# index-tts/index-tts

Measured on AMD Instinct MI355X. Metric: audio-seconds/sec (RTF) IndexTTS-2.5, 64-utt batch @1/2/4/8 MI355X, higher is better.
Workload: dtype bf16 (GPT GEMM operands / KV cache; f32 accumulate, residual stream, norms: the reference's own GPU mode) + fp32x3 (flow matching: f32 activations / weights / accumulation, GEMM and attention products on the bf16 matrix pipe with every f32 operand carried exactly as three bf16 planes = 24 significan

## Files before the change

### include/indextts_hip.h

```cpp
#ifndef INDEXTTS_HIP_H
#define INDEXTTS_HIP_H

#include <stddef.h>
#include <stdint.h>

#ifdef __cplusplus
extern "C" {
#endif

#define ITTS_ABI_VERSION 13

int itts_abi_version(void);
const char* itts_last_error(void);
int itts_device_count(void);

int itts_set_option(const char* name, int value);
int itts_get_option(const char* name, int* value);
int itts_reset_options(void);
int itts_option_count(void);
const char* itts_option_name(int index);
const char* itts_option_doc(int index);
int itts_option_default(int index);


int itts_aa_act_forward(const float* x, float* y, const float* alpha, const float* beta, const float* up_filter,
                        const float* down_filter, int B, int C, int T, const int32_t* lens, int len_mult,
                        int logscale, void* stream);

size_t itts_packed_conv_floats(int Cout, int Cin, int k);
int itts_pack_conv1d_weight(const float* w, int Cout, int Cin, int k, float* out);
int itts_pack_convT_weight(const float* w, int Cin, int Cout, int k, int u, int phase, float* out);

int itts_conv1d_forward(const float* x, const float* wpk, const float* bias, const float* bias_b, const float* res,
                        float* y, int B, int Cin, int Cout, int T, int k, int dilation, const int32_t* lens,
                        int len_mult, int acc_mode, float div, void* stream);

size_t itts_conv1d_h3_packed_bytes(int Cout, int Cin, int k);
int itts_pack_conv1d_h3_weight(const float* w, int Cout, int Cin, int k, void* out);
size_t itts_conv1d_h3_scratch_bytes(int B, int Cin, int T);
int itts_conv1d_h3_forward(const float* x, const void* wp3, const float* bias, const float* res, float* y, int B, int Cin, int Cout,
                           int T, int k, int dilation, const int32_t* lens, int len_mult, int acc_mode, float div, void* scratch,
                           void* stream);

size_t itts_conv1d_x3_packed_bytes(int Cout, int Cin, int k);
int itts_pack_conv1d_x3_weight(const float* w, int Cout, int Cin, int k, void* out);
size_t itts_conv1d_x3_scratch_bytes(int B, int Cin, int T);
int itts_conv1d_x3_forward(const float* x, const void* wp3, const float* bias, const float* res, float* y, int B, int Cin, int Cout,
                           int T, int k, int dilation, const int32_t* lens, int len_mult, int acc_mode, float div, void* scratch,
                           void* stream);
int itts_conv_transpose1d_forward(const float* x, const float* wpk_phases, const float* bias, const float* bias_b,
                                  float* y, int B, int Cin, int Cout, int Tin, int k, int u, const int32_t* lens,
                                  int len_mult_in, void* stream);

const char* itts_voc_last_path(void);
int itts_voc_path_count(void);
const char* itts_voc_path_name(int index);
int itts_aa_act_planes_forward(const float* x, void* planes, const float* alpha, const float* beta, const float* up_filter,
                               const float* down_filter, int B, int C, int T, const int32_t* lens, int len_mult, int logscale,
                               void* stream);
int itts_sin_reduced_forward(const float* x, float* y, size_t n, void* stream);

typedef struct {
    int32_t in_channels;
    int32_t upsample_initial_channel;
    int32_t num_upsamples;
    int32_t upsample_rates[8];
    int32_t upsample_kernel_sizes[8];
    int32_t num_kernels;
    int32_t resblock_kernel_sizes[4];
    int32_t num_dilations;
    int32_t resblock_dilations[4][4];
    int32_t snake_logscale;
    int32_t activation;
    int32_t use_tanh_at_final;
    int32_t use_bias_at_final;
    int32_t cond_dim;
    int32_t cond_in_each_up_layer;
} itts_bigvgan_config;

typedef struct itts_bigvgan itts_bigvgan;

int itts_bigvgan_create(const itts_bigvgan_config* cfg, itts_bigvgan** out);
int itts_bigvgan_device(const itts_bigvgan* h);
int itts_bigvgan_set_conv_mode(itts_bigvgan* h, int mode, int min_channels);
int itts_bigvgan_range_check(itts_bigvgan* h);
int itts_bigvgan_load_tensor(itts_bigvgan* h, const char* name, const float* host_data, const int64_t* shape, int ndim);
int itts_bigvgan_finalize(itts_bigvgan* h);
void itts_bigvgan_destroy(itts_bigvgan* h);
size_t itts_bigvgan_workspace_bytes(const itts_bigvgan* h, int B, int T);

int itts_bigvgan_forward(itts_bigvgan* h, const float* x, const int32_t* lens, const float* spk, float* wav, int B,
                         int T, void* workspace, size_t workspace_bytes, void* stream);

typedef struct itts_bigvgan_stream itts_bigvgan_stream;
int itts_bigvgan_stream_open(itts_bigvgan* h, int chunk_frames, int halo_frames, itts_bigvgan_stream** out);
size_t itts_bigvgan_stream_workspace_bytes(const itts_bigvgan_stream* s);
int itts_bigvgan_stream_push(itts_bigvgan_stream* s, const float* mel, int ld_mel, int n_frames, int is_last,
                             const float* spk, float* wav_out, int32_t* n_samples_out, void* workspace,
                             size_t workspace_bytes, void* stream);
void itts_bigvgan_stream_close(itts_bigvgan_stream* s);

int itts_bigvgan_set_profiling(itts_bigvgan* h, int enable);
int itts_bigvgan_profile_read(itts_bigvgan* h, double* ms, double* launches, double* flops, double* bytes);
int itts_bigvgan_profile_records(itts_bigvgan* h, double* out, int max_records);

#define ITTS_PREC_F32 0
#define ITTS_PREC_BF16 1
#define ITTS_PREC_F32X3 2

typedef struct {
    int32_t layers, model_dim, heads;
    int32_t vocab;
    int32_t n_mel_pos;
    int32_t precision;
    int32_t start_mel_token, stop_mel_token;
    float ln_eps;
} itts_gpt_config;

typedef struct {
    int32_t do_sample;
    int32_t num_beams;
    int32_t top_k;
    int32_t min_tokens_to_keep;
    int32_t max_new_tokens;
    int32_t pos_offset;
    float top_p, temperature, repetition_penalty, length_penalty;
    float typical_mass;
    int32_t reserved;
    uint64_t seed;
} itts_gen_params;

typedef struct itts_gpt itts_gpt;

size_t itts_packed_gemm_bytes(int K, int N, int precision);
int itts_pack_gemm_weight(const float* w, int K, int N, int transposed, int precision, void* out);

int itts_gpt_create(const itts_gpt_config* cfg, itts_gpt** out);
int itts_gpt_device(const itts_gpt* h);
int itts_gpt_load_tensor(itts_gpt* h, const char* name, const float* host_data, const int64_t* shape, int ndim);
int itts_gpt_finalize(itts_gpt* h);
void itts_gpt_destroy(itts_gpt* h);
size_t itts_gpt_workspace_bytes(const itts_gpt* h, int nseq, int S, int Tmax);

int itts_gpt_generate(itts_gpt* h, const float* prefix_embeds, const int32_t* pad_lens, int nseq, int S,
                      const itts_gen_params* params, const int32_t* penalty_ids, int n_penalty_ids,
                      const double* uniforms, int64_t* codes_out, int32_t* n_steps_out, void* workspace,
                      size_t workspace_bytes, int use_graph, void* stream);
int itts_gpt_generate_chunk(itts_gpt* h, const float* prefix_embeds, const int32_t* pad_lens, int nseq, int S,
                            const itts_gen_params* params, const int32_t* penalty_ids, int n_penalty_ids,
                            const double* uniforms, int64_t* codes_out, int32_t step_limit, int32_t* n_steps_out,
                            void* workspace, size_t workspace_bytes, int use_graph, void* stream);
size_t itts_gpt_admit_workspace_bytes(const itts_gpt* h, int n_new, int S_new);
int itts_gpt_admit_rows(itts_gpt* h, const float* prefix_embeds, const int32_t* pad_lens, const int32_t* slots, int n_new, int S_new,
                        const int32_t* row_limits_new, const itts_gen_params* params, const int32_t* penalty_ids, int n_penalty_ids,
                        const double* uniforms, int64_t* codes_out, void* workspace, size_t workspace_bytes, void* admit_workspace,
                        size_t admit_bytes, void* stream);
size_t itts_gpt_beam_workspace_bytes(const itts_gpt* h, int n_utts, int num_beams, int S, int Tmax);
int itts_gpt_generate_beam(itts_gpt* h, const float* prefix_embeds, const int32_t* pad_lens, int n_utts, int num_beams,
                           int S, const itts_gen_params* params, const int32_t* penalty_ids, int n_penalty_ids,
                           const double* uniforms, int32_t* hist_tok_out, int32_t* hist_par_out, float* beam_scores_out,
                           float* hyps_out, int32_t* n_hyps_out, uint8_t* done_out, int32_t* n_steps_out,
                           void* workspace, size_t workspace_bytes, int use_graph, void* stream);
int itts_gpt_generate_beam_chunk(itts_gpt* h, const float* prefix_embeds, const int32_t* pad_lens, int n_utts, int num_beams, int S,
                                 const itts_gen_params* params, const int32_t* penalty_ids, int n_penalty_ids, const int32_t* group_caps,
                                 int32_t* hist_tok_out, int32_t* hist_par_out, float* beam_scores_out, float* hyps_out, int32_t* n_hyps_out,
                                 uint8_t* done_out, int32_t step_limit, int32_t* n_steps_out, void* workspace, size_t workspace_bytes,
                                 int use_graph, void* stream);
size_t itts_gpt_admit_beam_workspace_bytes(const itts_gpt* h, int n_new, int S_new);
int itts_gpt_admit_beam_groups(itts_gpt* h, const float* prefix_embeds, const int32_t* pad_lens, const int32_t* slots, int n_new, int S_new,
                               const int32_t* group_caps_new, const itts_gen_params* params, const int32_t* penalty_ids, int n_penalty_ids,
                               void* workspace, size_t workspace_bytes, void* admit_workspace, size_t admit_bytes, void* stream);
int itts_gpt_last_timing(const itts_gpt* h, float* prefill_ms, float* decode_ms, int32_t* steps);
int itts_gpt_graph_stats(const itts_gpt* h, int32_t* captures, int32_t* hits);
int itts_gpt_set_compaction(itts_gpt* h, int enable, int granularity);
int itts_gpt_set_chunk_return(itts_gpt* h, int finished_rows);
int itts_gpt_set_row_limits(itts_gpt* h, const int32_t* limits, int n);
int itts_gpt_set_code_prefix(itts_gpt* h, const int64_t* codes, const int32_t* lens, int n, int width, int prefix_pos_offset, int chunk);
size_t itts_gpt_admit_prefix_workspace_bytes(const itts_gpt* h, int n_new, int S_new, int max_prefix);
int itts_gpt_last_prefix(const itts_gpt* h, int32_t* max_len, int32_t* chunks);
int itts_gpt_set_token_scores(itts_gpt* h, float* logp_model, float* logp_sampled, int n, int max_new);
int itts_gpt_set_alignment(itts_gpt* h, const int32_t* pairs, int n_pairs, const int32_t* span, float* out, int n, int max_new, int text_cap);
typedef struct {
    int32_t  do_sample, top_k, min_tokens_to_keep;
    float    top_p, temperature, repetition_penalty, typical_mass;
    int32_t  stream;
    uint64_t seed;
} itts_row_sampling;
int itts_gpt_set_row_sampling(itts_gpt* h, const itts_row_sampling* table, int n);
typedef struct {
    int32_t  do_sample, top_k, min_tokens_to_keep;
    float    top_p, temperature, repetition_penalty, typical_mass, length_penalty;
    int32_t  stream;
    uint64_t seed;
} itts_group_sampling;
int itts_gpt_set_group_sampling(itts_gpt* h, const itts_group_sampling* table, int n_groups);
typedef struct {
    int32_t  min_new_tokens;
    int32_t  min_length;
    int32_t  no_repeat_ngram_size;
    int32_t  decay_start;
    float    min_p;
    float    epsilon_cutoff;
    float    eta_cutoff;
    int32_t  n_suppress, n_begin_suppress, n_decay;
    const int32_t* suppress_ids;
    const int32_t* begin_suppress_ids;
    const float*   decay_table;
} itts_logits_filters;
int itts_gpt_set_logits_filters(itts_gpt* h, const itts_logits_filters* f);
int itts_gpt_compaction_stats(const itts_gpt* h, int64_t* row_steps, int32_t* compactions);

int itts_gpt_forward_latent(itts_gpt* h, const float* x, int nseq, int S, float* out, void* workspace,
                            size_t workspace_bytes, void* stream);
// ... 155 lines not shown
```

### indextts_amd/_lib.py

```python
import ctypes as C
import os

HERE = os.path.dirname(os.path.abspath(__file__))
LIB_PATH = os.path.join(HERE, "csrc", "libindextts_hip.so")

c_f32p = C.POINTER(C.c_float)
c_i32p = C.POINTER(C.c_int32)
c_i64p = C.POINTER(C.c_int64)
vp = C.c_void_p


class BigVGANConfig(C.Structure):
    _fields_ = [
        ("in_channels", C.c_int32), ("upsample_initial_channel", C.c_int32), ("num_upsamples", C.c_int32),
        ("upsample_rates", C.c_int32 * 8), ("upsample_kernel_sizes", C.c_int32 * 8), ("num_kernels", C.c_int32),
        ("resblock_kernel_sizes", C.c_int32 * 4), ("num_dilations", C.c_int32),
        ("resblock_dilations", (C.c_int32 * 4) * 4), ("snake_logscale", C.c_int32), ("activation", C.c_int32),
        ("use_tanh_at_final", C.c_int32), ("use_bias_at_final", C.c_int32), ("cond_dim", C.c_int32),
        ("cond_in_each_up_layer", C.c_int32),
    ]


class S2MelConfig(C.Structure):
    _fields_ = [("hidden_dim", C.c_int32), ("num_heads", C.c_int32), ("depth", C.c_int32), ("in_channels", C.c_int32),
                ("wavenet_hidden", C.c_int32), ("wavenet_layers", C.c_int32), ("wavenet_kernel", C.c_int32),
                ("wavenet_dilation_rate", C.c_int32), ("precision", C.c_int32), ("norm_eps", C.c_float)]


class FbankConfig(C.Structure):
    _fields_ = [("frame_length", C.c_int32), ("hop", C.c_int32), ("n_fft", C.c_int32), ("n_mels", C.c_int32), ("pad", C.c_int32),
                ("remove_dc", C.c_int32), ("power", C.c_int32), ("take_log", C.c_int32), ("layout", C.c_int32),
                ("preemphasis", C.c_float), ("mag_eps", C.c_float), ("floor", C.c_float), ("scale", C.c_float)]


class GPTConfig(C.Structure):
    _fields_ = [("layers", C.c_int32), ("model_dim", C.c_int32), ("heads", C.c_int32), ("vocab", C.c_int32),
                ("n_mel_pos", C.c_int32), ("precision", C.c_int32), ("start_mel_token", C.c_int32),
                ("stop_mel_token", C.c_int32), ("ln_eps", C.c_float)]


ABI_VERSION = 13
ERR_ARG, ERR_HIP, ERR_STATE = 1, 2, 3


class GenParams(C.Structure):
    _fields_ = [("do_sample", C.c_int32), ("num_beams", C.c_int32), ("top_k", C.c_int32),
                ("min_tokens_to_keep", C.c_int32), ("max_new_tokens", C.c_int32), ("pos_offset", C.c_int32),
                ("top_p", C.c_float), ("temperature", C.c_float), ("repetition_penalty", C.c_float),
                ("length_penalty", C.c_float), ("typical_mass", C.c_float), ("reserved", C.c_int32),
                ("seed", C.c_uint64)]


class RowSampling(C.Structure):
    _fields_ = [("do_sample", C.c_int32), ("top_k", C.c_int32), ("min_tokens_to_keep", C.c_int32),
                ("top_p", C.c_float), ("temperature", C.c_float), ("repetition_penalty", C.c_float),
                ("typical_mass", C.c_float), ("stream", C.c_int32), ("seed", C.c_uint64)]


class GroupSampling(C.Structure):
    _fields_ = [("do_sample", C.c_int32), ("top_k", C.c_int32), ("min_tokens_to_keep", C.c_int32),
                ("top_p", C.c_float), ("temperature", C.c_float), ("repetition_penalty", C.c_float),
                ("typical_mass", C.c_float), ("length_penalty", C.c_float), ("stream", C.c_int32), ("seed", C.c_uint64)]


class LogitsFilters(C.Structure):
    _fields_ = [("min_new_tokens", C.c_int32), ("min_length", C.c_int32), ("no_repeat_ngram_size", C.c_int32), ("decay_start", C.c_int32),
                ("min_p", C.c_float), ("epsilon_cutoff", C.c_float), ("eta_cutoff", C.c_float),
                ("n_suppress", C.c_int32), ("n_begin_suppress", C.c_int32), ("n_decay", C.c_int32),
                ("suppress_ids", C.POINTER(C.c_int32)), ("begin_suppress_ids", C.POINTER(C.c_int32)), ("decay_table", C.POINTER(C.c_float))]


SIGNATURES = {
    "itts_abi_version": (C.c_int, []),
    "itts_last_error": (C.c_char_p, []),
    "itts_device_count": (C.c_int, []),
    "itts_set_option": (C.c_int, [C.c_char_p, C.c_int]),
    "itts_get_option": (C.c_int, [C.c_char_p, C.POINTER(C.c_int)]),
    "itts_reset_options": (C.c_int, []),
    "itts_option_count": (C.c_int, []),
    "itts_option_name": (C.c_char_p, [C.c_int]),
    "itts_option_doc": (C.c_char_p, [C.c_int]),
    "itts_option_default": (C.c_int, [C.c_int]),
    "itts_aa_act_forward": (C.c_int, [vp, vp, vp, vp, vp, vp, C.c_int, C.c_int, C.c_int, vp, C.c_int, C.c_int, vp]),
    "itts_packed_conv_floats": (C.c_size_t, [C.c_int, C.c_int, C.c_int]),
    "itts_pack_conv1d_weight": (C.c_int, [vp, C.c_int, C.c_int, C.c_int, vp]),
    "itts_pack_convT_weight": (C.c_int, [vp, C.c_int, C.c_int, C.c_int, C.c_int, C.c_int, vp]),
    "itts_conv1d_forward": (C.c_int, [vp, vp, vp, vp, vp, vp, C.c_int, C.c_int, C.c_int, C.c_int, C.c_int, C.c_int,
                                      vp, C.c_int, C.c_int, C.c_float, vp]),
    "itts_conv_transpose1d_forward": (C.c_int, [vp, vp, vp, vp, vp, C.c_int, C.c_int, C.c_int, C.c_int, C.c_int,
                                                C.c_int, vp, C.c_int, vp]),
    "itts_voc_last_path": (C.c_char_p, []),
    "itts_voc_path_count": (C.c_int, []),
    "itts_voc_path_name": (C.c_char_p, [C.c_int]),
    "itts_aa_act_planes_forward": (C.c_int, [vp, vp, vp, vp, vp, vp, C.c_int, C.c_int, C.c_int, vp, C.c_int, C.c_int, vp]),
    "itts_sin_reduced_forward": (C.c_int, [vp, vp, C.c_size_t, vp]),
    "itts_bigvgan_create": (C.c_int, [C.POINTER(BigVGANConfig), C.POINTER(vp)]),
    "itts_bigvgan_device": (C.c_int, [vp]),
    "itts_bigvgan_load_tensor": (C.c_int, [vp, C.c_char_p, vp, c_i64p, C.c_int]),
    "itts_bigvgan_set_conv_mode": (C.c_int, [vp, C.c_int, C.c_int]),
    "itts_bigvgan_range_check": (C.c_int, [vp]),
    "itts_conv1d_h3_packed_bytes": (C.c_size_t, [C.c_int, C.c_int, C.c_int]),
    "itts_pack_conv1d_h3_weight": (C.c_int, [vp, C.c_int, C.c_int, C.c_int, vp]),
    "itts_conv1d_h3_scratch_bytes": (C.c_size_t, [C.c_int, C.c_int, C.c_int]),
    "itts_conv1d_h3_forward": (C.c_int, [vp, vp, vp, vp, vp, C.c_int, C.c_int, C.c_int, C.c_int, C.c_int, C.c_int, vp, C.c_int, C.c_int,
                                         C.c_float, vp, vp]),
    "itts_conv1d_x3_packed_bytes": (C.c_size_t, [C.c_int, C.c_int, C.c_int]),
    "itts_pack_conv1d_x3_weight": (C.c_int, [vp, C.c_int, C.c_int, C.c_int, vp]),
    "itts_conv1d_x3_scratch_bytes": (C.c_size_t, [C.c_int, C.c_int, C.c_int]),
    "itts_conv1d_x3_forward": (C.c_int, [vp, vp, vp, vp, vp, C.c_int, C.c_int, C.c_int, C.c_int, C.c_int, C.c_int, vp, C.c_int, C.c_int,
                                         C.c_float, vp, vp]),
    "itts_bigvgan_finalize": (C.c_int, [vp]),
    "itts_bigvgan_destroy": (None, [vp]),
    "itts_bigvgan_workspace_bytes": (C.c_size_t, [vp, C.c_int, C.c_int]),
    "itts_bigvgan_forward": (C.c_int, [vp, vp, vp, vp, vp, C.c_int, C.c_int, vp, C.c_size_t, vp]),
    "itts_bigvgan_stream_open": (C.c_int, [vp, C.c_int, C.c_int, C.POINTER(vp)]),
    "itts_bigvgan_stream_workspace_bytes": (C.c_size_t, [vp]),
    "itts_bigvgan_stream_push": (C.c_int, [vp, vp, C.c_int, C.c_int, C.c_int, vp, vp, C.POINTER(C.c_int32), vp, C.c_size_t, vp]),
    "itts_bigvgan_stream_close": (None, [vp]),
    "itts_bigvgan_set_profiling": (C.c_int, [vp, C.c_int]),
    "itts_bigvgan_profile_read": (C.c_int, [vp, vp, vp, vp, vp]),
    "itts_bigvgan_profile_records": (C.c_int, [vp, vp, C.c_int]),
    "itts_packed_gemm_bytes": (C.c_size_t, [C.c_int, C.c_int, C.c_int]),
    "itts_pack_gemm_weight": (C.c_int, [vp, C.c_int, C.c_int, C.c_int, C.c_int, vp]),
    "itts_gpt_create": (C.c_int, [C.POINTER(GPTConfig), C.POINTER(vp)]),
    "itts_gpt_device": (C.c_int, [vp]),
    "itts_gpt_load_tensor": (C.c_int, [vp, C.c_char_p, vp, c_i64p, C.c_int]),
    "itts_gpt_finalize": (C.c_int, [vp]),
    "itts_gpt_destroy": (None, [vp]),
    "itts_gpt_workspace_bytes": (C.c_size_t, [vp, C.c_int, C.c_int, C.c_int]),
    "itts_gpt_generate": (C.c_int, [vp, vp, vp, C.c_int, C.c_int, C.POINTER(GenParams), c_i32p, C.c_int, vp, vp,
                                    C.POINTER(C.c_int32), vp, C.c_size_t, C.c_int, vp]),
    "itts_gpt_generate_chunk": (C.c_int, [vp, vp, vp, C.c_int, C.c_int, C.POINTER(GenParams), c_i32p, C.c_int, vp, vp, C.c_int32,
                                          C.POINTER(C.c_int32), vp, C.c_size_t, C.c_int, vp]),
    "itts_gpt_beam_workspace_bytes": (C.c_size_t, [vp, C.c_int, C.c_int, C.c_int, C.c_int]),
    "itts_gpt_generate_beam": (C.c_int, [vp, vp, vp, C.c_int, C.c_int, C.c_int, C.POINTER(GenParams), c_i32p, C.c_int, vp,
                                         vp, vp, vp, vp, vp, vp, C.POINTER(C.c_int32), vp, C.c_size_t, C.c_int, vp]),
    "itts_gpt_admit_workspace_bytes": (C.c_size_t, [vp, C.c_int, C.c_int]),
    "itts_gpt_admit_rows": (C.c_int, [vp, vp, vp, vp, C.c_int, C.c_int, vp, vp, vp, C.c_int, vp, vp, vp, C.c_size_t, vp, C.c_size_t, vp]),
    "itts_gpt_generate_beam_chunk": (C.c_int, [vp, vp, vp, C.c_int, C.c_int, C.c_int, C.POINTER(GenParams), c_i32p, C.c_int, c_i32p,
                                               vp, vp, vp, vp, vp, vp, C.c_int32, C.POINTER(C.c_int32), vp, C.c_size_t, C.c_int, vp]),
    "itts_gpt_admit_beam_workspace_bytes": (C.c_size_t, [vp, C.c_int, C.c_int]),
    "itts_gpt_admit_beam_groups": (C.c_int, [vp, vp, vp, c_i32p, C.c_int, C.c_int, c_i32p, C.POINTER(GenParams), c_i32p, C.c_int,
                                             vp, C.c_size_t, vp, C.c_size_t, vp]),
    "itts_gpt_last_timing": (C.c_int, [vp, C.POINTER(C.c_float), C.POINTER(C.c_float), C.POINTER(C.c_int32)]),
    "itts_gpt_graph_stats": (C.c_int, [vp, C.POINTER(C.c_int32), C.POINTER(C.c_int32)]),
    "itts_gpt_set_compaction": (C.c_int, [vp, C.c_int, C.c_int]),
    "itts_gpt_set_row_limits": (C.c_int, [vp, vp, C.c_int]),
    "itts_gpt_set_code_prefix": (C.c_int, [vp, vp, c_i32p, C.c_int, C.c_int, C.c_int, C.c_int]),
    "itts_gpt_admit_prefix_workspace_bytes": (C.c_size_t, [vp, C.c_int, C.c_int, C.c_int]),
    "itts_gpt_last_prefix": (C.c_int, [vp, C.POINTER(C.c_int32), C.POINTER(C.c_int32)]),
    "itts_gpt_set_token_scores": (C.c_int, [vp, vp, vp, C.c_int, C.c_int]),
    "itts_gpt_set_alignment": (C.c_int, [vp, C.POINTER(C.c_int32), C.c_int, vp, vp, C.c_int, C.c_int, C.c_int]),
    "itts_gpt_set_row_sampling": (C.c_int, [vp, vp, C.c_int]),
    "itts_gpt_set_group_sampling": (C.c_int, [vp, vp, C.c_int]),
    "itts_gpt_set_logits_filters": (C.c_int, [vp, C.POINTER(LogitsFilters)]),
    "itts_gpt_set_chunk_return": (C.c_int, [vp, C.c_int]),
    "itts_gpt_compaction_stats": (C.c_int, [vp, C.POINTER(C.c_int64), C.POINTER(C.c_int32)]),
    "itts_gpt_forward_latent": (C.c_int, [vp, vp, C.c_int, C.c_int, vp, vp, C.c_size_t, vp]),
    "itts_gpt_latent_workspace_bytes": (C.c_size_t, [vp, C.c_int, C.c_int, C.c_int, C.c_int]),
    "itts_gpt_latent_open": (C.c_int, [vp, vp, c_i32p, C.c_int, C.c_int, C.c_int, C.c_int, vp, C.c_size_t, vp, C.POINTER(vp)]),
    "itts_gpt_latent_append": (C.c_int, [vp, vp, C.c_int, vp, vp]),
    "itts_gpt_latent_appended": (C.c_int, [vp]),
    "itts_gpt_latent_close": (C.c_int, [vp]),
    "itts_gpt_rescore_workspace_bytes": (C.c_size_t, [vp, C.c_int, C.c_int, C.c_int, C.c_int]),
    "itts_gpt_rescore": (C.c_int, [vp, vp, vp, C.c_int, C.c_int, vp, c_i32p, C.c_int, C.c_int, vp, c_i32p, C.c_int, vp, vp, C.c_int, C.c_int,
                                   vp, C.c_size_t, vp]),
    "itts_gpt_logp_gather_forward": (C.c_int, [vp, vp, vp, C.c_int, C.c_int, C.c_int, vp]),
    "itts_gpt_attention_align_mq_forward": (C.c_int, [vp, vp, vp, vp, C.POINTER(C.c_int32), C.c_int, vp, vp, vp, vp, vp,
                                                      C.c_int, C.c_int, C.c_int, C.c_int, C.c_int, C.c_int, C.c_int, C.c_int, C.c_int, vp]),
    "itts_gemm_tile_occupancy": (C.c_int, [C.c_int, C.POINTER(C.c_int32)]),
    "itts_s2mel_create": (C.c_int, [C.POINTER(S2MelConfig), C.POINTER(vp)]),
    "itts_s2mel_device": (C.c_int, [vp]),
    "itts_s2mel_load_tensor": (C.c_int, [vp, C.c_char_p, vp, c_i64p, C.c_int]),
    "itts_s2mel_set_tail": (C.c_int, [vp, vp, vp, vp, vp, vp, vp, vp, C.c_int, C.c_int, C.c_int]),
    "itts_s2mel_finalize": (C.c_int, [vp]),
    "itts_s2mel_destroy": (None, [vp]),
    "itts_s2mel_workspace_bytes": (C.c_size_t, [vp, C.c_int, C.c_int, C.c_int]),
    "itts_s2mel_mods_per_step": (C.c_int, [vp]),
    "itts_s2mel_estimator": (C.c_int, [vp, vp, vp, vp, vp, vp, vp, vp, vp, vp, C.c_int, C.c_int, C.c_int, vp, vp, C.c_size_t, vp]),
    "itts_s2mel_solve": (C.c_int, [vp, vp, vp, vp, vp, vp, vp, vp, vp, vp, vp, C.c_int, C.c_int, C.c_int, C.c_int, C.c_int,
                                   C.POINTER(C.c_float), C.c_float, vp, C.c_size_t, vp]),
    "itts_s2mel_set_profiling": (C.c_int, [vp, C.c_int]),
    "itts_s2mel_profile_read": (C.c_int, [vp, vp, vp, vp]),
    "itts_s2mel_set_trace": (C.c_int, [vp, vp, C.c_int]),
    "itts_s2mel_trace_count": (C.c_int, [vp]),
    "itts_s2mel_trace_wanted": (C.c_int, [vp]),
    "itts_s2mel_trace_label": (C.c_char_p, [vp, C.c_int]),
    "itts_s2mel_set_capture": (C.c_int, [vp, vp, C.c_size_t, C.c_char_p]),
    "itts_s2mel_capture_offset": (C.c_longlong, [vp, C.c_int, C.POINTER(C.c_size_t)]),
    "itts_s2mel_noise_forward": (C.c_int, [vp, vp, vp, vp, vp, vp, vp, C.c_int, C.c_int, C.c_int, vp]),
    "itts_s2mel_attention_scratch_bytes": (C.c_size_t, [C.c_int, C.c_int, C.c_int, C.c_int, C.c_int]),
    "itts_s2mel_attention_forward": (C.c_int, [vp, vp, vp, vp, vp, vp, vp, C.c_int, C.c_int, C.c_int, C.c_int, C.c_int, vp, vp,
                                               C.c_size_t, vp]),
    "itts_vq_project_forward": (C.c_int, [vp, vp, vp, vp, vp, C.c_int, C.c_int, C.c_int, C.c_int, vp]),
    "itts_vq_search_forward": (C.c_int, [vp, vp, vp, vp, vp, vp, C.c_int, C.c_int, C.c_int, C.c_int, vp]),
    "itts_tok_gather_conv_forward": (C.c_int, [vp, vp, vp, vp, vp, vp, vp, C.c_int, C.c_int, C.c_int, vp]),
    "itts_tok_dwconv_forward": (C.c_int, [vp, vp, vp, vp, vp, vp, vp, C.c_int, C.c_int, C.c_int, vp]),
    "itts_tok_gelu_forward": (C.c_int, [vp, C.c_size_t, vp]),
    "itts_attention_forward": (C.c_int, [vp, vp, vp, vp, vp, vp, C.c_int, C.c_int, C.c_int, C.c_int, C.c_float, vp]),
    "itts_attention_relkey_forward": (C.c_int, [vp, vp, vp, vp, vp, vp, vp, vp, C.c_int, C.c_int, C.c_int, C.c_int, C.c_int, C.c_int, C.c_float, vp]),
    "itts_tok_dwconv_causal_forward": (C.c_int, [vp, vp, vp, vp, vp, vp, vp, C.c_int, C.c_int, C.c_int, vp]),
    "itts_tok_glu_forward": (C.c_int, [vp, vp, C.c_int, C.c_int, C.c_int, vp]),
    "itts_tok_act_forward": (C.c_int, [vp, C.c_size_t, C.c_int, vp]),
    "itts_tok_l2norm_forward": (C.c_int, [vp, vp, C.c_int, C.c_int, C.c_float, vp]),
    "itts_tok_affine_forward": (C.c_int, [vp, C.c_int, vp, vp, vp, C.c_int, C.c_int, C.c_int, vp]),
    "itts_tok_ctxpool_forward": (C.c_int, [vp, vp, C.c_int, C.c_int, C.c_int, vp]),
    "itts_tok_gate_forward": (C.c_int, [vp, vp, C.c_size_t, vp]),
    "itts_tok_attnstats_forward": (C.c_int, [vp, vp, vp, C.c_int, C.c_int, C.c_float, vp]),
    "itts_tok_statspool_forward": (C.c_int, [vp, vp, C.c_int, C.c_int, vp]),
    "itts_tok_ctxpool_seq_forward": (C.c_int, [vp, vp, vp, vp, C.c_int, C.c_int, C.c_int, vp]),
    "itts_tok_statspool_seq_forward": (C.c_int, [vp, vp, vp, vp, C.c_int, C.c_int, vp]),
    "itts_tok_gather_conv1d_seq_forward": (C.c_int, [vp, vp, vp, vp, vp, vp, C.c_int, C.c_int, C.c_int, C.c_int, C.c_int, C.c_int, vp]),
    "itts_tok_gather_conv2d_seq_forward": (C.c_int, [vp, vp, vp, vp, C.c_int, C.c_int, C.c_int, C.c_int, C.c_int, vp]),
    "itts_tok_scale_residual_forward": (C.c_int, [vp, vp, vp, C.c_int, C.c_int, vp]),
    "itts_tok_groupnorm_mish_forward": (C.c_int, [vp, vp, vp, vp, vp, C.c_int, C.c_int, C.c_float, vp]),
    "itts_gemm_last_path": (C.c_char_p, []),
    "itts_gemm_path_count": (C.c_int, []),
    "itts_gemm_path_name": (C.c_char_p, [C.c_int]),
    "itts_gemm_forward": (C.c_int, [vp, vp, vp, vp, C.c_int, C.c_int, C.c_int, C.c_int, C.c_int, C.c_int, vp]),
    "itts_attention_last_path": (C.c_char_p, []),
    "itts_attention_path_count": (C.c_int, []),
    "itts_attention_path_name": (C.c_char_p, [C.c_int]),
    "itts_gpt_attention_forward": (C.c_int, [vp, vp, vp, vp, vp, vp, vp, vp, vp, vp, vp, C.c_int, C.c_int, C.c_int, C.c_int, C.c_int, C.c_int, vp]),
    "itts_gpt_attention_align_forward": (C.c_int, [vp, vp, vp, vp, C.POINTER(C.c_int32), C.c_int, vp, vp, vp, vp, vp, vp, vp, vp, vp,
                                                   C.c_int, C.c_int, C.c_int, C.c_int, C.c_int, C.c_int, C.c_int, vp]),
    "itts_layernorm_forward": (C.c_int, [vp, vp, vp, vp, vp, vp, C.c_int, C.c_int, C.c_float, vp]),
    "itts_gemm_ln_forward": (C.c_int, [vp, vp, vp, vp, vp, C.c_float, vp, vp, vp, vp, C.c_int, C.c_int, C.c_int, vp]),
    "itts_fbank_frames": (C.c_int, [C.POINTER(FbankConfig), C.c_int]),
    "itts_fbank_forward": (C.c_int, [vp, C.c_int, C.c_int, C.c_int64, C.POINTER(FbankConfig), vp, vp, vp, vp, C.c_int, C.c_int64, vp]),
    "itts_resample_forward": (C.c_int, [vp, vp, vp, C.c_int, C.c_int, C.c_int64, C.c_int, C.c_int64, C.c_int, C.c_int, C.c_int, vp]),
    "itts_tok_colnorm_forward": (C.c_int, [vp, vp, C.c_int, C.c_int, C.c_int, C.c_int, C.c_int, C.c_float, vp]),
}

_lib = None


class HipEngineError(RuntimeError):
    pass


def lib():
    global _lib
    if _lib is None:
        if not os.path.exists(LIB_PATH):
            raise HipEngineError(
                f"{LIB_PATH} is missing: build it with `python indextts_amd/build.py` (hipcc, gfx950). "
                "The engine has no CPU fallback.")
        import torch
# ... 104 lines not shown
```

### indextts_amd/bigvgan.py

```python
import ctypes as C
import json
import os
from typing import Dict, Optional

import torch

from . import _lib

_V2_DEFAULTS = dict(
    num_mels=80, upsample_rates=[4, 4, 2, 2, 2, 2], upsample_kernel_sizes=[8, 8, 4, 4, 4, 4],
    upsample_initial_channel=1536, resblock_kernel_sizes=[3, 7, 11],
    resblock_dilation_sizes=[[1, 3, 5], [1, 3, 5], [1, 3, 5]], activation="snakebeta", snake_logscale=True,
    use_tanh_at_final=True, use_bias_at_final=True, resblock="1")


def fold_weight_norm(sd: Dict[str, torch.Tensor]) -> Dict[str, torch.Tensor]:
    out = dict(sd)
    for k in list(sd.keys()):
        if k.endswith(".weight_g"):
            base, g, v = k[:-9], sd[k], sd[k[:-9] + ".weight_v"]
        elif k.endswith(".parametrizations.weight.original0"):
            base = k[: -len(".parametrizations.weight.original0")]
            g, v = sd[k], sd[base + ".parametrizations.weight.original1"]
        else:
# ... 178 lines not shown
                spk = spk.expand(x.shape[0], -1).contiguous()
        else:
            spk = None
        x = x.float().contiguous()
        B, Cin, T = x.shape
        if Cin != self.in_channels:
            raise ValueError(f"expected {self.in_channels} input channels, got {Cin}")
        wav = torch.empty(B, 1, T * self.total_up, dtype=torch.float32, device=x.device)
        if B == 0 or T == 0:
            return (wav, None) if v1 else wav
        lens_t = None
        if lens is not None:
            lens_t = torch.as_tensor(lens, dtype=torch.int32, device=x.device).contiguous()
            if lens_t.numel() != B:
                raise ValueError("lens must have one entry per batch row")
        ws = self._workspace(B, T, x.device)
        rc = _lib.lib().itts_bigvgan_forward(self._h, _lib.ptr(x), _lib.ptr(lens_t), _lib.ptr(spk), _lib.ptr(wav), B, T,
                                             _lib.ptr(ws), ws.numel(), _lib.stream_ptr(x.device))
        _lib.check(rc, "itts_bigvgan_forward")
        if self.conv_mode == 1:
            bad = _lib.lib().itts_bigvgan_range_check(self._h)
            if bad:
                raise _lib.HipEngineError("BigVGAN(conv_mode='f16x3'): an activation was not finite or outside the f16 range "
                                          "(|x| >= 65504); use the exact f32 mode for this model / input")
        return (wav, None) if v1 else wav

    __call__ = forward

    def receptive_field_frames(self) -> int:
        h = self.h
        kmax = max(h["resblock_kernel_sizes"])
        reach = 0
        for d in max(h["resblock_dilation_sizes"], key=lambda ds: sum(ds)):
            reach += 6 + (kmax - 1) // 2 * d + 6 + (kmax - 1) // 2
        frames, rate = 3.0, 1
        for u, k in zip(h["upsample_rates"], h["upsample_kernel_sizes"]):
            frames += (k / u) / rate
            rate *= u
            frames += reach / rate
        frames += (6 + 3) / rate
        return int(frames) + 2

    def stream(self, mel: torch.Tensor, chunk_frames: int = 256, halo_frames: Optional[int] = None):
        halo = self.receptive_field_frames() if halo_frames is None else int(halo_frames)
        T = mel.shape[-1]
        up = self.total_up
        for t0 in range(0, T, chunk_frames):
            t1 = min(T, t0 + chunk_frames)
            a, b = max(0, t0 - halo), min(T, t1 + halo)
            w = self.forward(mel[..., a:b].contiguous())
            yield w[..., (t0 - a) * up: (t0 - a) * up + (t1 - t0) * up]

    def open_stream(self, chunk_frames: int = 256, halo_frames: Optional[int] = None) -> "BigVGANStream":
        return BigVGANStream(self, chunk_frames, self.receptive_field_frames() if halo_frames is None else int(halo_frames))

    def forward_chunked(self, mel: torch.Tensor, chunk_frames: int = 256, halo_frames: Optional[int] = None) -> torch.Tensor:
        return torch.cat(list(self.stream(mel, chunk_frames, halo_frames)), dim=-1)

    def set_profiling(self, enable: bool):
        _lib.check(_lib.lib().itts_bigvgan_set_profiling(self._h, int(enable)), "itts_bigvgan_set_profiling")

    def profile_records(self):
        buf = (C.c_double * (4 * 1024))()
        n = _lib.lib().itts_bigvgan_profile_records(self._h, buf, 1024)
        if n < 0:
            _lib.check(1, "itts_bigvgan_profile_records")
        return [(int(buf[4 * i]), buf[4 * i + 1], buf[4 * i + 2], buf[4 * i + 3]) for i in range(min(n, 1024))]

    def profile(self):
        arr = [(C.c_double * 4)() for _ in range(4)]
        _lib.check(_lib.lib().itts_bigvgan_profile_read(self._h, *arr), "itts_bigvgan_profile_read")
        names = ("conv1d_mfma", "conv_transpose1d_mfma", "aa_activation", "conv_post")
        return {n: dict(ms=arr[0][i], launches=int(arr[1][i]), flops=arr[2][i], bytes=arr[3][i]) for i, n in enumerate(names)}

    def __del__(self):
        try:
            if getattr(self, "_h", None) and self._h.value:
                _lib.lib().itts_bigvgan_destroy(self._h)
                self._h = C.c_void_p()
        except Exception:
            pass


class BigVGANStream:
    def __init__(self, model: BigVGAN, chunk_frames: int, halo_frames: int):
        if model.cond_dim > 0:
            raise NotImplementedError("streaming is wired for the v2 generator (no speaker conditioning)")
        self.model, self.chunk, self.halo = model, int(chunk_frames), int(halo_frames)
        self._s = C.c_void_p()
        _lib.check(_lib.lib().itts_bigvgan_stream_open(model._h, self.chunk, self.halo, C.byref(self._s)), "itts_bigvgan_stream_open")
        self._ws = None

    def push(self, mel_chunk: torch.Tensor, last: bool = False) -> torch.Tensor:
        n_new = int(mel_chunk.shape[-1])
        x = mel_chunk.reshape(self.model.in_channels, n_new).float().contiguous()
        if not x.is_cuda:
            raise _lib.HipEngineError("BigVGANStream needs a CUDA/HIP tensor")
        L = _lib.lib()
        if self._ws is None:
            self._ws = torch.empty(L.itts_bigvgan_stream_workspace_bytes(self._s), dtype=torch.uint8, device=x.device)
        out = torch.empty((self.chunk + self.halo) * self.model.total_up, dtype=torch.float32, device=x.device)
        n = C.c_int32(0)
        _lib.check(L.itts_bigvgan_stream_push(self._s, _lib.ptr(x) if n_new else None, max(1, n_new), n_new,
                                              int(last), None, _lib.ptr(out), C.byref(n), _lib.ptr(self._ws), self._ws.numel(),
                                              _lib.stream_ptr(x.device)), "itts_bigvgan_stream_push")
        return out[: n.value].reshape(1, 1, -1)

    def close(self):
        if self._s and self._s.value:
            _lib.lib().itts_bigvgan_stream_close(self._s)
            self._s = C.c_void_p()

    def __del__(self):
        try:
            self.close()
        except Exception:
            pass


def anti_alias_activation(x, up_filter, down_filter, alpha, beta, lens=None, logscale=True, *, len_mult=1, out=None):
    if not x.is_cuda:
        raise _lib.HipEngineError("anti_alias_activation needs a device tensor")
    x = x.float().contiguous()
    y = out if out is not None else torch.empty_like(x)
    B, Cc, T = x.shape
    dev = x.device
    f = lambda t: t.detach().reshape(-1).to(dev, torch.float32).contiguous()
    a, b, fu, fd = f(alpha), f(beta), f(up_filter), f(down_filter)
    lens_t = None if lens is None else torch.as_tensor(lens, dtype=torch.int32, device=dev).contiguous()
    with _lib.on_device(x.device):
        _lib.check(_lib.lib().itts_aa_act_forward(_lib.ptr(x), _lib.ptr(y), _lib.ptr(a), _lib.ptr(b), _lib.ptr(fu),
                                                  _lib.ptr(fd), B, Cc, T, _lib.ptr(lens_t), int(len_mult), int(logscale),
                                                  _lib.stream_ptr(x.device)), "itts_aa_act_forward")
        return y


def anti_alias_activation_planes(x, up_filter, down_filter, alpha, beta, lens=None, logscale=True, *, len_mult=1, out=None):
    if not x.is_cuda:
        raise _lib.HipEngineError("anti_alias_activation_planes needs a device tensor")
    x = x.float().contiguous()
    B, Cc, T = x.shape
    dev = x.device
    p = out if out is not None else torch.empty(3, B, T, Cc, dtype=torch.bfloat16, device=dev)
    f = lambda t: t.detach().reshape(-1).to(dev, torch.float32).contiguous()
    a, b, fu, fd = f(alpha), f(beta), f(up_filter), f(down_filter)
    lens_t = None if lens is None else torch.as_tensor(lens, dtype=torch.int32, device=dev).contiguous()
    with _lib.on_device(x.device):
        _lib.check(_lib.lib().itts_aa_act_planes_forward(_lib.ptr(x), _lib.ptr(p), _lib.ptr(a), _lib.ptr(b), _lib.ptr(fu), _lib.ptr(fd), B, Cc, T,
                                                         _lib.ptr(lens_t), int(len_mult), int(logscale), _lib.stream_ptr(x.device)),
                   "itts_aa_act_planes_forward")
        return p


def sin_reduced(x):
    if not x.is_cuda:
        raise _lib.HipEngineError("sin_reduced needs a device tensor")
    x = x.float().contiguous()
    y = torch.empty_like(x)
    with _lib.on_device(x.device):
        _lib.check(_lib.lib().itts_sin_reduced_forward(_lib.ptr(x), _lib.ptr(y), x.numel(), _lib.stream_ptr(x.device)), "itts_sin_reduced_forward")
        return y


def pack_conv1d_weight(w: torch.Tensor) -> torch.Tensor:
    w = w.detach().to("cpu", torch.float32).contiguous()
    Cout, Cin, k = w.shape
    L = _lib.lib()
    out = torch.empty(L.itts_packed_conv_floats(Cout, Cin, k), dtype=torch.float32)
    _lib.check(L.itts_pack_conv1d_weight(_lib.ptr(w), Cout, Cin, k, _lib.ptr(out)), "itts_pack_conv1d_weight")
    return out


def pack_conv1d_h3_weight(w: torch.Tensor) -> torch.Tensor:
    w = w.detach().to("cpu", torch.float32).contiguous()
    Cout, Cin, k = w.shape
    L = _lib.lib()
    n = L.itts_conv1d_h3_packed_bytes(Cout, Cin, k)
    if n == 0:
        raise ValueError("pack_conv1d_h3_weight: C_in must be a multiple of 32")
    out = torch.empty(n, dtype=torch.uint8)
    _lib.check(L.itts_pack_conv1d_h3_weight(_lib.ptr(w), Cout, Cin, k, _lib.ptr(out)), "itts_pack_conv1d_h3_weight")
    return out


def conv1d_h3(x, w3_packed, bias, Cout, k, dilation=1, res=None, lens=None, len_mult=1, out=None, acc_mode=0, div=1.0):
    x = x.float().contiguous()
    B, Cin, T = x.shape
    y = out if out is not None else torch.empty(B, Cout, T, dtype=torch.float32, device=x.device)
    lens_t = None if lens is None else torch.as_tensor(lens, dtype=torch.int32, device=x.device).contiguous()
    L = _lib.lib()
    scratch = torch.empty(L.itts_conv1d_h3_scratch_bytes(B, Cin, T), dtype=torch.uint8, device=x.device)
    with _lib.on_device(x.device):
        _lib.check(L.itts_conv1d_h3_forward(_lib.ptr(x), _lib.ptr(w3_packed), _lib.ptr(bias), _lib.ptr(res), _lib.ptr(y), B, Cin, Cout, T, k,
                                            dilation, _lib.ptr(lens_t), len_mult, acc_mode, float(div), _lib.ptr(scratch),
                                            _lib.stream_ptr(x.device)), "itts_conv1d_h3_forward")
        return y


def pack_conv1d_x3_weight(w: torch.Tensor) -> torch.Tensor:
    w = w.detach().to("cpu", torch.float32).contiguous()
    Cout, Cin, k = w.shape
    L = _lib.lib()
    n = L.itts_conv1d_x3_packed_bytes(Cout, Cin, k)
    if n == 0:
        raise ValueError("pack_conv1d_x3_weight: C_in must be a multiple of 32")
    out = torch.empty(n, dtype=torch.uint8)
    _lib.check(L.itts_pack_conv1d_x3_weight(_lib.ptr(w), Cout, Cin, k, _lib.ptr(out)), "itts_pack_conv1d_x3_weight")
    return out


def conv1d_x3(x, w3_packed, bias, Cout, k, dilation=1, res=None, lens=None, len_mult=1, out=None, acc_mode=0, div=1.0):
    x = x.float().contiguous()
    B, Cin, T = x.shape
    y = out if out is not None else torch.empty(B, Cout, T, dtype=torch.float32, device=x.device)
    lens_t = None if lens is None else torch.as_tensor(lens, dtype=torch.int32, device=x.device).contiguous()
    L = _lib.lib()
    scratch = torch.empty(L.itts_conv1d_x3_scratch_bytes(B, Cin, T), dtype=torch.uint8, device=x.device)
    with _lib.on_device(x.device):
        _lib.check(L.itts_conv1d_x3_forward(_lib.ptr(x), _lib.ptr(w3_packed), _lib.ptr(bias), _lib.ptr(res), _lib.ptr(y), B, Cin, Cout, T, k,
                                            dilation, _lib.ptr(lens_t), len_mult, acc_mode, float(div), _lib.ptr(scratch),
                                            _lib.stream_ptr(x.device)), "itts_conv1d_x3_forward")
        return y


def pack_convT_weight(w: torch.Tensor, u: int) -> torch.Tensor:
    w = w.detach().to("cpu", torch.float32).contiguous()
    Cin, Cout, k = w.shape
    L = _lib.lib()
    per = L.itts_packed_conv_floats(Cout, Cin, k // u)
    out = torch.empty(per * u, dtype=torch.float32)
    for r in range(u):
        _lib.check(L.itts_pack_convT_weight(_lib.ptr(w), Cin, Cout, k, u, r, C.c_void_p(out.data_ptr() + 4 * per * r)),
                   "itts_pack_convT_weight")
    return out


def conv1d(x, w_packed, bias, Cout, k, dilation=1, res=None, lens=None, len_mult=1, out=None, acc_mode=0, div=1.0, *, bias_b=None):
    x = x.float().contiguous()
    B, Cin, T = x.shape
    y = out if out is not None else torch.empty(B, Cout, T, dtype=torch.float32, device=x.device)
    lens_t = None if lens is None else torch.as_tensor(lens, dtype=torch.int32, device=x.device).contiguous()
    with _lib.on_device(x.device):
        _lib.check(_lib.lib().itts_conv1d_forward(_lib.ptr(x), _lib.ptr(w_packed), _lib.ptr(bias), _lib.ptr(bias_b), _lib.ptr(res),
                                                  _lib.ptr(y), B, Cin, Cout, T, k, dilation, _lib.ptr(lens_t), len_mult,
                                                  acc_mode, float(div), _lib.stream_ptr(x.device)), "itts_conv1d_forward")
        return y


def conv_transpose1d(x, w_packed, bias, Cout, k, u, lens=None, *, bias_b=None, len_mult=1, out=None):
    x = x.float().contiguous()
    B, Cin, T = x.shape
    y = out if out is not None else torch.zeros(B, Cout, T * u, dtype=torch.float32, device=x.device)
    lens_t = None if lens is None else torch.as_tensor(lens, dtype=torch.int32, device=x.device).contiguous()
    with _lib.on_device(x.device):
        _lib.check(_lib.lib().itts_conv_transpose1d_forward(_lib.ptr(x), _lib.ptr(w_packed), _lib.ptr(bias), _lib.ptr(bias_b),
                                                            _lib.ptr(y), B, Cin, Cout, T, k, u, _lib.ptr(lens_t), int(len_mult),
                                                            _lib.stream_ptr(x.device)), "itts_conv_transpose1d_forward")
        return y
```

### indextts_amd/csrc/bigvgan_kernels.h

```cpp
#pragma once
#include "common.h"

struct ConvArgs {
    const float* x;
    float* y;
    const float* wpk;
    const float* bias;
    const float* bias_b;
    const float* res;
    const int* lens;
    int len_mult_in, len_mult_out;
    int Cin, Cout, Tin, Tout;
    int k, tap_base, tap_step, ostride, ooff, m_extra;
    int acc_mode;
    float div;
    int B, n_mt, n_co;
};

enum VocPath {
    VP_NONE = -1,
    VP_CONV_F32_BM32, VP_CONV_F32_BM64, VP_CONV_F32_BM96, VP_CONV_F32_BM128,
    VP_CONV_X3_NH1, VP_CONV_X3_NH2,
    VP_CONV_H3_TWO_STAGE, VP_CONV_H3_WIN256X128, VP_CONV_H3_WIN192X192, VP_CONV_H3_WIN256X96,
    VP_AA_V1_SINF, VP_AA_V2_SINF, VP_AA_V2_VSIN, VP_AA_PLANES_VSIN,
    VP_COUNT
};
void voc_note_path(int path);
int voc_last_path();
const char* voc_path_name(int path);

int launch_aa_act(const float* x, float* y, const float* alpha, const float* beta, const float* fu, const float* fd,
                  int B, int C, int T, const int* lens, int len_mult, int logscale, hipStream_t st);
int launch_sin_reduced(const float* x, float* y, size_t n, hipStream_t st);
int launch_conv(const ConvArgs& a, int B, hipStream_t st);
int launch_conv_post(const float* x, float* y, const float* w, const float* bias, int B, int Cin, int T, int k,
                     const int* lens, int len_mult, int use_tanh, hipStream_t st);
int launch_cond_bias(const float* spk, const float* w, const float* bias, float* out, int B, int Cout, int cond_dim,
                     hipStream_t st);

struct ConvH3Args {
    const void* xh; const void* xl;
    const void* wp;
    const float* bias;
    const float* res;
    float* y;
    const void* zero_row;
    const int* lens; int len_mult;
    int B, Cin, Cout, T, k, dil;
    int acc_mode; float div;
    int n_mt, n_co;
};
struct ConvX3Args {
    const void* xp;
    const void* wp;
    const float* bias;
    const float* res;
    float* y;
    const void* zero_row;
    const int* lens; int len_mult;
    int B, Cin, Cout, T, k, dil;
    int acc_mode; float div;
    int n_mt, n_co;
};
bool conv_x3_supported(int Cin, int Cout, int k, int dil);
size_t conv_x3_packed_bytes(int Cout, int Cin, int k);
int conv_x3_pack(const float* w, int Cout, int Cin, int k, void* out);
int launch_split_tm3(const float* x, void* xp, int B, int C, int T, const int* lens, int len_mult, hipStream_t st);
int launch_aa_act_planes(const float* x, void* xp, const float* alpha, const float* beta, const float* fu, const float* fd,
                         int B, int C, int T, const int* lens, int len_mult, int logscale, hipStream_t st);
int launch_conv_x3(const ConvX3Args& a, hipStream_t st);
size_t conv_h3_packed_bytes(int Cout, int Cin, int k);
int conv_h3_pack(const float* w, int Cout, int Cin, int k, void* out);
int launch_split_tm(const float* x, void* xh, void* xl, int B, int C, int T, const int* lens, int len_mult, int* range_flag, hipStream_t st);
int launch_conv_h3(const ConvH3Args& a, hipStream_t st);
```

### indextts_amd/csrc/bigvgan_kernels.hip

```cpp
#include "bigvgan_kernels.h"
#include <stdlib.h>

#define AA_TILE 1024

__global__ __launch_bounds__(256) void aa_act_kernel(const float* __restrict__ x, float* __restrict__ y,
                                                     const float* __restrict__ alpha, const float* __restrict__ beta,
                                                     const float* __restrict__ fu, const float* __restrict__ fd,
                                                     int C, int T, const int* __restrict__ lens, int len_mult,
                                                     int logscale) {
    __shared__ float xs[AA_TILE + 16];
    __shared__ float vs[2 * AA_TILE + 16];
    __shared__ float fus[12], fds[12];
    const int b = blockIdx.z, c = blockIdx.y;
    const int t0 = blockIdx.x * AA_TILE;
    const int len = lens ? min(lens[b] * len_mult, T) : T;
    if (t0 >= len) return;
    const int tid = threadIdx.x;
    if (tid < 12) { fus[tid] = fu[tid]; fds[tid] = fd[tid]; }
    const float* xr = x + ((size_t)b * C + c) * T;
    float* yr = y + ((size_t)b * C + c) * T;
    float a_e = alpha[c], b_e = beta[c];
    if (logscale) { a_e = expf(a_e); b_e = expf(b_e); }
    const float inv_b = 1.0f / (b_e + 1e-9f);
    const int n_out = min(AA_TILE, len - t0);
// ... 142 lines not shown
            for (int p = 0; p < 4; ++p)
                if (i0 + p < n_out) yr[t0 + i0 + p] = o[p];
        }
    }
}

#define AAP_TT 128
#define AAP_CB 32
#define AAP_RS 36
__device__ __forceinline__ uint32_t aap_cvt2(float a, float b) {
    typedef __bf16 bf2 __attribute__((ext_vector_type(2)));
    typedef float f2 __attribute__((ext_vector_type(2)));
    return __builtin_bit_cast(uint32_t, __builtin_convertvector(f2{a, b}, bf2));
}
__device__ __forceinline__ void aap_wave_sync() {
    __builtin_amdgcn_fence(__ATOMIC_RELEASE, "wavefront");
    __builtin_amdgcn_wave_barrier();
    __builtin_amdgcn_fence(__ATOMIC_ACQUIRE, "wavefront");
}
__device__ __forceinline__ int aap_slot(int tt) { return (tt & 3) * 32 + (tt >> 2); }

__global__ __launch_bounds__(256) void aa_act_planes_kernel(const float* __restrict__ x, u16* __restrict__ xh, u16* __restrict__ xm, u16* __restrict__ xl,
                                                            const float* __restrict__ alpha, const float* __restrict__ beta,
                                                            const float* __restrict__ fu, const float* __restrict__ fd,
                                                            int C, int T, const int* __restrict__ lens, int len_mult, int logscale) {
    __shared__ __attribute__((aligned(256))) float xs[4][2][192];
    __shared__ __attribute__((aligned(256))) float vs[4][2][320];
    __shared__ __attribute__((aligned(16))) u16 ot[3][AAP_TT][AAP_RS];
    const int b = blockIdx.z, c0 = blockIdx.y * AAP_CB, t0 = blockIdx.x * AAP_TT;
    const int tid = threadIdx.x, lane = tid & 63, w = tid >> 6, sub = lane >> 5, pos = lane & 31;
    const int len = lens ? min(lens[b] * len_mult, T) : T;
    const int n_out = len - t0 < AAP_TT ? (len - t0 < 0 ? 0 : len - t0) : AAP_TT;
    if (n_out > 0) {
        float fus[12], fds[12];
#pragma unroll
        for (int j = 0; j < 12; ++j) { fus[j] = 2.0f * fu[j]; fds[j] = fd[j]; }
        float* xw_ = xs[w][sub];
        float* vw_ = vs[w][sub];
        int toff[5];
#pragma unroll
        for (int k = 0; k < 5; ++k) {
            int t = t0 - 6 + pos + 32 * k;
            toff[k] = t < 0 ? 0 : (t > len - 1 ? len - 1 : t);
        }
        auto chan = [&](int it) { const int c = c0 + w * 8 + it * 2 + sub; return c < C ? c : C - 1; };
        float xn[5];
        {
            const float* xr = x + ((size_t)b * C + chan(0)) * T;
#pragma unroll
            for (int k = 0; k < 5; ++k) xn[k] = xr[toff[k]];
        }
#pragma unroll 1
        for (int it = 0; it < 4; ++it) {
            const int cl = w * 8 + it * 2 + sub;
            const bool c_ok = c0 + cl < C;
            float a_e = alpha[chan(it)], b_e = beta[chan(it)];
            if (logscale) { a_e = expf(a_e); b_e = expf(b_e); }
            const float inv_b = 1.0f / (b_e + 1e-9f);
            aap_wave_sync();
#pragma unroll
            for (int k = 0; k < 5; ++k) xw_[pos + 32 * k] = xn[k];
            if (it < 3) {
                const float* xr = x + ((size_t)b * C + chan(it + 1)) * T;
#pragma unroll
                for (int k = 0; k < 5; ++k) xn[k] = xr[toff[k]];
            }
            aap_wave_sync();
            auto snake8 = [&](int vb, float* v) {
                float xw[12];
                *(f32x4*)&xw[0] = *(const f32x4*)&xw_[(vb >> 1)];
                *(f32x4*)&xw[4] = *(const f32x4*)&xw_[(vb >> 1) + 4];
                *(f32x4*)&xw[8] = *(const f32x4*)&xw_[(vb >> 1) + 8];
#pragma unroll
                for (int p = 0; p < 4; ++p) {
                    float ue = 0.f, uo = 0.f;
#pragma unroll
                    for (int j = 0; j < 6; ++j) {
                        ue = fmaf(fus[1 + 2 * j], xw[p + 5 - j], ue);
                        uo = fmaf(fus[2 * j], xw[p + 6 - j], uo);
                    }
                    const float se = sin_reduced(ue * a_e);
                    const float so = sin_reduced(uo * a_e);
                    v[2 * p] = fmaf(inv_b * se, se, ue);
                    v[2 * p + 1] = fmaf(inv_b * so, so, uo);
                }
            };
            {
                float v[8];
                const int vb = 8 * pos;
                snake8(vb, v);
                *(f32x4*)&vw_[aa_sw(vb)] = *(const f32x4*)&v[0];
                *(f32x4*)&vw_[aa_sw(vb + 4)] = *(const f32x4*)&v[4];
            }
            if (pos < 2) {
                float vt[8];
                snake8(2 * AAP_TT + 8 * pos, vt);
                *(f32x4*)&vw_[aa_sw(2 * AAP_TT + 8 * pos)] = *(const f32x4*)&vt[0];
                *(f32x4*)&vw_[aa_sw(2 * AAP_TT + 8 * pos + 4)] = *(const f32x4*)&vt[4];
            }
            aap_wave_sync();
            if (t0 == 0 && pos < 6) vw_[aa_sw(pos)] = vw_[aa_sw(6)];
            const int vi_end = (2 * len - 1) - (2 * t0 - 6);
            if (vi_end < 2 * AAP_TT + 12 - 1) {
                const int vi = vi_end + 1 + pos;
                if (pos < 8 && vi < 2 * AAP_TT + 16) vw_[aa_sw(vi)] = vw_[aa_sw(vi_end)];
            }
            aap_wave_sync();
            float vw[20];
            const int base = 8 * pos;
#pragma unroll
            for (int k = 0; k < 5; ++k) *(f32x4*)&vw[4 * k] = *(const f32x4*)&vw_[aa_sw(base + 4 * k)];
            float o[4];
#pragma unroll
            for (int p = 0; p < 4; ++p) {
                float acc = 0.f;
#pragma unroll
                for (int j = 0; j < 12; ++j) acc = fmaf(fds[j], vw[2 * p + j + 1], acc);
                o[p] = (4 * pos + p < n_out && c_ok) ? acc : 0.f;
            }
#pragma unroll
            for (int e = 0; e < 2; ++e) {
                const float f0 = o[2 * e], f1 = o[2 * e + 1];
                const uint32_t h = aap_cvt2(f0, f1);
                const float r0 = f0 - __uint_as_float(h << 16), r1 = f1 - __uint_as_float(h & 0xffff0000u);
                const uint32_t m = aap_cvt2(r0, r1);
                const float s0 = r0 - __uint_as_float(m << 16), s1 = r1 - __uint_as_float(m & 0xffff0000u);
                const uint32_t l = aap_cvt2(s0, s1);
                const int sa = aap_slot(4 * pos + 2 * e), sb = aap_slot(4 * pos + 2 * e + 1);
                ot[0][sa][cl] = (u16)h; ot[0][sb][cl] = (u16)(h >> 16);
                ot[1][sa][cl] = (u16)m; ot[1][sb][cl] = (u16)(m >> 16);
                ot[2][sa][cl] = (u16)l; ot[2][sb][cl] = (u16)(l >> 16);
            }
        }
    }
    __syncthreads();
    const size_t plane_row = (size_t)b * T;
    const int q = tid & 3;
#pragma unroll 1
    for (int r = tid >> 2; r < 3 * AAP_TT; r += 64) {
        const int p = r / AAP_TT, tt = r - p * AAP_TT;
        const int t = t0 + tt;
        if (t >= T || c0 + 8 * q >= C) continue;
        uint2 lo = {0u, 0u}, hi = {0u, 0u};
        if (n_out > 0) {
            const u16* src = &ot[p][aap_slot(tt)][8 * q];
            lo = *(const uint2*)src;
            hi = *(const uint2*)(src + 4);
        }
        u16* dst = (p == 0 ? xh : (p == 1 ? xm : xl)) + (plane_row + t) * C + c0 + 8 * q;
        *(uint4*)dst = uint4{lo.x, lo.y, hi.x, hi.y};
    }
}

#define CI_CHUNK 32
#define CONV_HALO 64


template <int WM, int WN, int MT, int NT>
__global__ __launch_bounds__(256) __attribute__((amdgpu_waves_per_eu((WM == 1 && MT == 1) ? 4 : 1, (WM == 1 && MT == 1) ? 4 : 8)))
void conv_mfma_kernel(ConvArgs a) {
    constexpr int BM = WM * MT * 32;
    constexpr int BN = WN * NT * 32;
    constexpr int LDW = BN + CONV_HALO;
    extern __shared__ __attribute__((aligned(16))) float xs[];

    const int tid = threadIdx.x, lane = tid & 63, w = tid >> 6;
    const int wm = w / WN, wn = w % WN;
    const int L = blockIdx.x;
    const int xcd = L & 7, slot = L >> 3;
    const int tile = (slot / a.n_co) * 8 + xcd;
    if (tile >= a.n_mt * a.B) return;
    const int b = tile / a.n_mt;
    const int m0 = (tile - b * a.n_mt) * BN;
    const int co0 = (slot % a.n_co) * BM;
    const int len_in = a.lens ? min(a.lens[b] * a.len_mult_in, a.Tin) : a.Tin;
    const int len_out = a.lens ? min(a.lens[b] * a.len_mult_out, a.Tout) : a.Tout;
    const int m_count = len_in + a.m_extra;
    if (m0 >= m_count) return;

    const int span = (a.k - 1) * (a.tap_step < 0 ? -a.tap_step : a.tap_step);
    const int last_off = a.tap_base + (a.k - 1) * a.tap_step;
    const int min_off = a.tap_base < last_off ? a.tap_base : last_off;
    const int W = BN + span;
    const int n_cosub = (a.Cout + 31) >> 5;
    const int cin8 = a.Cin >> 3;

    f32x16 acc[MT][NT];
#pragma unroll
    for (int i = 0; i < MT; ++i)
#pragma unroll
        for (int j = 0; j < NT; ++j)
#pragma unroll
            for (int r = 0; r < 16; ++r) acc[i][j][r] = 0.f;

    const float* xb = a.x + (size_t)b * a.Cin * a.Tin;
    const int lane_row = lane >> 5;
    const int lane_col = lane & 31;

    constexpr int NCOL = LDW / 64;
    float stage[CI_CHUNK / 4][NCOL];
    const int w_u = __builtin_amdgcn_readfirstlane(w);
    auto stage_load = [&](int ci0s) {
        const int cnt = min(CI_CHUNK, a.Cin - ci0s);
#pragma unroll
        for (int rr = 0; rr < CI_CHUNK / 4; ++rr) {
            const int r = w_u + 4 * rr;
            const bool row_ok = r < cnt;
            const float* xr = xb + (size_t)(ci0s + (row_ok ? r : 0)) * a.Tin;
            const __amdgpu_buffer_rsrc_t rsrc =
                __builtin_amdgcn_make_buffer_rsrc(const_cast<float*>(xr), 0, row_ok ? len_in * 4 : 0, 0x00020000);
#pragma unroll
            for (int i = 0; i < NCOL; ++i) {
                const int t = m0 + min_off + lane + 64 * i;
                stage[rr][i] = __builtin_bit_cast(float, __builtin_amdgcn_raw_buffer_load_b32(rsrc, t * 4, 0, 0));
            }
        }
    };
    auto stage_write = [&]() {
#pragma unroll
        for (int rr = 0; rr < CI_CHUNK / 4; ++rr)
#pragma unroll
            for (int i = 0; i < NCOL; ++i) xs[(w + 4 * rr) * LDW + lane + 64 * i] = stage[rr][i];
    };
    stage_load(0);

    constexpr int CP4 = CI_CHUNK / 8;
    f32x4 a_cur[CP4][MT], a_nxt[CP4][MT];
    const int nchunks = (a.Cin + CI_CHUNK - 1) / CI_CHUNK;
    const int G = nchunks * a.k;
    const unsigned wpk_bytes = (unsigned)n_cosub * a.k * cin8 * 64u * 16u;
    const __amdgpu_buffer_rsrc_t wrs = __builtin_amdgcn_make_buffer_rsrc(const_cast<float*>(a.wpk), 0, (int)wpk_bytes, 0x00020000);
    auto load_tap = [&](int g, f32x4 (&dst)[CP4][MT]) {
        const int c = g / a.k, j = g - c * a.k;
        const int cbase = c * CI_CHUNK;
        const int cp4n = min(CI_CHUNK, a.Cin - cbase) >> 3;
#pragma unroll
        for (int cp4 = 0; cp4 < CP4; ++cp4) {
#pragma unroll
            for (int mt = 0; mt < MT; ++mt) {
                const int co_sub = (co0 >> 5) + wm * MT + mt;
                const bool ok = (cp4 < cp4n) && (co_sub < n_cosub);
                const unsigned off = ok ? ((unsigned)((co_sub * a.k + j) * cin8 + ((cbase >> 3) + cp4)) * 64u + lane) * 16u
                                        : 0xFFFFFFF0u;
                dst[cp4][mt] = __builtin_bit_cast(f32x4, __builtin_amdgcn_raw_buffer_load_b128(wrs, off, 0, 0));
            }
        }
    };
    auto compute_tap = [&](int j) {
        const int colb = wn * NT * 32 + lane_col + (a.tap_base + j * a.tap_step - min_off);
        const float* xcol = xs + lane_row * LDW + colb;
        float bcur[4][NT], bnxt[4][NT];
#pragma unroll
        for (int sidx = 0; sidx < 4; ++sidx)
#pragma unroll
            for (int nt = 0; nt < NT; ++nt) bcur[sidx][nt] = xcol[(2 * sidx) * LDW + nt * 32];
#pragma unroll
        for (int cp4 = 0; cp4 < CP4; ++cp4) {
            if (cp4 + 1 < CP4) {
#pragma unroll
                for (int sidx = 0; sidx < 4; ++sidx)
#pragma unroll
                    for (int nt = 0; nt < NT; ++nt) bnxt[sidx][nt] = xcol[((cp4 + 1) * 8 + 2 * sidx) * LDW + nt * 32];
            }
#pragma unroll
            for (int sidx = 0; sidx < 4; ++sidx)
#pragma unroll
                for (int mt = 0; mt < MT; ++mt)
#pragma unroll
                    for (int nt = 0; nt < NT; ++nt)
                        acc[mt][nt] = __builtin_amdgcn_mfma_f32_32x32x2f32(a_cur[cp4][mt][sidx], bcur[sidx][nt], acc[mt][nt], 0, 0, 0);
            if (cp4 + 1 < CP4) {
#pragma unroll
                for (int sidx = 0; sidx < 4; ++sidx)
#pragma unroll
                    for (int nt = 0; nt < NT; ++nt) bcur[sidx][nt] = bnxt[sidx][nt];
            }
        }
#pragma unroll
        for (int cp4 = 0; cp4 < CP4; ++cp4)
#pragma unroll
            for (int mt = 0; mt < MT; ++mt) a_cur[cp4][mt] = a_nxt[cp4][mt];
    };
    load_tap(0, a_cur);
    int g = 0;
    for (int ci0 = 0; ci0 < a.Cin; ci0 += CI_CHUNK) {
        __syncthreads();
        stage_write();
        __syncthreads();
        load_tap(g + 1 < G ? g + 1 : G - 1, a_nxt);
        stage_load(ci0 + CI_CHUNK);
        compute_tap(0);
        ++g;
        for (int j = 1; j < a.k; ++j, ++g) {
            load_tap(g + 1 < G ? g + 1 : G - 1, a_nxt);
            compute_tap(j);
        }
    }

    const int plane_bytes = a.Cout * a.Tout * 4;
    const __amdgpu_buffer_rsrc_t yrs =
        __builtin_amdgcn_make_buffer_rsrc(a.y + (size_t)b * a.Cout * a.Tout, 0, plane_bytes, 0x00020000);
    const float* resb = a.res ? a.res + (size_t)b * a.Cout * a.Tout : a.y;
    const __amdgpu_buffer_rsrc_t rrs = __builtin_amdgcn_make_buffer_rsrc(const_cast<float*>(resb), 0, plane_bytes, 0x00020000);
#pragma unroll
    for (int mt = 0; mt < MT; ++mt) {
#pragma unroll
        for (int hf = 0; hf < 2; ++hf) {
            int corow[8];
            float badd[8];
#pragma unroll
            for (int q = 0; q < 8; ++q) {
                const int r = hf * 8 + q;
                corow[q] = co0 + (wm * MT + mt) * 32 + (r & 3) + 8 * (r >> 2) + 4 * lane_row;
                badd[q] = 0.f;
            }
            if (a.bias) {
#pragma unroll
                for (int q = 0; q < 8; ++q) badd[q] = a.bias[corow[q] < a.Cout ? corow[q] : a.Cout - 1];
            }
            if (a.bias_b) {
                const float* bb = a.bias_b + (size_t)b * a.Cout;
#pragma unroll
                for (int q = 0; q < 8; ++q) badd[q] += bb[corow[q] < a.Cout ? corow[q] : a.Cout - 1];
            }
#pragma unroll
            for (int nt = 0; nt < NT; ++nt) {
                const int m = m0 + (wn * NT + nt) * 32 + lane_col;
                const int n = m * a.ostride + a.ooff;
                const bool n_ok = (m < m_count) && (n >= 0) && (n < len_out);
                unsigned voff[8];
                float v[8];
#pragma unroll
                for (int q = 0; q < 8; ++q) {
                    const bool ok = n_ok && corow[q] < a.Cout;
                    voff[q] = ok ? (unsigned)(corow[q] * a.Tout + n) * 4u : 0xFFFFFFF0u;
                    v[q] = acc[mt][nt][hf * 8 + q] + badd[q];
                }
                if (a.res) {
                    float rv[8];
#pragma unroll
                    for (int q = 0; q < 8; ++q) rv[q] = __builtin_bit_cast(float, __builtin_amdgcn_raw_buffer_load_b32(rrs, voff[q], 0, 0));
#pragma unroll
                    for (int q = 0; q < 8; ++q) v[q] += rv[q];
                }
                if (a.acc_mode != 0) {
                    float yo[8];
#pragma unroll
                    for (int q = 0; q < 8; ++q) yo[q] = __builtin_bit_cast(float, __builtin_amdgcn_raw_buffer_load_b32(yrs, voff[q], 0, 0));
#pragma unroll
                    for (int q = 0; q < 8; ++q) v[q] = a.acc_mode == 1 ? yo[q] + v[q] : (yo[q] + v[q]) / a.div;
                }
#pragma unroll
                for (int q = 0; q < 8; ++q) __builtin_amdgcn_raw_buffer_store_b32(__builtin_bit_cast(unsigned, v[q]), yrs, voff[q], 0, 0);
            }
        }
    }
}

__global__ __launch_bounds__(256) void conv_post_kernel(const float* __restrict__ x, float* __restrict__ y,
                                                        const float* __restrict__ w, const float* __restrict__ bias,
                                                        int Cin, int T, int k, const int* __restrict__ lens,
                                                        int len_mult, int use_tanh) {
    extern __shared__ float ws[];
    const int b = blockIdx.y;
    for (int i = threadIdx.x; i < Cin * k; i += 256) ws[i] = w[i];
    __syncthreads();
    const int t = blockIdx.x * 256 + threadIdx.x;
    if (t >= T) return;
    const int len = lens ? min(lens[b] * len_mult, T) : T;
    float acc = 0.f;
    if (t < len) {
        const int pad = (k - 1) / 2;
        acc = bias ? bias[0] : 0.f;
        const float* xb = x + (size_t)b * Cin * T;
        for (int ci = 0; ci < Cin; ++ci) {
            const float* xr = xb + (size_t)ci * T;
            for (int j = 0; j < k; ++j) {
                const int tt = t + j - pad;
                if (tt >= 0 && tt < len) acc = fmaf(ws[ci * k + j], xr[tt], acc);
            }
        }
        acc = use_tanh ? tanhf(acc) : fminf(1.0f, fmaxf(-1.0f, acc));
    }
    y[(size_t)b * T + t] = acc;
}

__global__ __launch_bounds__(256) void cond_bias_kernel(const float* __restrict__ spk, const float* __restrict__ w,
                                                        const float* __restrict__ bias, float* __restrict__ out,
                                                        int Cout, int cond_dim) {
    const int b = blockIdx.y;
    const int co = blockIdx.x * 256 + threadIdx.x;
    if (co >= Cout) return;
    float acc = bias ? bias[co] : 0.f;
    const float* wr = w + (size_t)co * cond_dim;
    const float* sr = spk + (size_t)b * cond_dim;
    for (int d = 0; d < cond_dim; ++d) acc = fmaf(wr[d], sr[d], acc);
    out[(size_t)b * Cout + co] = acc;
}

static const char* const kVocPathNames[VP_COUNT] = {
    "conv_f32_bm32", "conv_f32_bm64", "conv_f32_bm96", "conv_f32_bm128",
    "conv_x3_nh1", "conv_x3_nh2",
    "conv_h3_two_stage", "conv_h3_win256x128", "conv_h3_win192x192", "conv_h3_win256x96",
    "aa_v1_sinf", "aa_v2_sinf", "aa_v2_vsin", "aa_planes_vsin",
};
static thread_local int t_voc_last_path = VP_NONE;
void voc_note_path(int path) { t_voc_last_path = path; }
int voc_last_path() { return t_voc_last_path; }
const char* voc_path_name(int path) { return (path >= 0 && path < VP_COUNT) ? kVocPathNames[path] : nullptr; }

int launch_aa_act(const float* x, float* y, const float* alpha, const float* beta, const float* fu, const float* fd,
                  int B, int C, int T, const int* lens, int len_mult, int logscale, hipStream_t st) {
    if (B <= 0 || C <= 0 || T <= 0) return ITTS_OK;
    const int mode = itts_opt(OPT_AA_ACT);
    voc_note_path(mode == 0 ? VP_AA_V1_SINF : mode == 1 ? VP_AA_V2_SINF : VP_AA_V2_VSIN);
    if (mode == 0) hipLaunchKernelGGL(aa_act_kernel, dim3(ceil_div(T, AA_TILE), C, B), dim3(256), 0, st, x, y, alpha, beta, fu, fd, C, T, lens, len_mult, logscale);
    else if (mode == 1) hipLaunchKernelGGL((aa_act_kernel_v2<4, false>), dim3(ceil_div(T, 1024), C, B), dim3(256), 0, st, x, y, alpha, beta, fu, fd, C, T, lens, len_mult, logscale);
    else hipLaunchKernelGGL((aa_act_kernel_v2<4, true>), dim3(ceil_div(T, 1024), C, B), dim3(256), 0, st, x, y, alpha, beta, fu, fd, C, T, lens, len_mult, logscale);
    HIP_TRY(hipGetLastError());
    return ITTS_OK;
}

int launch_sin_reduced(const float* x, float* y, size_t n, hipStream_t st) {
    if (n == 0) return ITTS_OK;
    if (n > ((size_t)1 << 31)) { itts_set_error("sin_reduced: n too large"); return ITTS_ERR_ARG; }
    hipLaunchKernelGGL(sin_reduced_kernel, dim3((unsigned)((n + 255) / 256)), dim3(256), 0, st, x, y, n);
    HIP_TRY(hipGetLastError());
    return ITTS_OK;
}

int launch_aa_act_planes(const float* x, void* xp, const float* alpha, const float* beta, const float* fu, const float* fd,
                         int B, int C, int T, const int* lens, int len_mult, int logscale, hipStream_t st) {
    if (B <= 0 || C <= 0 || T <= 0) return ITTS_OK;
    if (C % 8) { itts_set_error("aa_act_planes: C %% 8 != 0"); return ITTS_ERR_ARG; }
    u16* p = (u16*)xp;
    const size_t plane = (size_t)B * T * C;
    voc_note_path(VP_AA_PLANES_VSIN);
    hipLaunchKernelGGL(aa_act_planes_kernel, dim3(ceil_div(T, AAP_TT), ceil_div(C, AAP_CB), B), dim3(256), 0, st, x, p, p + plane, p + 2 * plane,
                       alpha, beta, fu, fd, C, T, lens, len_mult, logscale);
    HIP_TRY(hipGetLastError());
    return ITTS_OK;
}

template <int WM, int WN, int MT, int NT>
static int launch_conv_cfg(const ConvArgs& a, int B, int m_total, hipStream_t st) {
    constexpr int BM = WM * MT * 32, BN = WN * NT * 32;
    const size_t lds = (size_t)CI_CHUNK * (BN + CONV_HALO) * sizeof(float);
    ConvArgs a2 = a;
    a2.B = B;
    a2.n_mt = ceil_div(m_total, BN);
    a2.n_co = ceil_div(a.Cout, BM);
    const long long tiles8 = ((long long)a2.n_mt * B + 7) / 8 * 8;
    const long long nblocks = tiles8 * a2.n_co;
    if (nblocks > 2147483647ll) { itts_set_error("conv: grid too large"); return ITTS_ERR_ARG; }
    voc_note_path(VP_CONV_F32_BM32 + BM / 32 - 1);
    hipLaunchKernelGGL((conv_mfma_kernel<WM, WN, MT, NT>), dim3((unsigned)nblocks), dim3(256), lds, st, a2);
    HIP_TRY(hipGetLastError());
    return ITTS_OK;
}

int launch_conv(const ConvArgs& a, int B, hipStream_t st) {
    if (B <= 0) return ITTS_OK;
    if (a.Cin % 8 != 0) { itts_set_error("conv: C_in=%d must be a multiple of 8", a.Cin); return ITTS_ERR_ARG; }
    if ((long long)a.Cout * a.Tout >= (1ll << 29)) { itts_set_error("conv: C_out*T_out = %lld exceeds the 2 GiB per-row plane limit", (long long)a.Cout * a.Tout); return ITTS_ERR_ARG; }
    if ((long long)a.Tin >= (1ll << 29)) { itts_set_error("conv: T too large"); return ITTS_ERR_ARG; }
    const int span = (a.k - 1) * (a.tap_step < 0 ? -a.tap_step : a.tap_step);
    if (span > CONV_HALO) { itts_set_error("conv: tap span %d exceeds halo %d", span, CONV_HALO); return ITTS_ERR_ARG; }
    const int m_total = a.Tin + a.m_extra;
    const int n_cosub = (a.Cout + 31) / 32;
    const int force_bm = itts_opt(OPT_CONV_BM);
    const int bm_sub = force_bm ? force_bm / 32 : 1;
    (void)n_cosub;
    switch (bm_sub) {
        case 1: return launch_conv_cfg<1, 4, 1, 2>(a, B, m_total, st);
        case 2: return launch_conv_cfg<1, 4, 2, 2>(a, B, m_total, st);
        case 3: return launch_conv_cfg<1, 4, 3, 2>(a, B, m_total, st);
        default: return launch_conv_cfg<2, 2, 2, 2>(a, B, m_total, st);
    }
}

int launch_conv_post(const float* x, float* y, const float* w, const float* bias, int B, int Cin, int T, int k,
                     const int* lens, int len_mult, int use_tanh, hipStream_t st) {
    if (B <= 0 || T <= 0) return ITTS_OK;
    dim3 grid(ceil_div(T, 256), B);
    hipLaunchKernelGGL(conv_post_kernel, grid, dim3(256), (size_t)Cin * k * sizeof(float), st, x, y, w, bias, Cin, T, k,
                       lens, len_mult, use_tanh);
    HIP_TRY(hipGetLastError());
    return ITTS_OK;
}

int launch_cond_bias(const float* spk, const float* w, const float* bias, float* out, int B, int Cout, int cond_dim,
                     hipStream_t st) {
    if (B <= 0 || Cout <= 0) return ITTS_OK;
    dim3 grid(ceil_div(Cout, 256), B);
    hipLaunchKernelGGL(cond_bias_kernel, grid, dim3(256), 0, st, spk, w, bias, out, Cout, cond_dim);
    HIP_TRY(hipGetLastError());
    return ITTS_OK;
}
```

### indextts_amd/csrc/bigvgan_x3.hip

```cpp
#include <string.h>

#include "bigvgan_kernels.h"
#include "common.h"

typedef __bf16 x3_bf16x8 __attribute__((ext_vector_type(8)));
typedef uint32_t x3_v4u __attribute__((ext_vector_type(4)));

#define CX3_BK 32
#define CX3_MT 4
#define CX3_NT 3
#define CX3_BM 256
#define CX3_BN 96
#define CX3_SLACK 64
#define CX3_ACH ((CX3_BM + CX3_SLACK) / 16)
#define CX3_ABUF (3 * CX3_ACH * 1024)
#define CX3_NWT 6
#define CX3_WST (3 * CX3_NWT * 1024)
#define CX3_LDS (2 * CX3_ABUF + 2 * CX3_WST)

__device__ __forceinline__ uint32_t cx3_cvt2(float a, float b) {
    typedef __bf16 bf2 __attribute__((ext_vector_type(2)));
    typedef float f2 __attribute__((ext_vector_type(2)));
    return __builtin_bit_cast(uint32_t, __builtin_convertvector(f2{a, b}, bf2));
}

__global__ __launch_bounds__(256) void split_tm3_kernel(const float* __restrict__ x, u16* __restrict__ xh, u16* __restrict__ xm, u16* __restrict__ xl,
                                                        int C, int T, const int* __restrict__ lens, int len_mult) {
    __shared__ float tile[64][65];
    const int b = blockIdx.z, c0 = blockIdx.y * 64, t0 = blockIdx.x * 64;
    const int tid = threadIdx.x, lane = tid & 63, w = tid >> 6;
    const int len = lens ? min(lens[b] * len_mult, T) : T;
    const float* xb = x + (size_t)b * C * T;
#pragma unroll
    for (int i = 0; i < 16; ++i) {
        const int c = c0 + w * 16 + i, t = t0 + lane;
        tile[w * 16 + i][lane] = (c < C && t < len) ? xb[(size_t)c * T + t] : 0.f;
    }
    __syncthreads();
    const int cb = (tid & 7) * 8;
    if (c0 + cb >= C) return;
#pragma unroll
    for (int hf = 0; hf < 2; ++hf) {
        const int tl = (tid >> 3) + 32 * hf, t = t0 + tl;
        if (t >= T) break;
        x3_v4u ph, pm, pl;
#pragma unroll
        for (int e = 0; e < 4; ++e) {
            const float f0 = tile[cb + 2 * e][tl], f1 = tile[cb + 2 * e + 1][tl];
            const uint32_t h = cx3_cvt2(f0, f1);
            const float r0 = f0 - __uint_as_float(h << 16), r1 = f1 - __uint_as_float(h & 0xffff0000u);
            const uint32_t m = cx3_cvt2(r0, r1);
            const float s0 = r0 - __uint_as_float(m << 16), s1 = r1 - __uint_as_float(m & 0xffff0000u);
            ph[e] = h; pm[e] = m; pl[e] = cx3_cvt2(s0, s1);
        }
        const size_t o = ((size_t)b * T + t) * C + c0 + cb;
        *(x3_v4u*)(xh + o) = ph;
        *(x3_v4u*)(xm + o) = pm;
        *(x3_v4u*)(xl + o) = pl;
    }
}

template <int N>
__device__ __forceinline__ void cx3_wait_vm() { asm volatile("s_waitcnt vmcnt(%0)" ::"n"(N) : "memory"); }

template <int NH>
__global__ __launch_bounds__(512) __attribute__((amdgpu_waves_per_eu(2, 2))) void conv_x3w_kernel(ConvX3Args a) {
    extern __shared__ __attribute__((aligned(16))) char sm[];
    const int lane = threadIdx.x & 63, w = __builtin_amdgcn_readfirstlane(threadIdx.x >> 6);
    const int wr = w >> 1, wc = w & 1;
    const int L = blockIdx.x;
    const int xcd = L & 7, slot = L >> 3;
    const int tile = (slot / a.n_co) * 8 + xcd;
    if (tile >= a.n_mt * a.B) return;
    const int b = tile / a.n_mt;
    const int m0 = (tile - b * a.n_mt) * CX3_BM;
    const int co0 = (slot % a.n_co) * (CX3_BN * NH);
    const int len = a.lens ? min(a.lens[b] * a.len_mult, a.T) : a.T;
    if (m0 >= len) return;
    const int nkc = a.Cin / CX3_BK, G = a.k * nkc * NH;
    const int ntiles = (a.Cout + 15) >> 4;
    const int pad = (a.k - 1) / 2 * a.dil;
    const int nach = (CX3_BM + 2 * pad + 15) >> 4;

    const int srow = lane & 15, skp = lane >> 4;
    const size_t plane = (size_t)a.B * a.T * a.Cin * 2;
    const char* x_b = (const char*)a.xp + ((size_t)b * a.T * a.Cin + skp * 8) * 2;
    const char* zr = (const char*)a.zero_row;
    const int my_ach = (nach - w + 7) >> 3;
    auto issue_a = [&](int kc_, int buf) {
        char* base = sm + buf * CX3_ABUF;
#pragma unroll
        for (int i = 0; i < 3; ++i) {
            const int c = w + 8 * i;
            if (c < nach) {
                const int t = m0 - pad + c * 16 + srow;
                const bool ok = (unsigned)t < (unsigned)a.T;
                const size_t o = ((size_t)(ok ? t : 0) * a.Cin + kc_ * CX3_BK) * 2;
#pragma unroll
                for (int pl = 0; pl < 3; ++pl)
                    __builtin_amdgcn_global_load_lds((const __attribute__((address_space(1))) void*)(ok ? x_b + pl * plane + o : zr),
                                                     (__attribute__((address_space(3))) void*)(base + (pl * CX3_ACH + c) * 1024), 16, 0, 0);
            }
        }
    };
    const bool w_on = w < CX3_NWT;
    auto issue_w = [&](int g) {
        if (!w_on) return;
        const int kc_ = g / (a.k * NH), r_ = g - kc_ * a.k * NH;
        const int h_ = r_ / a.k, j_ = r_ - h_ * a.k;
        int ntg = (co0 >> 4) + h_ * CX3_NWT + w;
        ntg = ntg < ntiles ? ntg : ntiles - 1;
        const char* wsrc = (const char*)a.wp + ((size_t)ntg * a.k * nkc + (size_t)j_ * nkc + kc_) * 1024 + lane * 16;
        const size_t wstream = (size_t)ntiles * a.k * nkc * 1024;
        char* base = sm + 2 * CX3_ABUF + (g & 1) * CX3_WST;
#pragma unroll
        for (int pl = 0; pl < 3; ++pl)
            __builtin_amdgcn_global_load_lds((const __attribute__((address_space(1))) void*)(wsrc + pl * wstream),
                                             (__attribute__((address_space(3))) void*)(base + (pl * CX3_NWT + w) * 1024), 16, 0, 0);
    };

    f32x4 acc[NH][CX3_MT][CX3_NT];
#pragma unroll
    for (int h = 0; h < NH; ++h)
#pragma unroll
        for (int i = 0; i < CX3_MT; ++i)
#pragma unroll
            for (int jn = 0; jn < CX3_NT; ++jn) acc[h][i][jn] = f32x4{0.f, 0.f, 0.f, 0.f};

    const int row16 = lane & 15, kg = lane >> 4;
    const int b_off = wc * CX3_NT * 1024 + lane * 16;

    issue_a(0, 0);
    issue_w(0);
    auto read_a = [&](int kc, int j, x3_v4u (&af)[CX3_MT][3]) {
        const char* abase = sm + (kc & 1) * CX3_ABUF;
        const int rbase = wr * CX3_MT * 16 + row16 + j * a.dil;
#pragma unroll
        for (int mt = 0; mt < CX3_MT; ++mt) {
            const int rr = rbase + mt * 16;
            const char* ap = abase + (rr >> 4) * 1024 + kg * 256 + (rr & 15) * 16;
#pragma unroll
            for (int pl = 0; pl < 3; ++pl) af[mt][pl] = *(const x3_v4u*)(ap + pl * CX3_ACH * 1024);
        }
    };
    bool a_recent = false;
    x3_v4u afc[CX3_MT][3];
    auto ktile = [&](int g, int kc, int kc_n, int j_n, f32x4 (&ac)[CX3_MT][CX3_NT], bool first_of_chunk) {
        if (a_recent) { if (my_ach == 3) cx3_wait_vm<9>(); else cx3_wait_vm<6>(); } else cx3_wait_vm<0>();
        __builtin_amdgcn_s_barrier();
        asm volatile("" ::: "memory");
        if (g + 1 < G) issue_w(g + 1);
        a_recent = false;
        if (first_of_chunk && kc + 1 < nkc) { issue_a(kc + 1, (kc + 1) & 1); a_recent = true; }
        const char* wbase = sm + 2 * CX3_ABUF + (g & 1) * CX3_WST;
        x3_v4u bf[CX3_NT][3];
#pragma unroll
        for (int nt = 0; nt < CX3_NT; ++nt)
#pragma unroll
            for (int pl = 0; pl < 3; ++pl) bf[nt][pl] = *(const x3_v4u*)(wbase + pl * CX3_NWT * 1024 + b_off + nt * 1024);
        if (g == 0) read_a(0, 0, afc);
        const char* abase_n = sm + (kc_n & 1) * CX3_ABUF;
        const int rbase_n = wr * CX3_MT * 16 + row16 + j_n * a.dil;
        const bool more = g + 1 < G;
#pragma unroll
        for (int mt = 0; mt < CX3_MT; ++mt) {
            constexpr int PA[6] = {2, 0, 1, 1, 0, 0};
            constexpr int PB[6] = {0, 2, 1, 0, 1, 0};
#pragma unroll
            for (int q = 0; q < 6; ++q)
#pragma unroll
                for (int nt = 0; nt < CX3_NT; ++nt)
                    ac[mt][nt] = __builtin_amdgcn_mfma_f32_16x16x32_bf16(__builtin_bit_cast(x3_bf16x8, afc[mt][PA[q]]),
                                                                         __builtin_bit_cast(x3_bf16x8, bf[nt][PB[q]]), ac[mt][nt], 0, 0, 0);
            if (more) {
                const int rr = rbase_n + mt * 16;
                const char* ap = abase_n + (rr >> 4) * 1024 + kg * 256 + (rr & 15) * 16;
#pragma unroll
                for (int pl = 0; pl < 3; ++pl) afc[mt][pl] = *(const x3_v4u*)(ap + pl * CX3_ACH * 1024);
            }
        }
    };
    {
        int g = 0;
        for (int kc = 0; kc < nkc; ++kc) {
#pragma unroll
            for (int h = 0; h < NH; ++h)
                for (int j = 0; j < a.k; ++j, ++g) {
                    int j_n = j + 1, kc_n = kc;
                    if (j_n == a.k) { j_n = 0; if (h == NH - 1) kc_n = kc + 1; }
                    ktile(g, kc, kc_n, j_n, acc[h], h == 0 && j == 0);
                }
        }
    }

    const bool vec = (a.T & 3) == 0;
    float* yb = a.y + (size_t)b * a.Cout * a.T;
    const float* rb = a.res ? a.res + (size_t)b * a.Cout * a.T : nullptr;
#pragma unroll
    for (int h = 0; h < NH; ++h)
#pragma unroll
    for (int nt = 0; nt < CX3_NT; ++nt) {
        const int co = co0 + h * CX3_BN + (wc * CX3_NT + nt) * 16 + (lane & 15);
        if (co >= a.Cout) continue;
        const float bias = a.bias ? a.bias[co] : 0.f;
#pragma unroll
        for (int mt = 0; mt < CX3_MT; ++mt) {
            const int t = m0 + (wr * CX3_MT + mt) * 16 + (lane >> 4) * 4;
            if (t >= len) continue;
            f32x4 v;
#pragma unroll
            for (int r = 0; r < 4; ++r) v[r] = acc[h][mt][nt][r] + bias;
            const size_t o = (size_t)co * a.T + t;
            if (vec && t + 3 < len) {
                if (rb) { const f32x4 rv = *(const f32x4*)(rb + o); v += rv; }
                if (a.acc_mode != 0) {
                    const f32x4 yo = *(const f32x4*)(yb + o);
                    v = yo + v;
                    if (a.acc_mode == 2) v = v / a.div;
                }
                *(f32x4*)(yb + o) = v;
            } else {
#pragma unroll
                for (int r = 0; r < 4; ++r) {
                    if (t + r >= len) break;
                    float s = v[r];
                    if (rb) s += rb[o + r];
                    if (a.acc_mode != 0) { s = yb[o + r] + s; if (a.acc_mode == 2) s = s / a.div; }
                    yb[o + r] = s;
                }
            }
        }
    }
}

bool conv_x3_supported(int Cin, int Cout, int k, int dil) {
    return Cin >= CX3_BK && Cin % CX3_BK == 0 && Cout >= 1 && (k & 1) && k >= 3 && (k - 1) * dil <= CX3_SLACK;
}

size_t conv_x3_packed_bytes(int Cout, int Cin, int k) {
    return (size_t)3 * ((Cout + 15) / 16) * ((size_t)k * (Cin / CX3_BK)) * 1024;
}

static uint16_t cx3_bf16_rne(float f) {
    uint32_t u;
    memcpy(&u, &f, 4);
    if ((u & 0x7f800000u) == 0x7f800000u) return (uint16_t)(u >> 16);
    u += 0x7fffu + ((u >> 16) & 1u);
    return (uint16_t)(u >> 16);
}
static float cx3_bf16_f(uint16_t h) { const uint32_t u = (uint32_t)h << 16; float f; memcpy(&f, &u, 4); return f; }

int conv_x3_pack(const float* w, int Cout, int Cin, int k, void* out) {
    if (!w || !out || Cout < 1 || Cin < CX3_BK || Cin % CX3_BK || k < 1 || !(k & 1)) {
        itts_set_error("conv_x3_pack: need C_in %% 32 == 0 and an odd kernel size (Cout=%d Cin=%d k=%d)", Cout, Cin, k);
        return ITTS_ERR_ARG;
    }
    const int ntiles = (Cout + 15) / 16, nkc = Cin / CX3_BK;
    const size_t nk = (size_t)k * nkc, stream = (size_t)ntiles * nk * 512;
    u16* o0 = (u16*)out;
    for (int nt = 0; nt < ntiles; ++nt)
        for (int j = 0; j < k; ++j)
            for (int kc = 0; kc < nkc; ++kc)
                for (int lane = 0; lane < 64; ++lane)
                    for (int e = 0; e < 8; ++e) {
                        const int co = nt * 16 + (lane & 15), ci = kc * CX3_BK + (lane >> 4) * 8 + e;
                        const float f = co < Cout ? w[((size_t)co * Cin + ci) * k + j] : 0.f;
                        if (!(f - f == 0.f)) { itts_set_error("conv_x3_pack: weight %g is not finite", (double)f); return ITTS_ERR_ARG; }
                        const uint16_t h = cx3_bf16_rne(f);
                        const float r = f - cx3_bf16_f(h);
                        const uint16_t m = cx3_bf16_rne(r);
                        const uint16_t l = cx3_bf16_rne(r - cx3_bf16_f(m));
                        const size_t o = (((size_t)nt * nk + (size_t)j * nkc + kc) * 64 + lane) * 8 + e;
                        o0[o] = h; o0[stream + o] = m; o0[2 * stream + o] = l;
                    }
    return ITTS_OK;
}

int launch_split_tm3(const float* x, void* xp, int B, int C, int T, const int* lens, int len_mult, hipStream_t st) {
    if (B <= 0 || C <= 0 || T <= 0) return ITTS_OK;
    if (C % 8) { itts_set_error("split_tm3: C %% 8 != 0"); return ITTS_ERR_ARG; }
    u16* p = (u16*)xp;
    const size_t plane = (size_t)B * T * C;
    hipLaunchKernelGGL(split_tm3_kernel, dim3(ceil_div(T, 64), ceil_div(C, 64), B), dim3(256), 0, st, x, p, p + plane, p + 2 * plane, C, T, lens, len_mult);
    HIP_TRY(hipGetLastError());
    return ITTS_OK;
}

int launch_conv_x3(const ConvX3Args& a0, hipStream_t st) {
    if (a0.B <= 0 || a0.T <= 0) return ITTS_OK;
    if (!conv_x3_supported(a0.Cin, a0.Cout, a0.k, a0.dil)) {
        itts_set_error("conv_x3: need C_in %% 32 == 0, odd k >= 3 and (k - 1) * dilation <= %d (Cin=%d k=%d dil=%d)", CX3_SLACK, a0.Cin, a0.k, a0.dil);
        return ITTS_ERR_ARG;
    }
    if ((long long)a0.Cout * a0.T >= (1ll << 31) || (long long)a0.Cin * a0.T >= (1ll << 31)) { itts_set_error("conv_x3: row plane too large"); return ITTS_ERR_ARG; }
    ConvX3Args a = a0;
    const int nh = a.Cout > CX3_BN ? 2 : 1;
    a.n_mt = ceil_div(a.T, CX3_BM);
    a.n_co = ceil_div(a.Cout, CX3_BN * nh);
    const long long tiles8 = ((long long)a.n_mt * a.B + 7) / 8 * 8;
    const long long nblocks = tiles8 * a.n_co;
    if (nblocks > 2147483647ll) { itts_set_error("conv_x3: grid too large"); return ITTS_ERR_ARG; }
    static ItPerDevice<bool> attr_set_pd;
    bool& attr_set = attr_set_pd.cur();
    if (!attr_set) {
        HIP_TRY(hipFuncSetAttribute((const void*)conv_x3w_kernel<1>, hipFuncAttributeMaxDynamicSharedMemorySize, CX3_LDS));
        HIP_TRY(hipFuncSetAttribute((const void*)conv_x3w_kernel<2>, hipFuncAttributeMaxDynamicSharedMemorySize, CX3_LDS));
        attr_set = true;
    }
    voc_note_path(nh == 2 ? VP_CONV_X3_NH2 : VP_CONV_X3_NH1);
    if (nh == 2) hipLaunchKernelGGL(conv_x3w_kernel<2>, dim3((unsigned)nblocks), dim3(512), CX3_LDS, st, a);
    else hipLaunchKernelGGL(conv_x3w_kernel<1>, dim3((unsigned)nblocks), dim3(512), CX3_LDS, st, a);
    HIP_TRY(hipGetLastError());
    return ITTS_OK;
}
```

### indextts_amd/csrc/capi_bigvgan.hip

```cpp
#include <math.h>
#include <stdarg.h>
#include <string.h>
#include <map>
#include <string>
#include <vector>

#include "../../include/indextts_hip.h"
#include "bigvgan_kernels.h"

static thread_local char g_err[1024] = "";
void itts_set_error(const char* fmt, ...) {
    va_list ap;
    va_start(ap, fmt);
    vsnprintf(g_err, sizeof(g_err), fmt, ap);
    va_end(ap);
}
extern "C" const char* itts_last_error(void) { return g_err; }
extern "C" int itts_abi_version(void) { return ITTS_ABI_VERSION; }
extern "C" int itts_device_count(void) {
    int n = 0;
    hipError_t e = hipGetDeviceCount(&n);
    if (e != hipSuccess) {
        itts_set_error("hipGetDeviceCount: %s", hipGetErrorString(e));
        return -1;
    }
    return n;
}

extern "C" size_t itts_packed_conv_floats(int Cout, int Cin, int k) {
    return (size_t)((Cout + 31) / 32) * k * (Cin / 8) * 64 * 4;
}

template <class F>
static void pack_generic(F w, int Cout, int Cin, int k, float* out) {
    const int n_cosub = (Cout + 31) / 32, cin8 = Cin / 8;
    for (int cs = 0; cs < n_cosub; ++cs)
        for (int j = 0; j < k; ++j)
            for (int c8 = 0; c8 < cin8; ++c8)
                for (int lane = 0; lane < 64; ++lane)
                    for (int s = 0; s < 4; ++s) {
                        const int co = cs * 32 + (lane & 31);
                        const int ci = c8 * 8 + 2 * s + (lane >> 5);
                        const size_t o = ((((size_t)cs * k + j) * cin8 + c8) * 64 + lane) * 4 + s;
                        out[o] = co < Cout ? w(co, ci, j) : 0.f;
                    }
}

extern "C" int itts_pack_conv1d_weight(const float* w, int Cout, int Cin, int k, float* out) {
    if (!w || !out || Cout <= 0 || Cin <= 0 || Cin % 8 || k <= 0) {
        itts_set_error("pack_conv1d: bad args Cout=%d Cin=%d k=%d (C_in must be a multiple of 8)", Cout, Cin, k);
        return ITTS_ERR_ARG;
    }
    pack_generic([&](int co, int ci, int j) { return w[((size_t)co * Cin + ci) * k + j]; }, Cout, Cin, k, out);
    return ITTS_OK;
}

extern "C" int itts_pack_convT_weight(const float* w, int Cin, int Cout, int k, int u, int phase, float* out) {
    if (!w || !out || Cin % 8 || u < 1 || k < u || k % u || ((k - u) & 1) || phase < 0 || phase >= u) {
        itts_set_error("pack_convT: bad args Cin=%d Cout=%d k=%d u=%d phase=%d (need k a multiple of u with k-u even)", Cin, Cout, k, u, phase);
        return ITTS_ERR_ARG;
    }
    pack_generic([&](int co, int ci, int jj) { return w[((size_t)ci * Cout + co) * k + phase + jj * u]; }, Cout, Cin, k / u,
                 out);
    return ITTS_OK;
}

extern "C" int itts_aa_act_forward(const float* x, float* y, const float* alpha, const float* beta,
                                   const float* up_filter, const float* down_filter, int B, int C, int T,
                                   const int32_t* lens, int len_mult, int logscale, void* stream) {
    if (!x || !y || !alpha || !beta || !up_filter || !down_filter || B < 0 || C < 0 || T < 0) {
        itts_set_error("aa_act: null pointer or negative dim");
        return ITTS_ERR_ARG;
    }
    if (B > 65535 || C > 65535) { itts_set_error("aa_act: B, C must be <= 65535"); return ITTS_ERR_ARG; }
    return launch_aa_act(x, y, alpha, beta, up_filter, down_filter, B, C, T, lens, len_mult < 1 ? 1 : len_mult,
                         logscale, (hipStream_t)stream);
}

extern "C" const char* itts_voc_last_path(void) {
    const char* n = voc_path_name(voc_last_path());
    return n ? n : "none";
}
extern "C" int itts_voc_path_count(void) { return VP_COUNT; }
extern "C" const char* itts_voc_path_name(int index) { return voc_path_name(index); }

extern "C" int itts_aa_act_planes_forward(const float* x, void* planes, const float* alpha, const float* beta, const float* up_filter,
                                          const float* down_filter, int B, int C, int T, const int32_t* lens, int len_mult, int logscale,
                                          void* stream) {
    if (!x || !planes || !alpha || !beta || !up_filter || !down_filter || B < 0 || C < 0 || T < 0) {
        itts_set_error("aa_act_planes: null pointer or negative dim");
        return ITTS_ERR_ARG;
    }
    if (B > 65535 || C > 65535 * 32) { itts_set_error("aa_act_planes: B must be <= 65535, C <= 32 * 65535"); return ITTS_ERR_ARG; }
    return launch_aa_act_planes(x, planes, alpha, beta, up_filter, down_filter, B, C, T, lens, len_mult < 1 ? 1 : len_mult, logscale,
                                (hipStream_t)stream);
}

extern "C" int itts_sin_reduced_forward(const float* x, float* y, size_t n, void* stream) {
    if (!x || !y) { itts_set_error("sin_reduced: null pointer"); return ITTS_ERR_ARG; }
    return launch_sin_reduced(x, y, n, (hipStream_t)stream);
}

static int conv1d_impl(const float* x, const float* wpk, const float* bias, const float* bias_b, const float* res,
                       float* y, int B, int Cin, int Cout, int T, int k, int dil, const int* lens, int len_mult,
                       int acc_mode, float div, hipStream_t st) {
    ConvArgs a;
    a.x = x; a.y = y; a.wpk = wpk; a.bias = bias; a.bias_b = bias_b; a.res = res; a.lens = lens;
    a.len_mult_in = a.len_mult_out = len_mult;
    a.Cin = Cin; a.Cout = Cout; a.Tin = T; a.Tout = T;
    a.k = k; a.tap_base = -((k - 1) / 2) * dil; a.tap_step = dil; a.ostride = 1; a.ooff = 0; a.m_extra = 0;
    a.acc_mode = acc_mode; a.div = div;
    return launch_conv(a, B, st);
}

extern "C" int itts_conv1d_forward(const float* x, const float* wpk, const float* bias, const float* bias_b,
                                   const float* res, float* y, int B, int Cin, int Cout, int T, int k, int dilation,
                                   const int32_t* lens, int len_mult, int acc_mode, float div, void* stream) {
    if (!x || !wpk || !y || B < 0 || T < 0 || k < 1 || (k & 1) == 0 || dilation < 1) {
        itts_set_error("conv1d: bad args (odd k, dilation >= 1 required)");
        return ITTS_ERR_ARG;
    }
    if (B > 65535) { itts_set_error("conv1d: B must be <= 65535"); return ITTS_ERR_ARG; }
    if (T == 0 || B == 0) return ITTS_OK;
    return conv1d_impl(x, wpk, bias, bias_b, res, y, B, Cin, Cout, T, k, dilation, lens, len_mult < 1 ? 1 : len_mult,
                       acc_mode, div, (hipStream_t)stream);
}

extern "C" size_t itts_conv1d_h3_packed_bytes(int Cout, int Cin, int k) { return (Cin > 0 && Cin % 32 == 0 && Cout > 0 && k > 0) ? conv_h3_packed_bytes(Cout, Cin, k) : 0; }
extern "C" int itts_pack_conv1d_h3_weight(const float* w, int Cout, int Cin, int k, void* out) { return conv_h3_pack(w, Cout, Cin, k, out); }
extern "C" size_t itts_conv1d_h3_scratch_bytes(int B, int Cin, int T) { return (size_t)B * T * Cin * 4 + 512; }
extern "C" int itts_conv1d_h3_forward(const float* x, const void* wp3, const float* bias, const float* res, float* y, int B, int Cin, int Cout,
                                      int T, int k, int dilation, const int32_t* lens, int len_mult, int acc_mode, float div, void* scratch,
                                      void* stream) {
    if (!x || !wp3 || !y || !scratch || B < 0 || T < 0 || acc_mode < 0 || acc_mode > 2) { itts_set_error("conv1d_h3_forward: bad args"); return ITTS_ERR_ARG; }
    if (B == 0 || T == 0) return ITTS_OK;
    hipStream_t st = (hipStream_t)stream;
    char* base = (char*)(((uintptr_t)scratch + 255) & ~(uintptr_t)255);
    const size_t half = (size_t)B * T * Cin * 2;
    void* zr = base + half * 2;
    HIP_TRY(hipMemsetAsync(zr, 0, 64, st));
    int rc = launch_split_tm(x, base, base + half, B, Cin, T, lens, len_mult < 1 ? 1 : len_mult, nullptr, st);
    if (rc) return rc;
    ConvH3Args g{};
    g.xh = base; g.xl = base + half; g.wp = wp3; g.bias = bias; g.res = res; g.y = y; g.zero_row = zr; g.lens = lens; g.len_mult = len_mult < 1 ? 1 : len_mult;
    g.B = B; g.Cin = Cin; g.Cout = Cout; g.T = T; g.k = k; g.dil = dilation; g.acc_mode = acc_mode; g.div = div;
    return launch_conv_h3(g, st);
}

extern "C" size_t itts_conv1d_x3_packed_bytes(int Cout, int Cin, int k) { return (Cin > 0 && Cin % 32 == 0 && Cout > 0 && k > 0) ? conv_x3_packed_bytes(Cout, Cin, k) : 0; }
extern "C" int itts_pack_conv1d_x3_weight(const float* w, int Cout, int Cin, int k, void* out) { return conv_x3_pack(w, Cout, Cin, k, out); }
extern "C" size_t itts_conv1d_x3_scratch_bytes(int B, int Cin, int T) { return (size_t)B * T * Cin * 6 + 512; }
extern "C" int itts_conv1d_x3_forward(const float* x, const void* wp3, const float* bias, const float* res, float* y, int B, int Cin, int Cout,
                                      int T, int k, int dilation, const int32_t* lens, int len_mult, int acc_mode, float div, void* scratch,
                                      void* stream) {
    if (!x || !wp3 || !y || !scratch || B < 0 || T < 0 || acc_mode < 0 || acc_mode > 2) { itts_set_error("conv1d_x3_forward: bad args"); return ITTS_ERR_ARG; }
    if (B == 0 || T == 0) return ITTS_OK;
    hipStream_t st = (hipStream_t)stream;
    char* base = (char*)(((uintptr_t)scratch + 255) & ~(uintptr_t)255);
    const size_t planes = (size_t)B * T * Cin * 6;
    void* zr = base + planes;
    HIP_TRY(hipMemsetAsync(zr, 0, 64, st));
    int rc = launch_split_tm3(x, base, B, Cin, T, lens, len_mult < 1 ? 1 : len_mult, st);
    if (rc) return rc;
    ConvX3Args g{};
    g.xp = base; g.wp = wp3; g.bias = bias; g.res = res; g.y = y; g.zero_row = zr; g.lens = lens; g.len_mult = len_mult < 1 ? 1 : len_mult;
    g.B = B; g.Cin = Cin; g.Cout = Cout; g.T = T; g.k = k; g.dil = dilation; g.acc_mode = acc_mode; g.div = div;
    return launch_conv_x3(g, st);
}

static int convT_impl(const float* x, const float* wpk_phases, const float* bias, const float* bias_b, float* y, int B,
                      int Cin, int Cout, int Tin, int k, int u, const int* lens, int len_mult_in, hipStream_t st) {
    const int p = (k - u) / 2, ntaps = k / u;
    const size_t per_phase = itts_packed_conv_floats(Cout, Cin, ntaps);
    for (int r = 0; r < u; ++r) {
        ConvArgs a;
        a.x = x; a.y = y; a.wpk = wpk_phases + per_phase * r; a.bias = bias; a.bias_b = bias_b; a.res = nullptr;
        a.lens = lens; a.len_mult_in = len_mult_in; a.len_mult_out = len_mult_in * u;
        a.Cin = Cin; a.Cout = Cout; a.Tin = Tin; a.Tout = Tin * u;
        a.k = ntaps; a.tap_base = 0; a.tap_step = -1; a.ostride = u; a.ooff = r - p; a.m_extra = ntaps - 1;
        a.acc_mode = 0; a.div = 1.f;
        int rc = launch_conv(a, B, st);
        if (rc) return rc;
    }
    return ITTS_OK;
}

extern "C" int itts_conv_transpose1d_forward(const float* x, const float* wpk_phases, const float* bias,
                                             const float* bias_b, float* y, int B, int Cin, int Cout, int Tin, int k,
                                             int u, const int32_t* lens, int len_mult_in, void* stream) {
    if (!x || !wpk_phases || !y || u < 1 || k < u || k % u || ((k - u) & 1)) {
        itts_set_error("conv_transpose1d: need k a multiple of u with k-u even (k=%d u=%d)", k, u);
        return ITTS_ERR_ARG;
    }
    if (B <= 0 || Tin <= 0) return ITTS_OK;
    return convT_impl(x, wpk_phases, bias, bias_b, y, B, Cin, Cout, Tin, k, u, lens, len_mult_in < 1 ? 1 : len_mult_in,
                      (hipStream_t)stream);
}

struct DevBuf {
    float* p = nullptr;
    size_t n = 0;
};
struct ConvL {
    int Cin = 0, Cout = 0, k = 0;
    DevBuf w, b;
    bool has_w = false, has_b = false;
    void* w3 = nullptr;
};
struct ActL {
    int C = 0;
    DevBuf alpha, beta, fu, fd;
    bool has_a = false, has_b = false, has_fu = false, has_fd = false;
};

struct itts_bigvgan {
    itts_bigvgan_config cfg;
    ConvL conv_pre;
    std::vector<ConvL> ups;
    std::vector<ConvL> convs1, convs2;
    std::vector<ActL> acts;
    ActL act_post;
    DevBuf post_w, post_b;
    bool has_post_w = false, has_post_b = false;
    ConvL cond_layer;
    std::vector<ConvL> conds;
    DevBuf default_filter;
    bool finalized = false;
    std::vector<float*> owned;
    int total_up = 1;
    bool profiling = false;
    std::vector<hipEvent_t> ev_pool;
    struct Rec { int cls; double flops; double bytes; };
    std::vector<Rec> recs;
    hipStream_t prof_stream = nullptr;
    int device = -1;
    int conv_mode = 0, h3_min_c = 96;
    void* zero_row = nullptr;
};

enum { PC_CONV = 0, PC_CONVT = 1, PC_ACT = 2, PC_POST = 3, PC_COUNT = 4 };

struct ProfScope {
    itts_bigvgan* h;
    hipStream_t st;
    bool on;
    size_t idx;
    ProfScope(itts_bigvgan* h_, hipStream_t st_, int cls, double flops, double bytes) : h(h_), st(st_), on(h_->profiling), idx(0) {
        if (!on) return;
        idx = h->recs.size();
        h->recs.push_back({cls, flops, bytes});
        while (h->ev_pool.size() < 2 * (idx + 1)) {
            hipEvent_t e;
            if (hipEventCreate(&e) != hipSuccess) { on = false; return; }
            h->ev_pool.push_back(e);
        }
        (void)hipEventRecord(h->ev_pool[2 * idx], st);
    }
    ~ProfScope() {
        if (on) (void)hipEventRecord(h->ev_pool[2 * idx + 1], st);
    }
};

static int upload(itts_bigvgan* h, const float* host, size_t n, DevBuf* dst) {
    if (dst->p) {
        dst->p = nullptr;
    }
    float* d = nullptr;
    HIP_TRY(hipMalloc((void**)&d, n * sizeof(float)));
    h->owned.push_back(d);
    HIP_TRY(hipMemcpy(d, host, n * sizeof(float), hipMemcpyHostToDevice));
    dst->p = d;
    dst->n = n;
    return ITTS_OK;
}

static int stage_channels(const itts_bigvgan_config& c, int i) { return c.upsample_initial_channel >> (i + 1); }

extern "C" int itts_bigvgan_create(const itts_bigvgan_config* cfg, itts_bigvgan** out) {
    if (!cfg || !out) { itts_set_error("bigvgan_create: null"); return ITTS_ERR_ARG; }
    const itts_bigvgan_config& c = *cfg;
    if (c.num_upsamples < 1 || c.num_upsamples > 8 || c.num_kernels < 1 || c.num_kernels > 4 || c.num_dilations < 1 ||
        c.num_dilations > 4 || c.in_channels % 8 || c.in_channels <= 0) {
        itts_set_error("bigvgan_create: unsupported config (ups=%d kernels=%d dil=%d in=%d)", c.num_upsamples,
                       c.num_kernels, c.num_dilations, c.in_channels);
        return ITTS_ERR_ARG;
    }
    for (int i = 0; i < c.num_upsamples; ++i) {
        const int uk = c.upsample_kernel_sizes[i], uu = c.upsample_rates[i];
        if (uu < 1 || uk < uu || uk % uu || ((uk - uu) & 1)) {
            itts_set_error("bigvgan_create: upsampler %d needs k a multiple of the stride with k-stride even (k=%d u=%d)", i, uk, uu);
            return ITTS_ERR_ARG;
        }
        if (stage_channels(c, i) < 1 || (c.upsample_initial_channel >> i) % 8) {
            itts_set_error("bigvgan_create: channel count at stage %d not a multiple of 8", i);
            return ITTS_ERR_ARG;
        }
    }
    if (stage_channels(c, c.num_upsamples - 1) % 8) {
        itts_set_error("bigvgan_create: final channel count %d not a multiple of 8", stage_channels(c, c.num_upsamples - 1));
        return ITTS_ERR_ARG;
    }
    for (int j = 0; j < c.num_kernels; ++j) {
        if ((c.resblock_kernel_sizes[j] & 1) == 0) { itts_set_error("even resblock kernel"); return ITTS_ERR_ARG; }
        for (int d = 0; d < c.num_dilations; ++d)
            if ((c.resblock_kernel_sizes[j] - 1) * c.resblock_dilations[j][d] > 64) {
                itts_set_error("bigvgan_create: receptive span of k=%d d=%d exceeds the 64-sample LDS halo",
                               c.resblock_kernel_sizes[j], c.resblock_dilations[j][d]);
                return ITTS_ERR_ARG;
            }
    }
    itts_bigvgan* h = new itts_bigvgan();
    h->cfg = c;
    h->device = itts_current_device();
    const int nres = c.num_upsamples * c.num_kernels;
    h->ups.resize(c.num_upsamples);
    h->conds.resize(c.num_upsamples);
    h->convs1.resize((size_t)nres * c.num_dilations);
    h->convs2.resize((size_t)nres * c.num_dilations);
    h->acts.resize((size_t)nres * 2 * c.num_dilations);
    h->total_up = 1;
    for (int i = 0; i < c.num_upsamples; ++i) h->total_up *= c.upsample_rates[i];
    *out = h;
    return ITTS_OK;
}

extern "C" int itts_bigvgan_device(const itts_bigvgan* h) { return h ? h->device : -1; }

extern "C" int itts_bigvgan_set_conv_mode(itts_bigvgan* h, int mode, int min_channels) {
    if (!h || mode < 0 || mode > 2) { itts_set_error("bigvgan_set_conv_mode: mode 0 (f32 MFMA), 1 (f16 x 3 split operands) or 2 (bf16 x 3 plane operands)"); return ITTS_ERR_ARG; }
    for (const ConvL& L : h->convs1)
        if (L.has_w) { itts_set_error("bigvgan_set_conv_mode: call before loading the weights"); return ITTS_ERR_STATE; }
    ItDevGuard dg(h->device);
    h->conv_mode = mode;
// ... 192 lines not shown
    const double cutoff = 0.25, half_width = 0.3, pi = 3.14159265358979323846;
    const double delta_f = 4 * half_width;
    const double A = 2.285 * (half - 1) * pi * delta_f + 7.95;
    double beta = 0.0;
    if (A > 50.0) beta = 0.1102 * (A - 8.7);
    else if (A >= 21.0) beta = 0.5842 * pow(A - 21.0, 0.4) + 0.07886 * (A - 21.0);
    double v[12], sum = 0;
    for (int n = 0; n < K; ++n) {
        const double r = 2.0 * n / (K - 1) - 1.0;
        const double win = bessel_i0(beta * sqrt(1.0 - r * r)) / bessel_i0(beta);
        const double t = (n - half) + 0.5;
        const double xx = 2 * cutoff * t;
        const double sinc = xx == 0 ? 1.0 : sin(pi * xx) / (pi * xx);
        v[n] = 2 * cutoff * win * sinc;
        sum += v[n];
    }
    for (int n = 0; n < K; ++n) f[n] = (float)(v[n] / sum);
}

extern "C" int itts_bigvgan_finalize(itts_bigvgan* h) {
    if (!h) { itts_set_error("finalize: null"); return ITTS_ERR_ARG; }
    ItDevGuard dg(h->device);
    const itts_bigvgan_config& c = h->cfg;
    std::string missing;
    auto need = [&](bool ok, const std::string& n) { if (!ok) missing += n + " "; };
    need(h->conv_pre.has_w, "conv_pre.weight");
    need(h->conv_pre.has_b, "conv_pre.bias");
    need(h->has_post_w, "conv_post.weight");
    if (c.use_bias_at_final) need(h->has_post_b, "conv_post.bias");
    for (int i = 0; i < c.num_upsamples; ++i) {
        need(h->ups[i].has_w, "ups." + std::to_string(i) + ".0.weight");
        need(h->ups[i].has_b, "ups." + std::to_string(i) + ".0.bias");
        if (c.cond_dim > 0 && c.cond_in_each_up_layer) need(h->conds[i].has_w && h->conds[i].has_b, "conds." + std::to_string(i));
    }
    if (c.cond_dim > 0) need(h->cond_layer.has_w && h->cond_layer.has_b, "cond_layer");
    for (size_t n = 0; n < h->convs1.size(); ++n) {
        need(h->convs1[n].has_w && h->convs1[n].has_b, "resblocks.convs1#" + std::to_string(n));
        need(h->convs2[n].has_w && h->convs2[n].has_b, "resblocks.convs2#" + std::to_string(n));
    }
    bool need_default = false;
    for (size_t n = 0; n < h->acts.size(); ++n) {
        need(h->acts[n].has_a && (c.activation == 1 || h->acts[n].has_b), "resblocks.activations#" + std::to_string(n));
        if (!h->acts[n].has_fu || !h->acts[n].has_fd) need_default = true;
    }
    need(h->act_post.has_a && (c.activation == 1 || h->act_post.has_b), "activation_post");
    if (!h->act_post.has_fu || !h->act_post.has_fd) need_default = true;
    if (!missing.empty()) {
        itts_set_error("bigvgan_finalize: missing tensors: %s", missing.c_str());
        return ITTS_ERR_STATE;
    }
    if (need_default && !h->default_filter.p) {
        float f[12];
        default_filter12(f);
        int rc = upload(h, f, 12, &h->default_filter);
        if (rc) return rc;
    }
    auto fix = [&](ActL& a) {
        if (!a.has_fu) a.fu = h->default_filter;
        if (!a.has_fd) a.fd = h->default_filter;
        if (c.activation == 1) a.beta = a.alpha;
    };
    for (auto& a : h->acts) fix(a);
    fix(h->act_post);
    h->finalized = true;
    return ITTS_OK;
}

static size_t max_stage_floats(const itts_bigvgan* h, int B, int T) {
    const itts_bigvgan_config& c = h->cfg;
    size_t mx = (size_t)c.upsample_initial_channel * T;
    size_t t = T;
    for (int i = 0; i < c.num_upsamples; ++i) {
        t *= c.upsample_rates[i];
        size_t v = (size_t)stage_channels(c, i) * t;
        if (v > mx) mx = v;
    }
    return mx * (size_t)B;
}

static size_t align256(size_t x) { return (x + 255) & ~(size_t)255; }

extern "C" size_t itts_bigvgan_workspace_bytes(const itts_bigvgan* h, int B, int T) {
    if (!h || B <= 0 || T <= 0) return 0;
    const itts_bigvgan_config& c = h->cfg;
    size_t cond = 0;
    if (c.cond_dim > 0) {
        cond = align256((size_t)B * c.upsample_initial_channel * 4);
        for (int i = 0; i < c.num_upsamples; ++i) cond += align256((size_t)B * stage_channels(c, i) * 4);
    }
    return (size_t)(h->conv_mode == 2 ? 9 : h->conv_mode == 1 ? 8 : 7) * align256(max_stage_floats(h, B, T) * sizeof(float)) + cond + 256;
}

extern "C" int itts_bigvgan_forward(itts_bigvgan* h, const float* x, const int32_t* lens, const float* spk, float* wav,
                                    int B, int T, void* workspace, size_t workspace_bytes, void* stream) {
    if (!h || !x || !wav || !workspace) { itts_set_error("bigvgan_forward: null pointer"); return ITTS_ERR_ARG; }
    if (!h->finalized) { itts_set_error("bigvgan_forward: call itts_bigvgan_finalize first"); return ITTS_ERR_STATE; }
    ItDevGuard dg(h->device);
    {
        const int dx = itts_ptr_device(x), dw = itts_ptr_device(workspace);
        if ((dx >= 0 && dx != h->device) || (dw >= 0 && dw != h->device)) {
            itts_set_error("bigvgan_forward: tensors are on device %d/%d but the model was created on device %d", dx, dw, h->device);
            return ITTS_ERR_ARG;
        }
    }
    if (B <= 0 || T <= 0) return ITTS_OK;
    if (B > 65535) { itts_set_error("bigvgan_forward: B must be <= 65535"); return ITTS_ERR_ARG; }
    const itts_bigvgan_config& c = h->cfg;
    if (c.cond_dim > 0 && !spk) { itts_set_error("bigvgan_forward: this model needs a speaker embedding"); return ITTS_ERR_ARG; }
    if (workspace_bytes < itts_bigvgan_workspace_bytes(h, B, T)) {
        itts_set_error("bigvgan_forward: workspace too small (%zu < %zu)", workspace_bytes, itts_bigvgan_workspace_bytes(h, B, T));
        return ITTS_ERR_ARG;
    }
    hipStream_t st = (hipStream_t)stream;
    const size_t bufsz = align256(max_stage_floats(h, B, T) * sizeof(float));
    char* base = (char*)(((uintptr_t)workspace + 255) & ~(uintptr_t)255);
    const int nbuf = h->conv_mode == 2 ? 9 : h->conv_mode == 1 ? 8 : 7;
    float* buf[8];
    for (int i = 0; i < 8; ++i) buf[i] = (float*)(base + bufsz * (i < nbuf ? i : 0));
    char* condp = base + bufsz * nbuf;
    float* SP = buf[7];
    float *P = buf[0], *X = buf[1], *XS = buf[2], *T1 = buf[3], *T2 = buf[4], *RA = buf[5], *RB = buf[6];
    const int ND = c.num_dilations;
    int rc;

    const float* cond0 = nullptr;
    std::vector<const float*> cond_up(c.num_upsamples, nullptr);
    if (c.cond_dim > 0) {
        float* p = (float*)condp;
        rc = launch_cond_bias(spk, h->cond_layer.w.p, h->cond_layer.b.p, p, B, c.upsample_initial_channel, c.cond_dim, st);
        if (rc) return rc;
        cond0 = p;
        condp += align256((size_t)B * c.upsample_initial_channel * 4);
        if (c.cond_in_each_up_layer)
            for (int i = 0; i < c.num_upsamples; ++i) {
                float* q = (float*)condp;
                rc = launch_cond_bias(spk, h->conds[i].w.p, h->conds[i].b.p, q, B, stage_channels(c, i), c.cond_dim, st);
                if (rc) return rc;
                cond_up[i] = q;
                condp += align256((size_t)B * stage_channels(c, i) * 4);
            }
    }

    h->recs.clear();
    h->prof_stream = st;
    auto conv_flops = [&](int Cin, int Cout, int k, int t) { return 2.0 * Cin * Cout * k * (double)t * B; };
    auto tensor_bytes = [&](int C, int t) { return 4.0 * C * (double)t * B; };
    { ProfScope ps(h, st, PC_CONV, conv_flops(c.in_channels, c.upsample_initial_channel, 7, T), tensor_bytes(c.in_channels + c.upsample_initial_channel, T));
    rc = conv1d_impl(x, h->conv_pre.w.p, h->conv_pre.b.p, cond0, nullptr, P, B, c.in_channels, c.upsample_initial_channel, T,
                     7, 1, lens, 1, 0, 1.f, st); }
    if (rc) return rc;

    const bool act_planes = h->conv_mode == 2 && itts_opt(OPT_VOC_ACT_PLANES) != 0 && itts_opt(OPT_AA_ACT) == 2;
    auto x3_conv = [&](const ConvL& L, int ch_, int kk_, int dil_) { return L.w3 && h->conv_mode == 2 && conv_x3_supported(ch_, ch_, kk_, dil_); };
    auto res_conv = [&](const ConvL& L, const float* xin, const float* res, float* yout, int ch_, int t_, int kk_, int dil_, int mult_, int mode_,
                        float div_, bool planes_ready) -> int {
        if (!L.w3 || (h->conv_mode == 2 && !conv_x3_supported(ch_, ch_, kk_, dil_)))
            return conv1d_impl(xin, L.w.p, L.b.p, nullptr, res, yout, B, ch_, ch_, t_, kk_, dil_, lens, mult_, mode_, div_, st);
        if (h->conv_mode == 2) {
            int rc3 = planes_ready ? ITTS_OK : launch_split_tm3(xin, SP, B, ch_, t_, lens, mult_, st);
            if (rc3) return rc3;
            ConvX3Args g{};
            g.xp = SP; g.wp = L.w3; g.bias = L.b.p; g.res = res; g.y = yout; g.zero_row = h->zero_row; g.lens = lens; g.len_mult = mult_;
            g.B = B; g.Cin = ch_; g.Cout = ch_; g.T = t_; g.k = kk_; g.dil = dil_; g.acc_mode = mode_; g.div = div_;
            return launch_conv_x3(g, st);
        }
        void* sh = SP;
        void* sl = (char*)SP + (size_t)B * t_ * ch_ * 2;
        int rc2 = launch_split_tm(xin, sh, sl, B, ch_, t_, lens, mult_, (int*)((char*)h->zero_row + 128), st);
        if (rc2) return rc2;
        ConvH3Args g{};
        g.xh = sh; g.xl = sl; g.wp = L.w3; g.bias = L.b.p; g.res = res; g.y = yout; g.zero_row = h->zero_row; g.lens = lens; g.len_mult = mult_;
        g.B = B; g.Cin = ch_; g.Cout = ch_; g.T = t_; g.k = kk_; g.dil = dil_; g.acc_mode = mode_; g.div = div_;
        return launch_conv_h3(g, st);
    };

    int t_cur = T, mult = 1;
    for (int i = 0; i < c.num_upsamples; ++i) {
        const int Cin = c.upsample_initial_channel >> i, ch = stage_channels(c, i);
        const int u = c.upsample_rates[i], k = c.upsample_kernel_sizes[i];
        { ProfScope ps(h, st, PC_CONVT, conv_flops(Cin, ch, k / u, t_cur * u), tensor_bytes(Cin, t_cur) + tensor_bytes(ch, t_cur * u));
          rc = convT_impl(P, h->ups[i].w.p, h->ups[i].b.p, cond_up[i], X, B, Cin, ch, t_cur, k, u, lens, mult, st); }
        if (rc) return rc;
        t_cur *= u;
        mult *= u;
        for (int j = 0; j < c.num_kernels; ++j) {
            const int n = i * c.num_kernels + j;
            const int kk = c.resblock_kernel_sizes[j];
            const float* cur = X;
            for (int d = 0; d < ND; ++d) {
                const ActL& a1 = h->acts[(size_t)n * 2 * ND + 2 * d];
                const ActL& a2 = h->acts[(size_t)n * 2 * ND + 2 * d + 1];
                const ConvL& c1 = h->convs1[(size_t)n * ND + d];
                const ConvL& c2 = h->convs2[(size_t)n * ND + d];
                const bool p1 = act_planes && x3_conv(c1, ch, kk, c.resblock_dilations[j][d]), p2 = act_planes && x3_conv(c2, ch, kk, 1);
                { ProfScope ps(h, st, PC_ACT, 0, tensor_bytes(2 * ch, t_cur));
                  rc = p1 ? launch_aa_act_planes(cur, SP, a1.alpha.p, a1.beta.p, a1.fu.p, a1.fd.p, B, ch, t_cur, lens, mult, c.snake_logscale, st)
                          : launch_aa_act(cur, T1, a1.alpha.p, a1.beta.p, a1.fu.p, a1.fd.p, B, ch, t_cur, lens, mult, c.snake_logscale, st); }
                if (rc) return rc;
                { ProfScope ps(h, st, PC_CONV, conv_flops(ch, ch, kk, t_cur), tensor_bytes(2 * ch, t_cur));
                  rc = res_conv(c1, T1, nullptr, T2, ch, t_cur, kk, c.resblock_dilations[j][d], mult, 0, 1.f, p1); }
                if (rc) return rc;
                { ProfScope ps(h, st, PC_ACT, 0, tensor_bytes(2 * ch, t_cur));
                  rc = p2 ? launch_aa_act_planes(T2, SP, a2.alpha.p, a2.beta.p, a2.fu.p, a2.fd.p, B, ch, t_cur, lens, mult, c.snake_logscale, st)
                          : launch_aa_act(T2, T1, a2.alpha.p, a2.beta.p, a2.fu.p, a2.fd.p, B, ch, t_cur, lens, mult, c.snake_logscale, st); }
                if (rc) return rc;
                if (d < ND - 1) {
                    float* nxt = (cur == RA) ? RB : RA;
                    { ProfScope ps(h, st, PC_CONV, conv_flops(ch, ch, kk, t_cur), tensor_bytes(3 * ch, t_cur));
                      rc = res_conv(c2, T1, cur, nxt, ch, t_cur, kk, 1, mult, 0, 1.f, p2); }
                    if (rc) return rc;
                    cur = nxt;
                } else {
                    int mode = (j == 0) ? 0 : 1;
                    if (j == c.num_kernels - 1) mode = (c.num_kernels == 1) ? 0 : 2;
                    { ProfScope ps(h, st, PC_CONV, conv_flops(ch, ch, kk, t_cur), tensor_bytes((mode ? 4 : 3) * ch, t_cur));
                      rc = res_conv(c2, T1, cur, XS, ch, t_cur, kk, 1, mult, mode, (float)c.num_kernels, p2); }
                    if (rc) return rc;
                }
            }
        }
        float* tmp = P; P = XS; XS = tmp;
    }
    const int ch = stage_channels(c, c.num_upsamples - 1);
    { ProfScope ps(h, st, PC_ACT, 0, tensor_bytes(2 * ch, t_cur));
      rc = launch_aa_act(P, T1, h->act_post.alpha.p, h->act_post.beta.p, h->act_post.fu.p, h->act_post.fd.p, B, ch, t_cur, lens, mult,
                         c.snake_logscale, st); }
    if (rc) return rc;
    ProfScope ps(h, st, PC_POST, 2.0 * ch * 7 * (double)t_cur * B, tensor_bytes(ch + 1, t_cur));
    return launch_conv_post(T1, wav, h->post_w.p, c.use_bias_at_final ? h->post_b.p : nullptr, B, ch, t_cur, 7, lens, mult,
                            c.use_tanh_at_final, st);
}

extern "C" int itts_bigvgan_set_profiling(itts_bigvgan* h, int enable) {
    if (!h) { itts_set_error("set_profiling: null"); return ITTS_ERR_ARG; }
    h->profiling = enable != 0;
    h->recs.clear();
    return ITTS_OK;
}

extern "C" int itts_bigvgan_profile_records(itts_bigvgan* h, double* out, int max_records) {
    if (!h || !out) { itts_set_error("profile_records: null"); return -1; }
    ItDevGuard dg(h->device);
    if (h->recs.empty()) return 0;
    if (hipStreamSynchronize(h->prof_stream) != hipSuccess) return -1;
    int n = 0;
    for (size_t i = 0; i < h->recs.size() && n < max_records; ++i, ++n) {
        float t = 0.f;
        (void)hipEventElapsedTime(&t, h->ev_pool[2 * i], h->ev_pool[2 * i + 1]);
        out[4 * n + 0] = h->recs[i].cls; out[4 * n + 1] = t; out[4 * n + 2] = h->recs[i].flops; out[4 * n + 3] = h->recs[i].bytes;
    }
    return (int)h->recs.size();
}

extern "C" int itts_bigvgan_profile_read(itts_bigvgan* h, double* ms, double* launches, double* flops, double* bytes) {
    if (!h || !ms || !launches || !flops || !bytes) { itts_set_error("profile_read: null"); return ITTS_ERR_ARG; }
    ItDevGuard dg(h->device);
    for (int i = 0; i < PC_COUNT; ++i) ms[i] = launches[i] = flops[i] = bytes[i] = 0;
    if (h->recs.empty()) return ITTS_OK;
    HIP_TRY(hipStreamSynchronize(h->prof_stream));
    for (size_t i = 0; i < h->recs.size(); ++i) {
        float t = 0.f;
        HIP_TRY(hipEventElapsedTime(&t, h->ev_pool[2 * i], h->ev_pool[2 * i + 1]));
        const auto& r = h->recs[i];
        ms[r.cls] += t; launches[r.cls] += 1; flops[r.cls] += r.flops; bytes[r.cls] += r.bytes;
    }
    return ITTS_OK;
}


struct itts_bigvgan_stream {
    itts_bigvgan* h;
    int chunk, halo, cap;
    int received, emitted;
    int base;
    float* ctx;
    float* xwin;
    float* wwin;
};

extern "C" int itts_bigvgan_stream_open(itts_bigvgan* h, int chunk_frames, int halo_frames, itts_bigvgan_stream** out) {
    if (!h || !out) { itts_set_error("bigvgan_stream_open: null pointer"); return ITTS_ERR_ARG; }
    if (!h->finalized) { itts_set_error("bigvgan_stream_open: call itts_bigvgan_finalize first"); return ITTS_ERR_STATE; }
    if (chunk_frames <= 0 || halo_frames < 0) { itts_set_error("bigvgan_stream_open: bad chunk/halo"); return ITTS_ERR_ARG; }
    ItDevGuard dg(h->device);
    auto* s = new itts_bigvgan_stream();
    s->h = h; s->chunk = chunk_frames; s->halo = halo_frames; s->cap = 2 * chunk_frames + 2 * halo_frames;
    s->received = s->emitted = s->base = 0;
    s->ctx = s->xwin = s->wwin = nullptr;
    const size_t C = (size_t)h->cfg.in_channels;
    hipError_t e = hipMalloc((void**)&s->ctx, C * s->cap * sizeof(float));
    if (e == hipSuccess) e = hipMalloc((void**)&s->xwin, C * s->cap * sizeof(float));
    if (e == hipSuccess) e = hipMalloc((void**)&s->wwin, (size_t)s->cap * h->total_up * sizeof(float));
    if (e != hipSuccess) {
        itts_set_error("bigvgan_stream_open: hipMalloc -> %s", hipGetErrorString(e));
        if (s->ctx) (void)hipFree(s->ctx);
        if (s->xwin) (void)hipFree(s->xwin);
        delete s;
        return ITTS_ERR_HIP;
    }
    *out = s;
    return ITTS_OK;
}

extern "C" void itts_bigvgan_stream_close(itts_bigvgan_stream* s) {
    if (!s) return;
    ItDevGuard dg(s->h->device);
    (void)hipFree(s->ctx); (void)hipFree(s->xwin); (void)hipFree(s->wwin);
    delete s;
}

extern "C" size_t itts_bigvgan_stream_workspace_bytes(const itts_bigvgan_stream* s) {
    return s ? itts_bigvgan_workspace_bytes(s->h, 1, s->cap) : 0;
}

extern "C" int itts_bigvgan_stream_push(itts_bigvgan_stream* s, const float* mel, int ld_mel, int n_frames, int is_last,
                                        const float* spk, float* wav_out, int32_t* n_samples_out, void* workspace,
                                        size_t workspace_bytes, void* stream) {
    if (!s || !wav_out || !n_samples_out || !workspace || (n_frames > 0 && !mel)) { itts_set_error("bigvgan_stream_push: null pointer"); return ITTS_ERR_ARG; }
    if (n_frames < 0 || n_frames > s->chunk || (n_frames > 0 && ld_mel < n_frames)) { itts_set_error("bigvgan_stream_push: n_frames %d outside 0..%d", n_frames, s->chunk); return ITTS_ERR_ARG; }
    ItDevGuard dg(s->h->device);
    hipStream_t st = (hipStream_t)stream;
    const int C = s->h->cfg.in_channels, up = s->h->total_up;
    *n_samples_out = 0;
    if (n_frames > 0) {
        const int col = s->received - s->base;
        HIP_TRY(hipMemcpy2DAsync(s->ctx + col, (size_t)s->cap * 4, mel, (size_t)ld_mel * 4, (size_t)n_frames * 4, C,
                                 hipMemcpyDeviceToDevice, st));
        s->received += n_frames;
    }
    const int emit_to = is_last ? s->received : s->received - s->halo;
    if (emit_to <= s->emitted) return ITTS_OK;
    const int w0 = (s->emitted - s->halo) > s->base ? (s->emitted - s->halo) : s->base;
    const int w1 = (emit_to + s->halo) < s->received ? (emit_to + s->halo) : s->received;
    const int Tw = w1 - w0;
    HIP_TRY(hipMemcpy2DAsync(s->xwin, (size_t)Tw * 4, s->ctx + (w0 - s->base), (size_t)s->cap * 4, (size_t)Tw * 4, C,
                             hipMemcpyDeviceToDevice, st));
    int rc = itts_bigvgan_forward(s->h, s->xwin, nullptr, spk, s->wwin, 1, Tw, workspace, workspace_bytes, stream);
    if (rc) return rc;
    const int n_out = (emit_to - s->emitted) * up;
    HIP_TRY(hipMemcpyAsync(wav_out, s->wwin + (size_t)(s->emitted - w0) * up, (size_t)n_out * 4, hipMemcpyDeviceToDevice, st));
    *n_samples_out = n_out;
    s->emitted = emit_to;
    const int nb = (s->emitted - s->halo) > s->base ? (s->emitted - s->halo) : s->base;
    if (nb > s->base) {
        const int keep = s->received - nb;
        if (keep > 0) {
            HIP_TRY(hipMemcpy2DAsync(s->xwin, (size_t)keep * 4, s->ctx + (nb - s->base), (size_t)s->cap * 4, (size_t)keep * 4, C,
                                     hipMemcpyDeviceToDevice, st));
            HIP_TRY(hipMemcpy2DAsync(s->ctx, (size_t)s->cap * 4, s->xwin, (size_t)keep * 4, (size_t)keep * 4, C,
                                     hipMemcpyDeviceToDevice, st));
        }
        s->base = nb;
    }
    return ITTS_OK;
}
```

### indextts_amd/csrc/common.h

```cpp
#pragma once
#include <hip/hip_runtime.h>
#include <stdint.h>
#include <stdio.h>
#include <string.h>

#define ITTS_OK 0
#define ITTS_ERR_ARG 1
#define ITTS_ERR_HIP 2
#define ITTS_ERR_STATE 3
#define ITTS_ERR_NOMEM 4

#define HIP_TRY(expr)                                                                         \
    do {                                                                                      \
        hipError_t _e = (expr);                                                               \
        if (_e != hipSuccess) {                                                               \
            itts_set_error("%s:%d %s -> %s", __FILE__, __LINE__, #expr, hipGetErrorString(_e)); \
            return ITTS_ERR_HIP;                                                              \
        }                                                                                     \
    } while (0)

void itts_set_error(const char* fmt, ...);

enum { OPT_DECODE_FUSE_LN, OPT_DECODE_GEMM, OPT_DECODE_ROT, OPT_DECODE_WNT, OPT_DECODE_NT, OPT_PREFILL_GEMM, OPT_TILE256, OPT_F32_TILE,
       OPT_X3_PRODUCTS, OPT_X3_SCHED, OPT_X3_ATTN, OPT_SAMPLE_RADIX, OPT_GPT_COMPACT, OPT_ATTN_WAVES, OPT_S2MEL_FUSED, OPT_FA_QS,
       OPT_F32_ATTN_SCALAR, OPT_FA32_QS, OPT_AA_ACT, OPT_CONV_BM, OPT_H3_KERNEL, OPT_DECODE_LN_NT, OPT_X3_APLANES, OPT_X3_PIN, OPT_PREFILL_ATTN, OPT_VOC_ACT_PLANES, OPT_X3_WAVES, OPT_S2MEL_PRUNE_LAST, OPT_X3_ATTN_SKIP, OPT_COUNT };
int itts_opt(int id);
unsigned itts_opt_epoch();

typedef float f32x4 __attribute__((ext_vector_type(4)));
typedef float f32x16 __attribute__((ext_vector_type(16)));
typedef short bf16x8 __attribute__((ext_vector_type(8)));
typedef unsigned short u16;

static inline int ceil_div(int a, int b) { return (a + b - 1) / b; }

struct ItDevGuard {
    int prev = -1;
    bool switched = false;
    explicit ItDevGuard(int dev) {
        if (dev < 0) return;
        if (hipGetDevice(&prev) != hipSuccess) { prev = -1; (void)hipGetLastError(); }
        if (prev != dev && hipSetDevice(dev) == hipSuccess) switched = true;
    }
    ~ItDevGuard() { if (switched && prev >= 0) (void)hipSetDevice(prev); }
    ItDevGuard(const ItDevGuard&) = delete;
    ItDevGuard& operator=(const ItDevGuard&) = delete;
};
static inline int itts_current_device() {
    int d = -1;
    if (hipGetDevice(&d) != hipSuccess) { d = -1; (void)hipGetLastError(); }
    return d;
}
static inline int itts_ptr_device(const void* p) {
    hipPointerAttribute_t at;
    if (!p || hipPointerGetAttributes(&at, p) != hipSuccess) { (void)hipGetLastError(); return -1; }
    return at.type == hipMemoryTypeDevice ? at.device : -1;
}

template <class T>
struct ItPerDevice {
    T v[32] = {};
    T& cur() {
        const int d = itts_current_device();
        return v[(d >= 0 && d < 32) ? d : 0];
    }
};

#ifdef __HIPCC__
__device__ __forceinline__ float wave_sum(float v) {
#pragma unroll
    for (int o = 32; o > 0; o >>= 1) v += __shfl_xor(v, o, 64);
    return v;
}
__device__ __forceinline__ float wave_max(float v) {
#pragma unroll
    for (int o = 32; o > 0; o >>= 1) v = fmaxf(v, __shfl_xor(v, o, 64));
    return v;
}
__device__ __forceinline__ float bf16_to_f32(u16 h) { return __uint_as_float(((uint32_t)h) << 16); }
__device__ __forceinline__ u16 f32_to_bf16(float f) {
    uint32_t u = __float_as_uint(f);
    if ((u & 0x7fffffffu) > 0x7f800000u) return (u16)((u >> 16) | 0x40);
    u += 0x7fffu + ((u >> 16) & 1u);
    return (u16)(u >> 16);
}
#endif

static inline u16 host_f32_to_bf16(float f) {
    uint32_t u;
    memcpy(&u, &f, 4);
    if ((u & 0x7fffffffu) > 0x7f800000u) return (u16)((u >> 16) | 0x40);
    u += 0x7fffu + ((u >> 16) & 1u);
    return (u16)(u >> 16);
}
```

### indextts_amd/csrc/options.hip

```cpp
#include <atomic>
#include <stdlib.h>
#include <string.h>

#include "../../include/indextts_hip.h"
#include "common.h"

namespace {
struct OptDef {
    const char* name;
    int def, lo, hi;
    const char* doc;
    const char* allowed = nullptr;
};
const OptDef kDefs[OPT_COUNT] = {
    {"decode_fuse_ln", 1, 0, 2, "GPT decode: LayerNorm (+ split-K reduce, bias, residual) inside the consuming GEMM -- 1: steps of 1-8 rows (measured faster), 2: up to 16 rows (measured slower above 8, kept for the A/B record), 0: separate ln_kernel launches; bitwise equal"},
    {"decode_gemm", 1, 0, 1, "bf16 decode GEMMs on the LDS-DMA slab kernel (0: register-path gemm_kernel; bitwise equal)"},
    {"decode_rot", 1, 0, 1, "per-block rotation of the slab DMA issue order in the decode GEMM (same bytes, same LDS image)"},
    {"decode_wnt", 0, 0, 1, "non-temporal policy on the decode GEMM's weight stream"},
    {"decode_nt", 0, 0, 4, "force the n-tiles per block of the 64-row decode GEMM (0: smallest that fits one round of blocks)", "0,1,2,4"},
    {"prefill_gemm", 1, 0, 1, "bf16 prefill GEMMs on the LDS-DMA tile kernels (0: register-path gemm_kernel; bitwise equal)"},
    {"tile256", -1, -1, 2, "bf16 tile GEMM: -1 pick by shape, 0 always 128x128, 1 always 256x256, 2 always 256x128 (bitwise equal)"},
    {"f32_tile", 1, 0, 1, "f32 GEMMs with plain epilogues on the f32-MFMA tile kernel (0: register-path kernel; bitwise equal)"},
    {"x3_products", 6, 6, 8, "plane products per f32 product of the fp32x3 GEMMs and attention: 6 (hh, hm, mh, hl, lh, mm; drops m*l and l*m, 2^-24 |ab| each: measured error vs f64 <= the native f32-MFMA kernels' on every benchmarked shape) or 8 (every term down to 2^-24 |ab|; two blocks per CU like the default since the packed-RoPE fix -- option x3_pin = 1 restores round 4's one-block pin as a diagnostic)", "6,8"},
    {"x3_sched", 1, 0, 1, "fp32x3 GEMM: interleave the operand split with the MFMAs (0: split as a burst; bitwise equal)"},
    {"x3_attn", 1, 0, 1, "fp32x3 s2mel: attention products on bf16 planes too (K / V^T written as three planes by the wqkv epilogue, flash_attn_x3_kernel); 0: the f32-MFMA flash kernel"},
    {"sample_radix", -1, -1, 1, "top-k threshold: -1 per-kernel default (radix select in sample_kernel, ballot bisection in the beam kernels), 0 bisection, 1 radix select (identical ids)"},
    {"gpt_compact", 1, 0, 1, "row compaction of ragged decode batches (0 disables it for every handle; identical ids)"},
    {"attn_waves", 0, 0, 16, "waves per block of the KV-cache attention kernel: 0 pick by shape, else 4 / 8 / 16 (the 16 canonical key streams are mapped onto them; bitwise equal)", "0,4,8,16"},
    {"s2mel_fused", 1, 0, 2, "s2mel: fused GEMM epilogues, sampled when a handle is created -- 1: fused, 0: separate element-wise kernels (2: round 4's spelling of 'the bf16 wqkv epilogue fused too'; the same as 1 since the RoPE fix of round 5)"},
    {"fa_qs", 0, 0, 4, "bf16 flash attention: query sub-tiles per wave (0: pick by shape)", "0,1,2,4"},
    {"f32_attn_scalar", 0, 0, 1, "f32 s2mel attention on the one-wave-per-query reference kernel (the A/B path of the f32 flash kernel)"},
    {"fa32_qs", 2, 1, 2, "f32 flash attention: query sub-tiles per wave"},
    {"aa_act", 2, 0, 2, "anti-aliased activation kernel variant (2: swizzled LDS tiles)"},
    {"conv_bm", 0, 0, 128, "force the co-tile height of conv_mfma_kernel (0: pick by channel count)", "0,32,64,96,128"},
    {"h3_kernel", 1, 0, 1, "f16x3 vocoder conv: 1 window kernel, 0 two-stage kernel"},
    {"decode_ln_nt", 2, 2, 4, "LayerNorm-fused decode GEMM at 5-16 rows (weights on waves 0-3, LayerNorm on waves 4-7): n-tiles per block, 2 or 4 (bitwise equal)", "2,4"},
    {"x3_aplanes", 0, 0, 1, "fp32x3 s2mel: the adaptive-RMSNorm outputs as three bf16 planes in fragment order, wqkv / w1|w3 GEMMs without an operand split (bitwise equal)"},
    {"x3_pin", 0, 0, 1, "fp32x3 GEMM: 1 pins the variants that are not the default one (8 products, burst split) to one block per CU -- round 4's workaround for their run-to-run differences, kept as a diagnostic; not needed since the RoPE fix of round 5 (DESIGN.md section 9)"},
    {"prefill_attn", -1, -1, 1, "attention of S > 1 passes (prefill, latent pass): -1 causal MFMA kernel in the bf16 mode, canonical-stream kernel in the f32 parity mode; 0 canonical-stream kernel (one block per query) always; 1 MFMA kernel in both precisions"},
    {"voc_act_planes", 1, 0, 1, "vocoder, bf16x3 conv mode: the anti-aliased activation in front of an x3 conv writes the conv's three operand planes itself (aa_act_planes_kernel); 0: f32 activation + split pass (bit-identical planes)"},
    {"x3_waves", 8, 4, 8, "fp32x3 GEMM: waves per 128 x 128 block -- 8 (4 x 2, wave tile 32 x 64, weights through LDS: four waves per SIMD at two blocks per CU; 64-utterance solve 314.7 vs 323.0 ms per Euler step, profiles/r06k) or 4 (2 x 2, wave tile 64 x 64, weights in registers: round 5's kernel); bitwise equal", "4,8"},
    {"s2mel_prune_last", 1, 0, 1, "fp32x3 s2mel solve with a tail layout: the LAST DiT layer's attention runs the queries of the tail rows only (keys / values: every frame) and writes the tail layout, its wo / FFN norm / w1|w3 / w2 stages run on the tail rows (residual gathered by a row map in the wo epilogue); the x_in GEMM reads its residual from const_in instead of a copy of it; 0: every row, copy first (bitwise equal)"},
    {"x3_attn_skip", 1, 0, 1, "fp32x3 flash attention: a last key tile with <= 32 valid keys skips the MFMAs of its fully masked half, and a wave whose 32 queries are all out of range only stages its share of K / V^T (0: full tiles, every wave computes; bitwise equal)"},
};
std::atomic<int> g_val[OPT_COUNT];
std::atomic<unsigned> g_epoch{1};
std::atomic<bool> g_init{false};

void ensure_init() {
    if (g_init.load(std::memory_order_acquire)) return;
    static std::atomic_flag once = ATOMIC_FLAG_INIT;
    if (!once.test_and_set()) {
        for (int i = 0; i < OPT_COUNT; ++i) g_val[i].store(kDefs[i].def, std::memory_order_relaxed);
        g_init.store(true, std::memory_order_release);
    } else {
        while (!g_init.load(std::memory_order_acquire)) {}
    }
}
int find(const char* name) {
    if (!name) return -1;
    for (int i = 0; i < OPT_COUNT; ++i)
        if (strcmp(kDefs[i].name, name) == 0) return i;
    return -1;
}
}

int itts_opt(int id) {
    ensure_init();
    return g_val[id].load(std::memory_order_relaxed);
}
unsigned itts_opt_epoch() { return g_epoch.load(std::memory_order_relaxed); }

extern "C" int itts_set_option(const char* name, int value) {
    ensure_init();
    const int i = find(name);
    if (i < 0) { itts_set_error("set_option: unknown option '%s'", name ? name : "(null)"); return ITTS_ERR_ARG; }
    if (value < kDefs[i].lo || value > kDefs[i].hi) {
        itts_set_error("set_option: %s = %d outside [%d, %d]", name, value, kDefs[i].lo, kDefs[i].hi);
        return ITTS_ERR_ARG;
    }
    if (kDefs[i].allowed) {
        bool ok = false;
        for (const char* p = kDefs[i].allowed; *p;) {
            char* end;
            const long v = strtol(p, &end, 10);
            ok |= v == value;
            p = *end == ',' ? end + 1 : end;
        }
        if (!ok) { itts_set_error("set_option: %s = %d is not one of {%s}", name, value, kDefs[i].allowed); return ITTS_ERR_ARG; }
    }
    if (g_val[i].exchange(value) != value) g_epoch.fetch_add(1);
    return ITTS_OK;
}
extern "C" int itts_get_option(const char* name, int* value) {
    ensure_init();
    const int i = find(name);
    if (i < 0 || !value) { itts_set_error("get_option: unknown option '%s'", name ? name : "(null)"); return ITTS_ERR_ARG; }
    *value = g_val[i].load();
    return ITTS_OK;
}
extern "C" int itts_reset_options(void) {
    ensure_init();
    bool changed = false;
    for (int i = 0; i < OPT_COUNT; ++i) changed |= g_val[i].exchange(kDefs[i].def) != kDefs[i].def;
    if (changed) g_epoch.fetch_add(1);
    return ITTS_OK;
}
extern "C" int itts_option_count(void) { return OPT_COUNT; }
extern "C" const char* itts_option_name(int index) { return (index >= 0 && index < OPT_COUNT) ? kDefs[index].name : nullptr; }
extern "C" const char* itts_option_doc(int index) { return (index >= 0 && index < OPT_COUNT) ? kDefs[index].doc : nullptr; }
extern "C" int itts_option_default(int index) { return (index >= 0 && index < OPT_COUNT) ? kDefs[index].def : 0; }
```

Baseline: 143.2.

## Keep vocoder resblock residual stream token-major across x3 conv stages

Adds a token-major [B][T][C] layout for the BigVGAN residual stream in stages whose resblock convs all run on the bf16x3 kernel. The upsampler and x3 convs write through token-major epilogues, a new activation kernel reads token-major input directly into planes, and one transpose per stage hands the output back to channel-major for the next upsampler. The aim is to remove per-activation transpose or split work and improve coalescing, at the cost of an extra transpose pass and new code paths. It is enabled by default through the voc_tm option.

```diff
diff --git a/include/indextts_hip.h b/include/indextts_hip.h
--- a/include/indextts_hip.h
+++ b/include/indextts_hip.h
@@ -59,6 +59,13 @@
                                const float* down_filter, int B, int C, int T, const int32_t* lens, int len_mult, int logscale,
                                void* stream);
 int itts_sin_reduced_forward(const float* x, float* y, size_t n, void* stream);
+
+int itts_aa_act_planes_tm_forward(const float* x, void* planes, const float* alpha, const float* beta, const float* up_filter,
+                                  const float* down_filter, int B, int C, int T, const int32_t* lens, int len_mult, int logscale,
+                                  void* stream);
+int itts_conv1d_x3_tm_forward(const float* x, const void* wp3, const float* bias, const float* res, float* y, int B, int Cin, int Cout,
+                              int T, int k, int dilation, const int32_t* lens, int len_mult, int acc_mode, float div, void* scratch,
+                              void* stream);
 
 typedef struct {
     int32_t in_channels;
diff --git a/indextts_amd/_lib.py b/indextts_amd/_lib.py
--- a/indextts_amd/_lib.py
+++ b/indextts_amd/_lib.py
@@ -94,6 +94,9 @@
     "itts_voc_path_name": (C.c_char_p, [C.c_int]),
     "itts_aa_act_planes_forward": (C.c_int, [vp, vp, vp, vp, vp, vp, C.c_int, C.c_int, C.c_int, vp, C.c_int, C.c_int, vp]),
     "itts_sin_reduced_forward": (C.c_int, [vp, vp, C.c_size_t, vp]),
+    "itts_aa_act_planes_tm_forward": (C.c_int, [vp, vp, vp, vp, vp, vp, C.c_int, C.c_int, C.c_int, vp, C.c_int, C.c_int, vp]),
+    "itts_conv1d_x3_tm_forward": (C.c_int, [vp, vp, vp, vp, vp, C.c_int, C.c_int, C.c_int, C.c_int, C.c_int, C.c_int, vp, C.c_int, C.c_int,
+                                            C.c_float, vp, vp]),
     "itts_bigvgan_create": (C.c_int, [C.POINTER(BigVGANConfig), C.POINTER(vp)]),
     "itts_bigvgan_device": (C.c_int, [vp]),
     "itts_bigvgan_load_tensor": (C.c_int, [vp, C.c_char_p, vp, c_i64p, C.c_int]),
diff --git a/indextts_amd/bigvgan.py b/indextts_amd/bigvgan.py
--- a/indextts_amd/bigvgan.py
+++ b/indextts_amd/bigvgan.py
@@ -354,6 +354,23 @@
         return p
 
 
+def anti_alias_activation_planes_tm(x, up_filter, down_filter, alpha, beta, lens=None, logscale=True, *, len_mult=1, out=None):
+    if not x.is_cuda:
+        raise _lib.HipEngineError("anti_alias_activation_planes_tm needs a device tensor")
+    x = x.float().contiguous()
+    B, T, Cc = x.shape
+    dev = x.device
+    p = out if out is not None else torch.empty(3, B, T, Cc, dtype=torch.bfloat16, device=dev)
+    f = lambda t: t.detach().reshape(-1).to(dev, torch.float32).contiguous()
+    a, b, fu, fd = f(alpha), f(beta), f(up_filter), f(down_filter)
+    lens_t = None if lens is None else torch.as_tensor(lens, dtype=torch.int32, device=dev).contiguous()
+    with _lib.on_device(x.device):
+        _lib.check(_lib.lib().itts_aa_act_planes_tm_forward(_lib.ptr(x), _lib.ptr(p), _lib.ptr(a), _lib.ptr(b), _lib.ptr(fu), _lib.ptr(fd), B, Cc, T,
+                                                            _lib.ptr(lens_t), int(len_mult), int(logscale), _lib.stream_ptr(x.device)),
+                   "itts_aa_act_planes_tm_forward")
+        return p
+
+
 def sin_reduced(x):
     if not x.is_cuda:
         raise _lib.HipEngineError("sin_reduced needs a device tensor")
@@ -425,6 +442,20 @@
         return y
 
 
+def conv1d_x3_tm(x, w3_packed, bias, Cout, k, dilation=1, res=None, lens=None, len_mult=1, out=None, acc_mode=0, div=1.0):
+    x = x.float().contiguous()
+    B, Cin, T = x.shape
+    y = out if out is not None else torch.empty(B, T, Cout, dtype=torch.float32, device=x.device)
+    lens_t = None if lens is None else torch.as_tensor(lens, dtype=torch.int32, device=x.device).contiguous()
+    L = _lib.lib()
+    scratch = torch.empty(L.itts_conv1d_x3_scratch_bytes(B, Cin, T), dtype=torch.uint8, device=x.device)
+    with _lib.on_device(x.device):
+        _lib.check(L.itts_conv1d_x3_tm_forward(_lib.ptr(x), _lib.ptr(w3_packed), _lib.ptr(bias), _lib.ptr(res), _lib.ptr(y), B, Cin, Cout, T, k,
+                                               dilation, _lib.ptr(lens_t), len_mult, acc_mode, float(div), _lib.ptr(scratch),
+                                               _lib.stream_ptr(x.device)), "itts_conv1d_x3_tm_forward")
+        return y
+
+
 def pack_convT_weight(w: torch.Tensor, u: int) -> torch.Tensor:
     w = w.detach().to("cpu", torch.float32).contiguous()
     Cin, Cout, k = w.shape
diff --git a/indextts_amd/csrc/bigvgan_kernels.h b/indextts_amd/csrc/bigvgan_kernels.h
--- a/indextts_amd/csrc/bigvgan_kernels.h
+++ b/indextts_amd/csrc/bigvgan_kernels.h
@@ -15,6 +15,7 @@
     int acc_mode;
     float div;
     int B, n_mt, n_co;
+    int y_tm = 0;
 };
 
 enum VocPath {
@@ -61,6 +62,7 @@
     int B, Cin, Cout, T, k, dil;
     int acc_mode; float div;
     int n_mt, n_co;
+    int tm;
 };
 bool conv_x3_supported(int Cin, int Cout, int k, int dil);
 size_t conv_x3_packed_bytes(int Cout, int Cin, int k);
@@ -69,6 +71,9 @@
 int launch_aa_act_planes(const float* x, void* xp, const float* alpha, const float* beta, const float* fu, const float* fd,
                          int B, int C, int T, const int* lens, int len_mult, int logscale, hipStream_t st);
 int launch_conv_x3(const ConvX3Args& a, hipStream_t st);
+int launch_aa_act_planes_tm(const float* x, void* xp, const float* alpha, const float* beta, const float* fu, const float* fd,
+                            int B, int C, int T, const int* lens, int len_mult, int logscale, hipStream_t st);
+int launch_tm_to_cm(const float* x, float* y, int B, int C, int T, const int* lens, int len_mult, hipStream_t st);
 size_t conv_h3_packed_bytes(int Cout, int Cin, int k);
 int conv_h3_pack(const float* w, int Cout, int Cin, int k, void* out);
 int launch_split_tm(const float* x, void* xh, void* xl, int B, int C, int T, const int* lens, int len_mult, int* range_flag, hipStream_t st);
diff --git a/indextts_amd/csrc/bigvgan_kernels.hip b/indextts_amd/csrc/bigvgan_kernels.hip
--- a/indextts_amd/csrc/bigvgan_kernels.hip
+++ b/indextts_amd/csrc/bigvgan_kernels.hip
@@ -318,11 +318,131 @@
     }
 }
 
+#ifndef AAT_CHUNK
+#define AAT_CHUNK 128
+#endif
+#define AAT_U 4
+__global__ __launch_bounds__(256) void aa_act_planes_tm_kernel(const float* __restrict__ x, u16* __restrict__ xh, u16* __restrict__ xm, u16* __restrict__ xl,
+                                                               const float* __restrict__ alpha, const float* __restrict__ beta,
+                                                               const float* __restrict__ fu, const float* __restrict__ fd,
+                                                               int C, int T, int n_chunk, int n_cg, long long n_task,
+                                                               const int* __restrict__ lens, int len_mult, int logscale) {
+    const int lane = threadIdx.x & 63;
+    const long long task = (long long)blockIdx.x * 4 + __builtin_amdgcn_readfirstlane(threadIdx.x >> 6);
+    if (task >= n_task) return;
+    const int cg = (int)(task % n_cg);
+    const long long bc = task / n_cg;
+    const int b = (int)(bc / n_chunk), t0 = (int)(bc - (long long)b * n_chunk) * AAT_CHUNK;
+    const int c = cg * 64 + lane;
+    if (c >= C) return;
+    const int len = lens ? min(lens[b] * len_mult, T) : T;
+    const size_t row0 = (size_t)b * T;
+    u16* ph = xh + row0 * C + c;
+    u16* pm = xm + row0 * C + c;
+    u16* pl = xl + row0 * C + c;
+    const int t_end = min(t0 + AAT_CHUNK, T);
+    if (t0 >= len) {
+        for (int t = t0; t < t_end; ++t) { ph[(size_t)t * C] = 0; pm[(size_t)t * C] = 0; pl[(size_t)t * C] = 0; }
+        return;
+    }
+    float fus[12], fds[12];
+#pragma unroll
+    for (int j = 0; j < 12; ++j) { fus[j] = 2.0f * fu[j]; fds[j] = fd[j]; }
+    float a_e = alpha[c], b_e = beta[c];
+    if (logscale) { a_e = expf(a_e); b_e = expf(b_e); }
+    const float inv_b = 1.0f / (b_e + 1e-9f);
+    const float* xc = x + row0 * C + c;
+    auto ld = [&](int t) { t = t < 0 ? 0 : (t > len - 1 ? len - 1 : t); return xc[(size_t)t * C]; };
+    float vlast = 0.f;
+    auto pair = [&](const float* X, int tp, float& vo, float& ve) {
+        float uo = 0.f, ue = 0.f;
+#pragma unroll
+        for (int j = 0; j < 6; ++j) {
+            ue = fmaf(fus[1 + 2 * j], X[5 - j], ue);
+            uo = fmaf(fus[2 * j], X[5 - j], uo);
+        }
+        const float so = sin_reduced(uo * a_e);
+        const float se = sin_reduced(ue * a_e);
+        vo = fmaf(inv_b * so, so, uo);
+        ve = fmaf(inv_b * se, se, ue);
+        if (tp + 3 <= len) vlast = vo; else vo = vlast;
+        if (tp + 3 > len - 1) ve = vlast;
+    };
+    float X[5 + AAT_U], V[10 + 2 * AAT_U], xn[AAT_U];
+    {
+        float W[10];
+#pragma unroll
+        for (int i = 0; i < 10; ++i) W[i] = ld(t0 - 5 + i);
+#pragma unroll
+        for (int i = 0; i < AAT_U; ++i) xn[i] = ld(t0 + 5 + i);
+#pragma unroll
+        for (int p = 0; p < 5; ++p) pair(&W[p], t0 - 5 + p, V[2 * p], V[2 * p + 1]);
+#pragma unroll
+        for (int i = 0; i < 5; ++i) X[i] = W[5 + i];
+        if (t0 == 0) {
+#pragma unroll
+            for (int i = 0; i < 5; ++i) V[i] = V[5];
+        }
+    }
+#pragma unroll 1
+    for (int t = t0; t < t_end; t += AAT_U) {
+#pragma unroll
+        for (int i = 0; i < AAT_U; ++i) X[5 + i] = xn[i];
+        if (t + AAT_U < t_end && t + AAT_U < len) {
+#pragma unroll
+            for (int i = 0; i < AAT_U; ++i) xn[i] = ld(t + AAT_U + 5 + i);
+        }
+#pragma unroll
+        for (int p = 0; p < AAT_U; ++p) {
+            if (t + p >= t_end) break;
+            float o = 0.f;
+            if (t + p < len) {
+                pair(&X[p], t + p, V[10 + 2 * p], V[11 + 2 * p]);
+#pragma unroll
+                for (int j = 0; j < 12; ++j) o = fmaf(fds[j], V[2 * p + j], o);
+            }
+            const uint32_t h = aap_cvt2(o, 0.f) & 0xffffu;
+            const float r = o - __uint_as_float(h << 16);
+            const uint32_t m = aap_cvt2(r, 0.f) & 0xffffu;
+            const float s = r - __uint_as_float(m << 16);
+            const uint32_t l = aap_cvt2(s, 0.f) & 0xffffu;
+            const size_t off = (size_t)(t + p) * C;
+            ph[off] = (u16)h; pm[off] = (u16)m; pl[off] = (u16)l;
+        }
+#pragma unroll
+        for (int i = 0; i < 5; ++i) X[i] = X[AAT_U + i];
+#pragma unroll
+        for (int i = 0; i < 10; ++i) V[i] = V[2 * AAT_U + i];
+    }
+}
+
+__global__ __launch_bounds__(256) void tm_to_cm_kernel(const float* __restrict__ x, float* __restrict__ y, int C, int T,
+                                                       const int* __restrict__ lens, int len_mult) {
+    __shared__ float tile[64][65];
+    const int b = blockIdx.z, c0 = blockIdx.y * 64, t0 = blockIdx.x * 64;
+    const int len = lens ? min(lens[b] * len_mult, T) : T;
+    if (t0 >= len) return;
+    const int lane = threadIdx.x & 63, w = threadIdx.x >> 6;
+    const float* xb = x + (size_t)b * T * C;
+    float* yb = y + (size_t)b * C * T;
+#pragma unroll
+    for (int i = 0; i < 16; ++i) {
+        const int t = t0 + w * 16 + i, c = c0 + lane;
+        tile[w * 16 + i][lane] = (t < T && c < C) ? xb[(size_t)t * C + c] : 0.f;
+    }
+    __syncthreads();
+#pragma unroll
+    for (int i = 0; i < 16; ++i) {
+        const int c = c0 + w * 16 + i, t = t0 + lane;
+        if (c < C && t < T) yb[(size_t)c * T + t] = tile[lane][w * 16 + i];
+    }
+}
+
 #define CI_CHUNK 32
 #define CONV_HALO 64
 
 
-template <int WM, int WN, int MT, int NT>
+template <int WM, int WN, int MT, int NT, bool YTM = false>
 __global__ __launch_bounds__(256) __attribute__((amdgpu_waves_per_eu((WM == 1 && MT == 1) ? 4 : 1, (WM == 1 && MT == 1) ? 4 : 8)))
 void conv_mfma_kernel(ConvArgs a) {
     constexpr int BM = WM * MT * 32;
@@ -494,6 +614,19 @@
                 const int m = m0 + (wn * NT + nt) * 32 + lane_col;
                 const int n = m * a.ostride + a.ooff;
                 const bool n_ok = (m < m_count) && (n >= 0) && (n < len_out);
+                if (YTM) {
+#pragma unroll
+                    for (int g4 = 0; g4 < 2; ++g4) {
+                        const bool ok = n_ok && corow[4 * g4] < a.Cout;
+                        const unsigned off = ok ? (unsigned)(n * a.Cout + corow[4 * g4]) * 4u : 0xFFFFFFF0u;
+                        typedef unsigned u32x4 __attribute__((ext_vector_type(4)));
+                        u32x4 pv;
+#pragma unroll
+                        for (int q = 0; q < 4; ++q) pv[q] = __builtin_bit_cast(unsigned, acc[mt][nt][hf * 8 + 4 * g4 + q] + badd[4 * g4 + q]);
+                        __builtin_amdgcn_raw_buffer_store_b128(pv, yrs, off, 0, 0);
+                    }
+                    continue;
+                }
                 unsigned voff[8];
                 float v[8];
 #pragma unroll
@@ -608,8 +741,32 @@
     return ITTS_OK;
 }
 
+int launch_aa_act_planes_tm(const float* x, void* xp, const float* alpha, const float* beta, const float* fu, const float* fd,
+                            int B, int C, int T, const int* lens, int len_mult, int logscale, hipStream_t st) {
+    if (B <= 0 || C <= 0 || T <= 0) return ITTS_OK;
+    u16* p = (u16*)xp;
+    const size_t plane = (size_t)B * T * C;
+    const int n_chunk = ceil_div(T, AAT_CHUNK), n_cg = ceil_div(C, 64);
+    const long long n_task = (long long)B * n_chunk * n_cg;
+    const long long nblocks = (n_task + 3) / 4;
+    if (nblocks > 2147483647ll) { itts_set_error("aa_act_planes_tm: grid too large"); return ITTS_ERR_ARG; }
+    hipLaunchKernelGGL(aa_act_planes_tm_kernel, dim3((unsigned)nblocks), dim3(256), 0, st, x, p, p + plane, p + 2 * plane, alpha, beta, fu, fd,
+                       C, T, n_chunk, n_cg, n_task, lens, len_mult, logscale);
+    HIP_TRY(hipGetLastError());
+    return ITTS_OK;
+}
+
+int launch_tm_to_cm(const float* x, float* y, int B, int C, int T, const int* lens, int len_mult, hipStream_t st) {
+    if (B <= 0 || C <= 0 || T <= 0) return ITTS_OK;
+    if (B > 65535 || ceil_div(C, 64) > 65535) { itts_set_error("tm_to_cm: B and C / 64 must be <= 65535"); return ITTS_ERR_ARG; }
+    hipLaunchKernelGGL(tm_to_cm_kernel, dim3(ceil_div(T, 64), ceil_div(C, 64), B), dim3(256), 0, st, x, y, C, T, lens, len_mult);
+    HIP_TRY(hipGetLastError());
+    return ITTS_OK;
+}
+
 template <int WM, int WN, int MT, int NT>
 static int launch_conv_cfg(const ConvArgs& a, int B, int m_total, hipStream_t st) {
+    if (a.y_tm && ((a.Cout & 3) || a.res || a.acc_mode != 0)) { itts_set_error("conv: a token-major output needs C_out %% 4 == 0 and a plain store"); return ITTS_ERR_ARG; }
     constexpr int BM = WM * MT * 32, BN = WN * NT * 32;
     const size_t lds = (size_t)CI_CHUNK * (BN + CONV_HALO) * sizeof(float);
     ConvArgs a2 = a;
@@ -620,7 +777,8 @@
     const long long nblocks = tiles8 * a2.n_co;
     if (nblocks > 2147483647ll) { itts_set_error("conv: grid too large"); return ITTS_ERR_ARG; }
     voc_note_path(VP_CONV_F32_BM32 + BM / 32 - 1);
-    hipLaunchKernelGGL((conv_mfma_kernel<WM, WN, MT, NT>), dim3((unsigned)nblocks), dim3(256), lds, st, a2);
+    if (a.y_tm) hipLaunchKernelGGL((conv_mfma_kernel<WM, WN, MT, NT, true>), dim3((unsigned)nblocks), dim3(256), lds, st, a2);
+    else hipLaunchKernelGGL((conv_mfma_kernel<WM, WN, MT, NT, false>), dim3((unsigned)nblocks), dim3(256), lds, st, a2);
     HIP_TRY(hipGetLastError());
     return ITTS_OK;
 }
diff --git a/indextts_amd/csrc/bigvgan_x3.hip b/indextts_amd/csrc/bigvgan_x3.hip
--- a/indextts_amd/csrc/bigvgan_x3.hip
+++ b/indextts_amd/csrc/bigvgan_x3.hip
@@ -63,7 +63,7 @@
 template <int N>
 __device__ __forceinline__ void cx3_wait_vm() { asm volatile("s_waitcnt vmcnt(%0)" ::"n"(N) : "memory"); }
 
-template <int NH>
+template <int NH, bool TM>
 __global__ __launch_bounds__(512) __attribute__((amdgpu_waves_per_eu(2, 2))) void conv_x3w_kernel(ConvX3Args a) {
     extern __shared__ __attribute__((aligned(16))) char sm[];
     const int lane = threadIdx.x & 63, w = __builtin_amdgcn_readfirstlane(threadIdx.x >> 6);
@@ -170,8 +170,10 @@
             for (int q = 0; q < 6; ++q)
 #pragma unroll
                 for (int nt = 0; nt < CX3_NT; ++nt)
-                    ac[mt][nt] = __builtin_amdgcn_mfma_f32_16x16x32_bf16(__builtin_bit_cast(x3_bf16x8, afc[mt][PA[q]]),
-                                                                         __builtin_bit_cast(x3_bf16x8, bf[nt][PB[q]]), ac[mt][nt], 0, 0, 0);
+                    ac[mt][nt] = TM ? __builtin_amdgcn_mfma_f32_16x16x32_bf16(__builtin_bit_cast(x3_bf16x8, bf[nt][PB[q]]),
+                                                                              __builtin_bit_cast(x3_bf16x8, afc[mt][PA[q]]), ac[mt][nt], 0, 0, 0)
+                                    : __builtin_amdgcn_mfma_f32_16x16x32_bf16(__builtin_bit_cast(x3_bf16x8, afc[mt][PA[q]]),
+                                                                              __builtin_bit_cast(x3_bf16x8, bf[nt][PB[q]]), ac[mt][nt], 0, 0, 0);
             if (more) {
                 const int rr = rbase_n + mt * 16;
                 const char* ap = abase_n + (rr >> 4) * 1024 + kg * 256 + (rr & 15) * 16;
@@ -193,6 +195,34 @@
         }
     }
 
+    if (TM) {
+        float* yb = a.y + (size_t)b * a.T * a.Cout;
+        const float* rb = a.res ? a.res + (size_t)b * a.T * a.Cout : nullptr;
+#pragma unroll
+        for (int h = 0; h < NH; ++h)
+#pragma unroll
+        for (int nt = 0; nt < CX3_NT; ++nt) {
+            const int co = co0 + h * CX3_BN + (wc * CX3_NT + nt) * 16 + (lane >> 4) * 4;
+            if (co >= a.Cout) continue;
+            f32x4 bias = f32x4{0.f, 0.f, 0.f, 0.f};
+            if (a.bias) bias = f32x4{a.bias[co], a.bias[co + 1], a.bias[co + 2], a.bias[co + 3]};
+#pragma unroll
+            for (int mt = 0; mt < CX3_MT; ++mt) {
+                const int t = m0 + (wr * CX3_MT + mt) * 16 + (lane & 15);
+                if (t >= len) continue;
+                f32x4 v = acc[h][mt][nt] + bias;
+                const size_t o = (size_t)t * a.Cout + co;
+                if (rb) { const f32x4 rv = *(const f32x4*)(rb + o); v += rv; }
+                if (a.acc_mode != 0) {
+                    const f32x4 yo = *(const f32x4*)(yb + o);
+                    v = yo + v;
+                    if (a.acc_mode == 2) v = v / a.div;
+                }
+                *(f32x4*)(yb + o) = v;
+            }
+        }
+        return;
+    }
     const bool vec = (a.T & 3) == 0;
     float* yb = a.y + (size_t)b * a.Cout * a.T;
     const float* rb = a.res ? a.res + (size_t)b * a.Cout * a.T : nullptr;
@@ -292,6 +322,7 @@
         itts_set_error("conv_x3: need C_in %% 32 == 0, odd k >= 3 and (k - 1) * dilation <= %d (Cin=%d k=%d dil=%d)", CX3_SLACK, a0.Cin, a0.k, a0.dil);
         return ITTS_ERR_ARG;
     }
+    if (a0.tm && (a0.Cout & 3)) { itts_set_error("conv_x3: the token-major epilogue needs C_out %% 4 == 0 (Cout=%d)", a0.Cout); return ITTS_ERR_ARG; }
     if ((long long)a0.Cout * a0.T >= (1ll << 31) || (long long)a0.Cin * a0.T >= (1ll << 31)) { itts_set_error("conv_x3: row plane too large"); return ITTS_ERR_ARG; }
     ConvX3Args a = a0;
     const int nh = a.Cout > CX3_BN ? 2 : 1;
@@ -303,13 +334,18 @@
     static ItPerDevice<bool> attr_set_pd;
     bool& attr_set = attr_set_pd.cur();
     if (!attr_set) {
-        HIP_TRY(hipFuncSetAttribute((const void*)conv_x3w_kernel<1>, hipFuncAttributeMaxDynamicSharedMemorySize, CX3_LDS));
-        HIP_TRY(hipFuncSetAttribute((const void*)conv_x3w_kernel<2>, hipFuncAttributeMaxDynamicSharedMemorySize, CX3_LDS));
+        HIP_TRY(hipFuncSetAttribute((const void*)conv_x3w_kernel<1, false>, hipFuncAttributeMaxDynamicSharedMemorySize, CX3_LDS));
+        HIP_TRY(hipFuncSetAttribute((const void*)conv_x3w_kernel<2, false>, hipFuncAttributeMaxDynamicSharedMemorySize, CX3_LDS));
+        HIP_TRY(hipFuncSetAttribute((const void*)conv_x3w_kernel<1, true>, hipFuncAttributeMaxDynamicSharedMemorySize, CX3_LDS));
+        HIP_TRY(hipFuncSetAttribute((const void*)conv_x3w_kernel<2, true>, hipFuncAttributeMaxDynamicSharedMemorySize, CX3_LDS));
         attr_set = true;
     }
     voc_note_path(nh == 2 ? VP_CONV_X3_NH2 : VP_CONV_X3_NH1);
-    if (nh == 2) hipLaunchKernelGGL(conv_x3w_kernel<2>, dim3((unsigned)nblocks), dim3(512), CX3_LDS, st, a);
-    else hipLaunchKernelGGL(conv_x3w_kernel<1>, dim3((unsigned)nblocks), dim3(512), CX3_LDS, st, a);
+    if (a.tm) {
+        if (nh == 2) hipLaunchKernelGGL((conv_x3w_kernel<2, true>), dim3((unsigned)nblocks), dim3(512), CX3_LDS, st, a);
+        else hipLaunchKernelGGL((conv_x3w_kernel<1, true>), dim3((unsigned)nblocks), dim3(512), CX3_LDS, st, a);
+    } else if (nh == 2) hipLaunchKernelGGL((conv_x3w_kernel<2, false>), dim3((unsigned)nblocks), dim3(512), CX3_LDS, st, a);
+    else hipLaunchKernelGGL((conv_x3w_kernel<1, false>), dim3((unsigned)nblocks), dim3(512), CX3_LDS, st, a);
     HIP_TRY(hipGetLastError());
     return ITTS_OK;
 }
diff --git a/indextts_amd/csrc/capi_bigvgan.hip b/indextts_amd/csrc/capi_bigvgan.hip
--- a/indextts_amd/csrc/capi_bigvgan.hip
+++ b/indextts_amd/csrc/capi_bigvgan.hip
@@ -94,6 +94,17 @@
     if (B > 65535 || C > 65535 * 32) { itts_set_error("aa_act_planes: B must be <= 65535, C <= 32 * 65535"); return ITTS_ERR_ARG; }
     return launch_aa_act_planes(x, planes, alpha, beta, up_filter, down_filter, B, C, T, lens, len_mult < 1 ? 1 : len_mult, logscale,
                                 (hipStream_t)stream);
+}
+
+extern "C" int itts_aa_act_planes_tm_forward(const float* x, void* planes, const float* alpha, const float* beta, const float* up_filter,
+                                             const float* down_filter, int B, int C, int T, const int32_t* lens, int len_mult, int logscale,
+                                             void* stream) {
+    if (!x || !planes || !alpha || !beta || !up_filter || !down_filter || B < 0 || C < 0 || T < 0) {
+        itts_set_error("aa_act_planes_tm: null pointer or negative dim");
+        return ITTS_ERR_ARG;
+    }
+    return launch_aa_act_planes_tm(x, planes, alpha, beta, up_filter, down_filter, B, C, T, lens, len_mult < 1 ? 1 : len_mult, logscale,
+                                   (hipStream_t)stream);
 }
 
 extern "C" int itts_sin_reduced_forward(const float* x, float* y, size_t n, void* stream) {
@@ -150,9 +161,9 @@
 extern "C" size_t itts_conv1d_x3_packed_bytes(int Cout, int Cin, int k) { return (Cin > 0 && Cin % 32 == 0 && Cout > 0 && k > 0) ? conv_x3_packed_bytes(Cout, Cin, k) : 0; }
 extern "C" int itts_pack_conv1d_x3_weight(const float* w, int Cout, int Cin, int k, void* out) { return conv_x3_pack(w, Cout, Cin, k, out); }
 extern "C" size_t itts_conv1d_x3_scratch_bytes(int B, int Cin, int T) { return (size_t)B * T * Cin * 6 + 512; }
-extern "C" int itts_conv1d_x3_forward(const float* x, const void* wp3, const float* bias, const float* res, float* y, int B, int Cin, int Cout,
-                                      int T, int k, int dilation, const int32_t* lens, int len_mult, int acc_mode, float div, void* scratch,
-                                      void* stream) {
+static int conv1d_x3_unit(const float* x, const void* wp3, const float* bias, const float* res, float* y, int B, int Cin, int Cout,
+                          int T, int k, int dilation, const int32_t* lens, int len_mult, int acc_mode, float div, void* scratch,
+                          void* stream, int tm) {
     if (!x || !wp3 || !y || !scratch || B < 0 || T < 0 || acc_mode < 0 || acc_mode > 2) { itts_set_error("conv1d_x3_forward: bad args"); return ITTS_ERR_ARG; }
     if (B == 0 || T == 0) return ITTS_OK;
     hipStream_t st = (hipStream_t)stream;
@@ -164,12 +175,22 @@
     if (rc) return rc;
     ConvX3Args g{};
     g.xp = base; g.wp = wp3; g.bias = bias; g.res = res; g.y = y; g.zero_row = zr; g.lens = lens; g.len_mult = len_mult < 1 ? 1 : len_mult;
-    g.B = B; g.Cin = Cin; g.Cout = Cout; g.T = T; g.k = k; g.dil = dilation; g.acc_mode = acc_mode; g.div = div;
+    g.B = B; g.Cin = Cin; g.Cout = Cout; g.T = T; g.k = k; g.dil = dilation; g.acc_mode = acc_mode; g.div = div; g.tm = tm;
     return launch_conv_x3(g, st);
 }
+extern "C" int itts_conv1d_x3_forward(const float* x, const void* wp3, const float* bias, const float* res, float* y, int B, int Cin, int Cout,
+                                      int T, int k, int dilation, const int32_t* lens, int len_mult, int acc_mode, float div, void* scratch,
+                                      void* stream) {
+    return conv1d_x3_unit(x, wp3, bias, res, y, B, Cin, Cout, T, k, dilation, lens, len_mult, acc_mode, div, scratch, stream, 0);
+}
+extern "C" int itts_conv1d_x3_tm_forward(const float* x, const void* wp3, const float* bias, const float* res, float* y, int B, int Cin, int Cout,
+                                         int T, int k, int dilation, const int32_t* lens, int len_mult, int acc_mode, float div, void* scratch,
+                                         void* stream) {
+    return conv1d_x3_unit(x, wp3, bias, res, y, B, Cin, Cout, T, k, dilation, lens, len_mult, acc_mode, div, scratch, stream, 1);
+}
 
 static int convT_impl(const float* x, const float* wpk_phases, const float* bias, const float* bias_b, float* y, int B,
-                      int Cin, int Cout, int Tin, int k, int u, const int* lens, int len_mult_in, hipStream_t st) {
+                      int Cin, int Cout, int Tin, int k, int u, const int* lens, int len_mult_in, hipStream_t st, int y_tm = 0) {
     const int p = (k - u) / 2, ntaps = k / u;
     const size_t per_phase = itts_packed_conv_floats(Cout, Cin, ntaps);
     for (int r = 0; r < u; ++r) {
@@ -178,7 +199,7 @@
         a.lens = lens; a.len_mult_in = len_mult_in; a.len_mult_out = len_mult_in * u;
         a.Cin = Cin; a.Cout = Cout; a.Tin = Tin; a.Tout = Tin * u;
         a.k = ntaps; a.tap_base = 0; a.tap_step = -1; a.ostride = u; a.ooff = r - p; a.m_extra = ntaps - 1;
-        a.acc_mode = 0; a.div = 1.f;
+        a.acc_mode = 0; a.div = 1.f; a.y_tm = y_tm;
         int rc = launch_conv(a, B, st);
         if (rc) return rc;
     }
@@ -677,6 +698,18 @@
 
     const bool act_planes = h->conv_mode == 2 && itts_opt(OPT_VOC_ACT_PLANES) != 0 && itts_opt(OPT_AA_ACT) == 2;
     auto x3_conv = [&](const ConvL& L, int ch_, int kk_, int dil_) { return L.w3 && h->conv_mode == 2 && conv_x3_supported(ch_, ch_, kk_, dil_); };
+    const bool tm_on = act_planes && itts_opt(OPT_VOC_TM) != 0;
+    auto stage_tm = [&](int i_, int ch_) {
+        if (!tm_on || (ch_ & 7)) return false;
+        for (int j_ = 0; j_ < c.num_kernels; ++j_)
+            for (int d_ = 0; d_ < ND; ++d_) {
+                const size_t n_ = (size_t)(i_ * c.num_kernels + j_) * ND + d_;
+                if (!x3_conv(h->convs1[n_], ch_, c.resblock_kernel_sizes[j_], c.resblock_dilations[j_][d_]) ||
+                    !x3_conv(h->convs2[n_], ch_, c.resblock_kernel_sizes[j_], 1)) return false;
+            }
+        return true;
+    };
+    bool tm = false;
     auto res_conv = [&](const ConvL& L, const float* xin, const float* res, float* yout, int ch_, int t_, int kk_, int dil_, int mult_, int mode_,
                         float div_, bool planes_ready) -> int {
         if (!L.w3 || (h->conv_mode == 2 && !conv_x3_supported(ch_, ch_, kk_, dil_)))
@@ -686,7 +719,7 @@
             if (rc3) return rc3;
             ConvX3Args g{};
             g.xp = SP; g.wp = L.w3; g.bias = L.b.p; g.res = res; g.y = yout; g.zero_row = h->zero_row; g.lens = lens; g.len_mult = mult_;
-            g.B = B; g.Cin = ch_; g.Cout = ch_; g.T = t_; g.k = kk_; g.dil = dil_; g.acc_mode = mode_; g.div = div_;
+            g.B = B; g.Cin = ch_; g.Cout = ch_; g.T = t_; g.k = kk_; g.dil = dil_; g.acc_mode = mode_; g.div = div_; g.tm = tm ? 1 : 0;
             return launch_conv_x3(g, st);
         }
         void* sh = SP;
@@ -704,7 +737,8 @@
         const int Cin = c.upsample_initial_channel >> i, ch = stage_channels(c, i);
         const int u = c.upsample_rates[i], k = c.upsample_kernel_sizes[i];
         { ProfScope ps(h, st, PC_CONVT, conv_flops(Cin, ch, k / u, t_cur * u), tensor_bytes(Cin, t_cur) + tensor_bytes(ch, t_cur * u));
-          rc = convT_impl(P, h->ups[i].w.p, h->ups[i].b.p, cond_up[i], X, B, Cin, ch, t_cur, k, u, lens, mult, st); }
+          tm = stage_tm(i, ch);
+          rc = convT_impl(P, h->ups[i].w.p, h->ups[i].b.p, cond_up[i], X, B, Cin, ch, t_cur, k, u, lens, mult, st, tm ? 1 : 0); }
         if (rc) return rc;
         t_cur *= u;
         mult *= u;
@@ -719,14 +753,16 @@
                 const ConvL& c2 = h->convs2[(size_t)n * ND + d];
                 const bool p1 = act_planes && x3_conv(c1, ch, kk, c.resblock_dilations[j][d]), p2 = act_planes && x3_conv(c2, ch, kk, 1);
                 { ProfScope ps(h, st, PC_ACT, 0, tensor_bytes(2 * ch, t_cur));
-                  rc = p1 ? launch_aa_act_planes(cur, SP, a1.alpha.p, a1.beta.p, a1.fu.p, a1.fd.p, B, ch, t_cur, lens, mult, c.snake_logscale, st)
+                  rc = tm ? launch_aa_act_planes_tm(cur, SP, a1.alpha.p, a1.beta.p, a1.fu.p, a1.fd.p, B, ch, t_cur, lens, mult, c.snake_logscale, st)
+                     : p1 ? launch_aa_act_planes(cur, SP, a1.alpha.p, a1.beta.p, a1.fu.p, a1.fd.p, B, ch, t_cur, lens, mult, c.snake_logscale, st)
                           : launch_aa_act(cur, T1, a1.alpha.p, a1.beta.p, a1.fu.p, a1.fd.p, B, ch, t_cur, lens, mult, c.snake_logscale, st); }
                 if (rc) return rc;
                 { ProfScope ps(h, st, PC_CONV, conv_flops(ch, ch, kk, t_cur), tensor_bytes(2 * ch, t_cur));
                   rc = res_conv(c1, T1, nullptr, T2, ch, t_cur, kk, c.resblock_dilations[j][d], mult, 0, 1.f, p1); }
                 if (rc) return rc;
                 { ProfScope ps(h, st, PC_ACT, 0, tensor_bytes(2 * ch, t_cur));
-                  rc = p2 ? launch_aa_act_planes(T2, SP, a2.alpha.p, a2.beta.p, a2.fu.p, a2.fd.p, B, ch, t_cur, lens, mult, c.snake_logscale, st)
+                  rc = tm ? launch_aa_act_planes_tm(T2, SP, a2.alpha.p, a2.beta.p, a2.fu.p, a2.fd.p, B, ch, t_cur, lens, mult, c.snake_logscale, st)
+                     : p2 ? launch_aa_act_planes(T2, SP, a2.alpha.p, a2.beta.p, a2.fu.p, a2.fd.p, B, ch, t_cur, lens, mult, c.snake_logscale, st)
                           : launch_aa_act(T2, T1, a2.alpha.p, a2.beta.p, a2.fu.p, a2.fd.p, B, ch, t_cur, lens, mult, c.snake_logscale, st); }
                 if (rc) return rc;
                 if (d < ND - 1) {
@@ -739,7 +775,8 @@
                     int mode = (j == 0) ? 0 : 1;
                     if (j == c.num_kernels - 1) mode = (c.num_kernels == 1) ? 0 : 2;
                     { ProfScope ps(h, st, PC_CONV, conv_flops(ch, ch, kk, t_cur), tensor_bytes((mode ? 4 : 3) * ch, t_cur));
-                      rc = res_conv(c2, T1, cur, XS, ch, t_cur, kk, 1, mult, mode, (float)c.num_kernels, p2); }
+                      rc = res_conv(c2, T1, cur, XS, ch, t_cur, kk, 1, mult, mode, (float)c.num_kernels, p2);
+                      if (!rc && tm && j == c.num_kernels - 1) { rc = launch_tm_to_cm(XS, X, B, ch, t_cur, lens, mult, st); float* sw = XS; XS = X; X = sw; } }
                     if (rc) return rc;
                 }
             }
diff --git a/indextts_amd/csrc/common.h b/indextts_amd/csrc/common.h
--- a/indextts_amd/csrc/common.h
+++ b/indextts_amd/csrc/common.h
@@ -23,7 +23,7 @@
 
 enum { OPT_DECODE_FUSE_LN, OPT_DECODE_GEMM, OPT_DECODE_ROT, OPT_DECODE_WNT, OPT_DECODE_NT, OPT_PREFILL_GEMM, OPT_TILE256, OPT_F32_TILE,
        OPT_X3_PRODUCTS, OPT_X3_SCHED, OPT_X3_ATTN, OPT_SAMPLE_RADIX, OPT_GPT_COMPACT, OPT_ATTN_WAVES, OPT_S2MEL_FUSED, OPT_FA_QS,
-       OPT_F32_ATTN_SCALAR, OPT_FA32_QS, OPT_AA_ACT, OPT_CONV_BM, OPT_H3_KERNEL, OPT_DECODE_LN_NT, OPT_X3_APLANES, OPT_X3_PIN, OPT_PREFILL_ATTN, OPT_VOC_ACT_PLANES, OPT_X3_WAVES, OPT_S2MEL_PRUNE_LAST, OPT_X3_ATTN_SKIP, OPT_COUNT };
+       OPT_F32_ATTN_SCALAR, OPT_FA32_QS, OPT_AA_ACT, OPT_CONV_BM, OPT_H3_KERNEL, OPT_DECODE_LN_NT, OPT_X3_APLANES, OPT_X3_PIN, OPT_PREFILL_ATTN, OPT_VOC_ACT_PLANES, OPT_X3_WAVES, OPT_S2MEL_PRUNE_LAST, OPT_X3_ATTN_SKIP, OPT_VOC_TM, OPT_COUNT };
 int itts_opt(int id);
 unsigned itts_opt_epoch();
 
diff --git a/indextts_amd/csrc/options.hip b/indextts_amd/csrc/options.hip
--- a/indextts_amd/csrc/options.hip
+++ b/indextts_amd/csrc/options.hip
@@ -42,6 +42,7 @@
     {"x3_waves", 8, 4, 8, "fp32x3 GEMM: waves per 128 x 128 block -- 8 (4 x 2, wave tile 32 x 64, weights through LDS: four waves per SIMD at two blocks per CU; 64-utterance solve 314.7 vs 323.0 ms per Euler step, profiles/r06k) or 4 (2 x 2, wave tile 64 x 64, weights in registers: round 5's kernel); bitwise equal", "4,8"},
     {"s2mel_prune_last", 1, 0, 1, "fp32x3 s2mel solve with a tail layout: the LAST DiT layer's attention runs the queries of the tail rows only (keys / values: every frame) and writes the tail layout, its wo / FFN norm / w1|w3 / w2 stages run on the tail rows (residual gathered by a row map in the wo epilogue); the x_in GEMM reads its residual from const_in instead of a copy of it; 0: every row, copy first (bitwise equal)"},
     {"x3_attn_skip", 1, 0, 1, "fp32x3 flash attention: a last key tile with <= 32 valid keys skips the MFMAs of its fully masked half, and a wave whose 32 queries are all out of range only stages its share of K / V^T (0: full tiles, every wave computes; bitwise equal)"},
+    {"voc_tm", 1, 0, 1, "vocoder, bf16x3 conv mode: the residual stream of a stage whose resblock convs all run on the x3 kernel is token-major [B][T][C] -- the upsampler and the x3 convs write it through token-major epilogues, the activation in front of an x3 conv reads it without a transpose (aa_act_planes_tm_kernel), one transpose pass hands the stage's output to the next upsampler; needs voc_act_planes = 1 and aa_act = 2; 0: channel-major stream (bitwise equal)"},
 };
 std::atomic<int> g_val[OPT_COUNT];
 std::atomic<unsigned> g_epoch{1};
```

Result: no change. 144.6 (median of 6 runs) (+0.9%).
